# bezirganyan/m2-mixer

Measured on AMD Instinct MI355X. Metric: training samples/sec AV-MNIST M2-Mixer-B bf16, higher is better.
Workload: dtype bf16

## Files before the change

include/m2mixer.h:

```cpp
#ifndef M2MIXER_H
#define M2MIXER_H

#include <stdint.h>

#ifdef __cplusplus
extern "C" {
#endif

#define M2M_ABI_VERSION 18
#define M2M_MAX_BLOCKS 8
#define M2M_ROWS_PER_WG 16

#define M2M_SPLIT_GPART 1472

#define M2M_PREC_BF16 0
#define M2M_PREC_F32 1

typedef struct m2m_block {
    const float* ln1_w;
    const float* ln1_b;
    const float* tok_w1;
    const float* tok_b1;
    const float* tok_w2;
    const float* tok_b2;
// ... 92 lines not shown
    const float* x0; int64_t x0_sample_stride;
    float* out; int64_t out_sample_stride;
    float* pooled;
    int32_t x0_parts;
    int64_t x0_part_stride;
} m2m_tower_io;
int m2m_towers_forward(const m2m_tower* const* towers, const m2m_tower_io* io, int ntowers, int B, int training,
                       uint32_t seed, uint32_t step, const uint32_t* step_dev, void* stream);
int m2m_towers_forward_embeds_ok(const m2m_tower* const* towers, int ntowers, const m2m_embed* const* embeds, int B);
int m2m_towers_forward_embeds(const m2m_tower* const* towers, const m2m_tower_io* io, int ntowers,
                              const m2m_embed* const* embeds, const float* const* inputs, const m2m_step_head* head,
                              int B, int training, uint32_t seed, uint32_t step, const uint32_t* step_dev, void* stream);

int m2m_tower_backward(const m2m_tower* t, int B, const float* d_out, int64_t d_out_sample_stride,
                       const float* d_pooled, float* d_x0, int64_t d_x0_sample_stride,
                       uint32_t seed, uint32_t step, const uint32_t* step_dev, void* stream);
typedef struct m2m_tower_gio {
    const float* d_out; int64_t d_out_sample_stride;
    const float* d_pooled;
    float* d_x0; int64_t d_x0_sample_stride;
} m2m_tower_gio;
int m2m_towers_backward(const m2m_tower* const* towers, const m2m_tower_gio* io, int ntowers, int B,
                        uint32_t seed, uint32_t step, const uint32_t* step_dev, void* stream);
int m2m_tower_wgrad(const m2m_tower* t, int B, uint32_t seed, uint32_t step, const uint32_t* step_dev, void* stream);
int m2m_wgrad_form(const m2m_tower* t, int B);
int m2m_split_form(const m2m_tower* a, const m2m_tower* b, int B, int training);
int m2m_towers_wgrad(const m2m_tower* const* towers, const m2m_tower* const* dev_towers, int ntowers,
                     const m2m_embed* const* embeds, const float* const* inputs, const float* const* d_x0s,
                     const m2m_tower* const* embed_towers, int nembeds,
                     int B, uint32_t seed, uint32_t step, const uint32_t* step_dev, void* stream);
int m2m_wgrad_groups(const m2m_tower* t, int B);
int m2m_embeds_wgrad_form(const m2m_embed* const* embeds, const m2m_tower* const* embed_towers, int nembeds, int B);
int m2m_wgrad_slot_groups(const m2m_tower* const* towers, int ntowers, int B);
int m2m_wgrad_fold(const m2m_tower* t, void* stream);
int m2m_embed_wgrad(const m2m_embed* e, const float* input, const float* d_x0, int B, void* stream);
int m2m_embeds_wgrad(const m2m_embed* const* embeds, const float* const* inputs, const float* const* d_x0s, int nembeds, int B,
                     void* stream);

typedef struct m2m_head {
    const float* pooled;
    const float* w;
    const float* b;
    float* g_w;
    float* g_b;
    float* d_pooled;
    float weight;
    float* g_part;
    const float* tokens;
    int64_t tok_sample_stride;
    int32_t ntok;
} m2m_head;
int m2m_heads_part_tiles(int B);
int m2m_heads_ce(const m2m_head* heads, int nheads, const int64_t* labels, int B, int D, int K,
                 float* logits, float* losses, int32_t* preds, int zero_losses, void* stream);

int m2m_heads_bce(const m2m_head* heads, int nheads, const float* targets, const float* pos_weight, int B, int D, int K,
                  float* logits, float* losses, int32_t* preds, int zero_losses, void* stream);

int m2m_heads_ce_w(const m2m_head* heads, int nheads, const int64_t* labels, int B, int D, int K,
                   float* logits, float* losses, int32_t* preds, int zero_losses, const float* weights, void* stream);
int m2m_heads_bce_w(const m2m_head* heads, int nheads, const float* targets, const float* pos_weight, int B, int D, int K,
                    float* logits, float* losses, int32_t* preds, int zero_losses, const float* weights, void* stream);

int m2m_heads_edl(const m2m_head* heads, int nheads, const int64_t* labels, int B, int D, int K,
                  float* logits, float* losses, int32_t* preds, float* uncertainty, int32_t* combined,
                  int zero_losses, const float* weights, void* stream);

int m2m_towers_wgrad_heads(const m2m_tower* const* towers, const m2m_tower* const* dev_towers, int ntowers,
                           const m2m_embed* const* embeds, const float* const* inputs, const float* const* d_x0s,
                           const m2m_tower* const* embed_towers, int nembeds,
                           int B, uint32_t seed, uint32_t step, const uint32_t* step_dev,
                           const m2m_head* heads, int nheads, int K, void* stream);

int m2m_towers_wgrad_tail(const m2m_tower* const* towers, const m2m_tower* const* dev_towers, int ntowers,
                          const m2m_embed* const* embeds, const float* const* inputs, const float* const* d_x0s,
                          const m2m_tower* const* embed_towers, int nembeds,
                          int B, uint32_t seed, uint32_t step, const uint32_t* step_dev,
                          const m2m_head* heads, int nheads, int K, uint32_t* bump_counter, void* stream);

int m2m_tower_backward_heads_ok(const m2m_tower* t, int B, int nheads, int K);
int m2m_tower_backward_heads(const m2m_tower* t, int B, const m2m_head* heads, int nheads, int own, const int64_t* labels,
                             int K, float* logits, float* losses, int32_t* preds, float* d_x0, int64_t d_x0_sample_stride,
                             uint32_t seed, uint32_t step, const uint32_t* step_dev, void* stream);

#define M2M_MLP_MAX_LAYERS 4
typedef struct m2m_mlp {
    int32_t nlayers;
    int32_t has_out;
    int32_t dims[M2M_MLP_MAX_LAYERS + 1];
    float p_drop;
    uint32_t site_base;
    const float* w[M2M_MLP_MAX_LAYERS];
    const float* b[M2M_MLP_MAX_LAYERS];
    float* g_w[M2M_MLP_MAX_LAYERS];
    float* g_b[M2M_MLP_MAX_LAYERS];
    float* act[M2M_MLP_MAX_LAYERS];
} m2m_mlp;
int m2m_mlp_forward(const m2m_mlp* m, const float* x, int B, float* out, int64_t out_sample_stride, float* out_dense,
                    int training, uint32_t seed, uint32_t step, const uint32_t* step_dev, void* stream);
int m2m_mlp_backward(const m2m_mlp* m, const float* x, int B, const float* d_out, int64_t d_out_sample_stride,
                     const float* d_out_dense, void* stream);
int m2m_mlp_forward_ride(const m2m_mlp* m, const float* x, int B, float* out, int64_t out_sample_stride, float* out_dense,
                         int training, uint32_t seed, uint32_t step, const uint32_t* step_dev);
int m2m_mlp_backward_ride(const m2m_mlp* m, const float* x, int B, const float* d_out, int64_t d_out_sample_stride,
                          const float* d_out_dense);
int m2m_mlp_ride_flush(void* stream);

int m2m_adam_step(float* param, float* grad, float* exp_avg, float* exp_avg_sq, int64_t n,
                  float* state, float beta1, float beta2, float eps, float weight_decay,
                  float grad_scale, int bump_step, void* stream);
int m2m_adam_step_bf16(float* param, float* grad, const void* grad_bf16, float* exp_avg, float* exp_avg_sq, int64_t n,
                       float* state, float beta1, float beta2, float eps, float weight_decay,
                       float grad_scale, int bump_step, void* stream);

#define M2M_MAX_GRAD_RANGES 16
typedef struct m2m_grad_range { int64_t lo, n; const float* add; int32_t keep; int32_t reserved; } m2m_grad_range;
int m2m_adam_step_ranges(float* param, float* grad, const void* grad_bf16, float* exp_avg, float* exp_avg_sq, int64_t n,
                         float* state, float beta1, float beta2, float eps, float weight_decay, float grad_scale, int bump_step,
                         const m2m_grad_range* ranges, int nranges, void* stream);

int64_t m2m_adam_pack_plan_bytes(void);
int m2m_adam_pack_plan(const m2m_tower* const* towers, int ntowers, const m2m_embed* const* embeds, int nembeds,
                       float* param, float* grad, const void* grad_bf16, float* exp_avg, float* exp_avg_sq, int64_t n,
                       const float* state, float beta1, float beta2, float eps, float weight_decay, float grad_scale,
                       void* plan_host);
int m2m_adam_pack_plan_ranges(const m2m_tower* const* towers, int ntowers, const m2m_embed* const* embeds, int nembeds,
                              float* param, float* grad, const void* grad_bf16, float* exp_avg, float* exp_avg_sq, int64_t n,
                              const float* state, float beta1, float beta2, float eps, float weight_decay, float grad_scale,
                              const m2m_grad_range* ranges, int nranges, void* plan_host);
int m2m_adam_pack_all(const m2m_tower* const* towers, int ntowers, const m2m_embed* const* embeds, int nembeds,
                      const void* plan_dev, const void* plan_host, void* stream);

int m2m_step_prologue(float* adam_state, uint32_t* drop_counter, float* losses, int nlosses, void* stream);

int m2m_counter_add(uint32_t* counter, uint32_t delta, void* stream);

#define M2M_FUSION_SUM 1
#define M2M_FUSION_MEAN 2
#define M2M_FUSION_MAX 3
int m2m_fusion_forward(int mode, const float* a, const float* b, float* y, int64_t n, void* stream);
int m2m_fusion_backward(int mode, const float* a, const float* b, const float* dy, float* da, float* db, int64_t n, void* stream);

typedef struct m2m_gate {
    int32_t D;
    int32_t reserved;
    const float *w1, *b1, *w2, *b2, *wz, *bz;
    float *g_w1, *g_b1, *g_w2, *g_b2, *g_wz, *g_bz;
    float *t1, *t2, *z, *dh, *part;
} m2m_gate;
int64_t m2m_gate_part_floats(int64_t rows, int D);
int m2m_gate_forward(const m2m_gate* g, const float* a, const float* b, float* y, int64_t rows, int save, void* stream);
int m2m_gate_backward(const m2m_gate* g, const float* dy, float* da, float* db, int64_t rows, void* stream);
int m2m_gate_wgrad(const m2m_gate* g, const float* a, const float* b, int64_t rows, void* stream);

#define M2M_SCORES_MAX_CLASSES 64
#define M2M_SCORES_MAX_LABELS 128
int m2m_scores_multiclass(const int32_t* preds, const int64_t* labels, int nheads, int B, int K, uint64_t* table, void* stream);
int m2m_scores_multilabel(const int32_t* preds, const float* targets, int nheads, int B, int K, uint64_t* table, void* stream);

#define M2M_RANK_STATE_WORDS 4
int m2m_rank_append(const float* logits, const int64_t* labels, int nheads, int B, int K, float* probs, int32_t* row_labels,
                    int64_t capacity, uint32_t* state, void* stream);
int m2m_rank_counts(const float* probs, const int32_t* row_labels, int nheads, int64_t n, int K, int64_t capacity, uint32_t* counts,
                    void* stream);

int m2m_dropout_mask(const m2m_tower* t, int blk, int site, int B, uint32_t seed, uint32_t step,
// ... 13 lines not shown
```

m2_mixer_amd/_lib.py:

```python
from __future__ import annotations

import ctypes as C
import os
import subprocess

_HERE = os.path.dirname(os.path.abspath(__file__))
LIB_PATH = os.environ.get("M2M_LIB_PATH", os.path.join(_HERE, "libm2mixer.so"))
CSRC = os.path.join(_HERE, "csrc")

ABI_VERSION = 18
MAX_BLOCKS = 8
ROWS_PER_WG = 16
HCHN_PAD = 4096
SPLIT_ROWS = 128
SPLIT_MAX = 8
SPLIT_GPART = 1472
PREC_BF16, PREC_F32 = 0, 1
PREC_BY_NAME = {"bf16": PREC_BF16, "fp32": PREC_F32, "f32": PREC_F32}

_fp = C.c_void_p


class Block(C.Structure):
    PARAMS = ["ln1_w", "ln1_b", "tok_w1", "tok_b1", "tok_w2", "tok_b2", "ln2_w", "ln2_b",
# ... 8 lines not shown
    _fields_ = [("prec", C.c_int32), ("D", C.c_int32), ("N", C.c_int32), ("T", C.c_int32), ("C", C.c_int32),
                ("Cp", C.c_int32), ("nblocks", C.c_int32), ("has_final_ln", C.c_int32),
                ("p_drop", C.c_float), ("site_base", C.c_uint32),
                ("lnf_w", _fp), ("lnf_b", _fp), ("g_lnf_w", _fp), ("g_lnf_b", _fp), ("x_final", _fp),
                ("ws_a", _fp), ("ws_b", _fp), ("blk", Block * MAX_BLOCKS),
                ("slabs", _fp), ("nsplit", C.c_int32), ("wgrad_flags", C.c_int32), ("xres", _fp), ("gpart", _fp),
                ("a_nat", _fp * MAX_BLOCKS), ("dy_nat", _fp * MAX_BLOCKS),
                ("wslot", _fp * MAX_BLOCKS),
                ("dx0_chn", _fp)]


WGRAD_OVERWRITE = 1
WGRAD_REDUCES_SMALL = 2
WGRAD_GROUP_SLOTS = 4
MAX_GRAD_RANGES = 16


class GradRange(C.Structure):
    _fields_ = [("lo", C.c_int64), ("n", C.c_int64), ("add", _fp), ("keep", C.c_int32), ("reserved", C.c_int32)]


class TowerIO(C.Structure):
    _fields_ = [("x0", _fp), ("x0_ss", C.c_int64), ("out", _fp), ("out_ss", C.c_int64), ("pooled", _fp),
                ("x0_parts", C.c_int32), ("x0_part_stride", C.c_int64)]


class StepHead(C.Structure):
    _fields_ = [("adam_state", _fp), ("drop_counter", _fp), ("losses", _fp), ("nlosses", C.c_int32)]


class TowerGIO(C.Structure):
    _fields_ = [("d_out", _fp), ("d_out_ss", C.c_int64), ("d_pooled", _fp), ("d_x0", _fp), ("d_x0_ss", C.c_int64)]


class Embed(C.Structure):
    _fields_ = [("prec", C.c_int32), ("Cin", C.c_int32), ("H", C.c_int32), ("W", C.c_int32), ("ph", C.c_int32),
                ("pw", C.c_int32), ("D", C.c_int32), ("K", C.c_int32), ("Kp", C.c_int32),
                ("w", _fp), ("b", _fp), ("wn", _fp), ("g_w", _fp), ("g_b", _fp), ("wgrad_flags", C.c_int32), ("reserved", C.c_int32)]


class Head(C.Structure):
    _fields_ = [("pooled", _fp), ("w", _fp), ("b", _fp), ("g_w", _fp), ("g_b", _fp), ("d_pooled", _fp),
                ("weight", C.c_float), ("g_part", _fp), ("tokens", _fp), ("tok_sample_stride", C.c_int64), ("ntok", C.c_int32)]


SCORES_MAX_CLASSES, SCORES_MAX_LABELS = 64, 128
RANK_STATE_WORDS = 4
FUSION_SUM, FUSION_MEAN, FUSION_MAX = 1, 2, 3


class Gate(C.Structure):
    _fields_ = [("D", C.c_int32), ("reserved", C.c_int32)] + [(n, _fp) for n in (
        "w1", "b1", "w2", "b2", "wz", "bz", "g_w1", "g_b1", "g_w2", "g_b2", "g_wz", "g_bz", "t1", "t2", "z", "dh", "part")]


MLP_MAX_LAYERS = 4


class Mlp(C.Structure):
    _fields_ = [("nlayers", C.c_int32), ("has_out", C.c_int32), ("dims", C.c_int32 * (MLP_MAX_LAYERS + 1)),
                ("p_drop", C.c_float), ("site_base", C.c_uint32),
                ("w", _fp * MLP_MAX_LAYERS), ("b", _fp * MLP_MAX_LAYERS), ("g_w", _fp * MLP_MAX_LAYERS),
                ("g_b", _fp * MLP_MAX_LAYERS), ("act", _fp * MLP_MAX_LAYERS)]


SIGNATURES = {
    "m2m_abi_version": (C.c_int, []),
    "m2m_last_error": (C.c_char_p, []),
    "m2m_packed_bytes": (C.c_int64, [C.c_int, C.c_int64, C.c_int64]),
    "m2m_pack": (C.c_int, [C.c_int, C.c_int, C.c_int, _fp, C.c_int64, C.c_int64, C.c_int64, C.c_int64, _fp, _fp]),
    "m2m_pack_tower": (C.c_int, [C.POINTER(Tower), _fp]),
    "m2m_pack_embed": (C.c_int, [C.POINTER(Embed), _fp]),
    "m2m_pack_skips_w1tc": (C.c_int, [C.POINTER(Tower)]),
    "m2m_pack_all": (C.c_int, [C.POINTER(C.POINTER(Tower)), C.c_int, C.POINTER(C.POINTER(Embed)), C.c_int, _fp]),
    "m2m_embed_forward": (C.c_int, [C.POINTER(Embed), _fp, C.c_int, _fp, _fp]),
    "m2m_embed_forward_head": (C.c_int, [C.POINTER(Embed), _fp, C.c_int, _fp, C.POINTER(StepHead), _fp]),
    "m2m_tower_forward": (C.c_int, [C.POINTER(Tower), _fp, C.c_int64, C.c_int, _fp, C.c_int64, _fp, C.c_int,
                                    C.c_uint32, C.c_uint32, _fp, _fp]),
    "m2m_tower_backward": (C.c_int, [C.POINTER(Tower), C.c_int, _fp, C.c_int64, _fp, _fp, C.c_int64,
                                     C.c_uint32, C.c_uint32, _fp, _fp]),
    "m2m_tower_backward_heads_ok": (C.c_int, [C.POINTER(Tower), C.c_int, C.c_int, C.c_int]),
    "m2m_tower_backward_heads": (C.c_int, [C.POINTER(Tower), C.c_int, C.POINTER(Head), C.c_int, C.c_int, _fp, C.c_int, _fp, _fp, _fp, _fp,
                                           C.c_int64, C.c_uint32, C.c_uint32, _fp, _fp]),
    "m2m_tower_wgrad": (C.c_int, [C.POINTER(Tower), C.c_int, C.c_uint32, C.c_uint32, _fp, _fp]),
    "m2m_towers_can_group": (C.c_int, [C.POINTER(Tower), C.POINTER(Tower), C.c_int]),
    "m2m_towers_forward": (C.c_int, [C.POINTER(C.POINTER(Tower)), C.POINTER(TowerIO), C.c_int, C.c_int, C.c_int, C.c_uint32,
                                     C.c_uint32, _fp, _fp]),
    "m2m_towers_forward_embeds_ok": (C.c_int, [C.POINTER(C.POINTER(Tower)), C.c_int, C.POINTER(C.POINTER(Embed)), C.c_int]),
    "m2m_towers_forward_embeds": (C.c_int, [C.POINTER(C.POINTER(Tower)), C.POINTER(TowerIO), C.c_int, C.POINTER(C.POINTER(Embed)),
                                            C.POINTER(_fp), C.POINTER(StepHead), C.c_int, C.c_int, C.c_uint32, C.c_uint32, _fp, _fp]),
    "m2m_towers_backward": (C.c_int, [C.POINTER(C.POINTER(Tower)), C.POINTER(TowerGIO), C.c_int, C.c_int, C.c_uint32, C.c_uint32,
                                      _fp, _fp]),
    "m2m_towers_wgrad": (C.c_int, [C.POINTER(C.POINTER(Tower)), C.POINTER(_fp), C.c_int, C.POINTER(C.POINTER(Embed)), C.POINTER(_fp),
                                   C.POINTER(_fp), C.POINTER(C.POINTER(Tower)), C.c_int, C.c_int, C.c_uint32, C.c_uint32, _fp, _fp]),
    "m2m_towers_wgrad_heads": (C.c_int, [C.POINTER(C.POINTER(Tower)), C.POINTER(_fp), C.c_int, C.POINTER(C.POINTER(Embed)), C.POINTER(_fp),
                                         C.POINTER(_fp), C.POINTER(C.POINTER(Tower)), C.c_int, C.c_int, C.c_uint32, C.c_uint32, _fp,
                                         C.POINTER(Head), C.c_int, C.c_int, _fp]),
    "m2m_towers_wgrad_tail": (C.c_int, [C.POINTER(C.POINTER(Tower)), C.POINTER(_fp), C.c_int, C.POINTER(C.POINTER(Embed)), C.POINTER(_fp),
                                        C.POINTER(_fp), C.POINTER(C.POINTER(Tower)), C.c_int, C.c_int, C.c_uint32, C.c_uint32, _fp,
                                        C.POINTER(Head), C.c_int, C.c_int, _fp, _fp]),
    "m2m_heads_part_tiles": (C.c_int, [C.c_int]),
    "m2m_wgrad_form": (C.c_int, [C.POINTER(Tower), C.c_int]),
    "m2m_split_form": (C.c_int, [C.POINTER(Tower), C.POINTER(Tower), C.c_int, C.c_int]),
    "m2m_embeds_wgrad_form": (C.c_int, [C.POINTER(C.POINTER(Embed)), C.POINTER(C.POINTER(Tower)), C.c_int, C.c_int]),
    "m2m_wgrad_groups": (C.c_int, [C.POINTER(Tower), C.c_int]),
    "m2m_wgrad_slot_groups": (C.c_int, [C.POINTER(C.POINTER(Tower)), C.c_int, C.c_int]),
    "m2m_wgrad_fold": (C.c_int, [C.POINTER(Tower), _fp]),
    "m2m_adam_step_ranges": (C.c_int, [_fp, _fp, _fp, _fp, _fp, C.c_int64, _fp, C.c_float, C.c_float, C.c_float, C.c_float,
                                       C.c_float, C.c_int, C.POINTER(GradRange), C.c_int, _fp]),
    "m2m_counter_add": (C.c_int, [_fp, C.c_uint32, _fp]),
    "m2m_embed_wgrad": (C.c_int, [C.POINTER(Embed), _fp, _fp, C.c_int, _fp]),
    "m2m_embeds_wgrad": (C.c_int, [C.POINTER(C.POINTER(Embed)), C.POINTER(_fp), C.POINTER(_fp), C.c_int, C.c_int, _fp]),
    "m2m_embeds_forward": (C.c_int, [C.POINTER(C.POINTER(Embed)), C.POINTER(_fp), C.POINTER(_fp), C.POINTER(C.c_int), C.POINTER(C.c_int64),
                                     C.c_int, C.c_int, C.POINTER(StepHead), _fp]),
    "m2m_embed_fwd_splits": (C.c_int, [C.POINTER(Embed)]),
    "m2m_heads_ce": (C.c_int, [C.POINTER(Head), C.c_int, _fp, C.c_int, C.c_int, C.c_int, _fp, _fp, _fp, C.c_int, _fp]),
    "m2m_step_prologue": (C.c_int, [_fp, _fp, _fp, C.c_int, _fp]),
    "m2m_heads_bce": (C.c_int, [C.POINTER(Head), C.c_int, _fp, _fp, C.c_int, C.c_int, C.c_int, _fp, _fp, _fp, C.c_int, _fp]),
    "m2m_heads_ce_w": (C.c_int, [C.POINTER(Head), C.c_int, _fp, C.c_int, C.c_int, C.c_int, _fp, _fp, _fp, C.c_int, _fp, _fp]),
    "m2m_heads_bce_w": (C.c_int, [C.POINTER(Head), C.c_int, _fp, _fp, C.c_int, C.c_int, C.c_int, _fp, _fp, _fp, C.c_int, _fp, _fp]),
    "m2m_heads_edl": (C.c_int, [C.POINTER(Head), C.c_int, _fp, C.c_int, C.c_int, C.c_int, _fp, _fp, _fp, _fp, _fp, C.c_int, _fp, _fp]),
    "m2m_fusion_forward": (C.c_int, [C.c_int, _fp, _fp, _fp, C.c_int64, _fp]),
    "m2m_fusion_backward": (C.c_int, [C.c_int, _fp, _fp, _fp, _fp, _fp, C.c_int64, _fp]),
    "m2m_gate_part_floats": (C.c_int64, [C.c_int64, C.c_int]),
    "m2m_gate_forward": (C.c_int, [C.POINTER(Gate), _fp, _fp, _fp, C.c_int64, C.c_int, _fp]),
    "m2m_gate_backward": (C.c_int, [C.POINTER(Gate), _fp, _fp, _fp, C.c_int64, _fp]),
    "m2m_gate_wgrad": (C.c_int, [C.POINTER(Gate), _fp, _fp, C.c_int64, _fp]),
    "m2m_scores_multiclass": (C.c_int, [_fp, _fp, C.c_int, C.c_int, C.c_int, _fp, _fp]),
    "m2m_scores_multilabel": (C.c_int, [_fp, _fp, C.c_int, C.c_int, C.c_int, _fp, _fp]),
    "m2m_rank_append": (C.c_int, [_fp, _fp, C.c_int, C.c_int, C.c_int, _fp, _fp, C.c_int64, _fp, _fp]),
    "m2m_rank_counts": (C.c_int, [_fp, _fp, C.c_int, C.c_int64, C.c_int, C.c_int64, _fp, _fp]),
    "m2m_mlp_forward": (C.c_int, [C.POINTER(Mlp), _fp, C.c_int, _fp, C.c_int64, _fp, C.c_int, C.c_uint32, C.c_uint32,
                                  _fp, _fp]),
    "m2m_mlp_backward": (C.c_int, [C.POINTER(Mlp), _fp, C.c_int, _fp, C.c_int64, _fp, _fp]),
    "m2m_mlp_forward_ride": (C.c_int, [C.POINTER(Mlp), _fp, C.c_int, _fp, C.c_int64, _fp, C.c_int, C.c_uint32, C.c_uint32, _fp]),
    "m2m_mlp_backward_ride": (C.c_int, [C.POINTER(Mlp), _fp, C.c_int, _fp, C.c_int64, _fp]),
    "m2m_mlp_ride_flush": (C.c_int, [_fp]),
    "m2m_adam_step": (C.c_int, [_fp, _fp, _fp, _fp, C.c_int64, _fp, C.c_float, C.c_float, C.c_float, C.c_float,
                                C.c_float, C.c_int, _fp]),
    "m2m_adam_step_bf16": (C.c_int, [_fp, _fp, _fp, _fp, _fp, C.c_int64, _fp, C.c_float, C.c_float, C.c_float, C.c_float,
                                     C.c_float, C.c_int, _fp]),
    "m2m_adam_pack_plan_bytes": (C.c_int64, []),
    "m2m_adam_pack_plan": (C.c_int, [C.POINTER(C.POINTER(Tower)), C.c_int, C.POINTER(C.POINTER(Embed)), C.c_int, _fp, _fp, _fp, _fp, _fp,
                                    C.c_int64, _fp, C.c_float, C.c_float, C.c_float, C.c_float, C.c_float, _fp]),
    "m2m_adam_pack_plan_ranges": (C.c_int, [C.POINTER(C.POINTER(Tower)), C.c_int, C.POINTER(C.POINTER(Embed)), C.c_int, _fp, _fp, _fp, _fp, _fp,
                                           C.c_int64, _fp, C.c_float, C.c_float, C.c_float, C.c_float, C.c_float,
                                           C.POINTER(GradRange), C.c_int, _fp]),
    "m2m_adam_pack_all": (C.c_int, [C.POINTER(C.POINTER(Tower)), C.c_int, C.POINTER(C.POINTER(Embed)), C.c_int, _fp, _fp, _fp]),
    "m2m_dropout_mask": (C.c_int, [C.POINTER(Tower), C.c_int, C.c_int, C.c_int, C.c_uint32, C.c_uint32, _fp, _fp]),
    "m2m_gelu_probe": (C.c_int, [_fp, _fp, _fp, C.c_int64, _fp]),
    "m2m_gelu_table_probe": (C.c_int, [C.c_int, _fp, _fp, _fp, C.c_int64, C.c_float, _fp]),
    "m2m_gemm_probe": (C.c_int, [C.c_int, _fp, _fp, C.c_int, C.c_int, C.c_int, _fp, C.c_int, _fp, _fp, _fp, _fp]),
    "m2m_clock_probe": (C.c_int, [_fp, C.c_int, C.c_int, _fp]),
}

_lib = None


def csrc_hash() -> str:
    import glob
    import hashlib
    h = hashlib.sha256()
    for f in sorted(glob.glob(os.path.join(CSRC, "*.hip")) + glob.glob(os.path.join(CSRC, "*.h")) +
                    [os.path.join(os.path.dirname(_HERE), "include", "m2mixer.h")]):
        h.update(os.path.basename(f).encode())
        h.update(open(f, "rb").read())
    return h.hexdigest()


def build(force: bool = False, verbose: bool = False) -> str:
    if force:
        subprocess.run(["make", "-C", CSRC, "clean"], check=True, capture_output=not verbose)
    r = subprocess.run(["make", "-C", CSRC, "-j", str(min(6, os.cpu_count() or 2))], capture_output=True, text=True)
    if r.returncode != 0:
        raise RuntimeError("building libm2mixer.so failed:\n" + r.stdout[-4000:] + r.stderr[-4000:])
    if verbose:
        print(r.stdout)
    return LIB_PATH


def lib() -> C.CDLL:
    global _lib
    if _lib is None:
# ... 36 lines not shown
```

m2_mixer_amd/csrc/heads.hip:

```cpp
#include "dispatch.h"

#define HEAD_S 16
#define HEAD_MAXK 32
#define HEAD_MAXH 4

struct HeadArgs {
    m2m_head h[HEAD_MAXH];
    const float* weights;
};

template <bool BCE, int S, int DD>
__global__ __launch_bounds__(NTHREADS) void heads_kernel(const HeadArgs ha, const void* __restrict__ labels_v,
                                                         const float* __restrict__ pos_weight, int B, int D_rt,
                                                         int K, float* __restrict__ logits_out, float* __restrict__ losses,
                                                         int32_t* __restrict__ preds, int nheads) {
    const int64_t* labels = reinterpret_cast<const int64_t*>(labels_v);
    const float* targets = reinterpret_cast<const float*>(labels_v);
    extern __shared__ __attribute__((aligned(16))) char smem[];
    constexpr int D = DD, DL = DD + 4, D4 = DD / 4;
    float* pl = reinterpret_cast<float*>(smem);
    float* wl = pl + S * DL;
    float* lg = wl + HEAD_MAXK * DL;
    float* red = lg + S * HEAD_MAXK;
    float* tm = red + S;

    const int tid = threadIdx.x;
    const int hI = blockIdx.y;
    const m2m_head& hd = ha.h[hI];
    const float hw = ha.weights ? ha.weights[hI] : hd.weight;
    const int s0 = blockIdx.x * S;
    const int ns = min(S, B - s0);

    {
        constexpr int NP = (S * D4 + NTHREADS - 1) / NTHREADS, NW = (HEAD_MAXK * D4 + NTHREADS - 1) / NTHREADS;
        f32x4_t pv[NP], wv[NW];
#pragma unroll
        for (int i = 0; i < NP; ++i) {
            const int idx = tid + i * NTHREADS, sI = idx / D4, c = (idx % D4) * 4;
            pv[i] = f32x4_t{0.f, 0.f, 0.f, 0.f};
            if (idx < S * D4 && sI < ns) {
                if (hd.tokens) {
                    const float* col = hd.tokens + (long)(s0 + sI) * hd.tok_sample_stride + c;
                    const int N = hd.ntok;
                    f32x4_t a = f32x4_t{0.f, 0.f, 0.f, 0.f};
                    for (int n0 = 0; n0 < N; n0 += 8) {
                        f32x4_t t8[8];
#pragma unroll
                        for (int j = 0; j < 8; ++j) t8[j] = *reinterpret_cast<const f32x4_t*>(col + (long)min(n0 + j, N - 1) * D);
#pragma unroll
                        for (int j = 0; j < 8; ++j)
                            if (n0 + j < N) a += t8[j];
                    }
                    pv[i] = a * (1.0f / (float)N);
                } else pv[i] = *reinterpret_cast<const f32x4_t*>(hd.pooled + (long)(s0 + sI) * D + c);
            }
        }
#pragma unroll
        for (int i = 0; i < NW; ++i) {
            const int idx = tid + i * NTHREADS;
            wv[i] = f32x4_t{0.f, 0.f, 0.f, 0.f};
            if (idx < K * D4) wv[i] = *reinterpret_cast<const f32x4_t*>(hd.w + (long)idx * 4);
        }
#pragma unroll
        for (int i = 0; i < NP; ++i) {
            const int idx = tid + i * NTHREADS;
            if (idx < S * D4) *reinterpret_cast<f32x4_t*>(pl + (idx / D4) * DL + (idx % D4) * 4) = pv[i];
        }
#pragma unroll
        for (int i = 0; i < NW; ++i) {
            const int idx = tid + i * NTHREADS;
            if (idx < HEAD_MAXK * D4) *reinterpret_cast<f32x4_t*>(wl + (idx / D4) * DL + (idx % D4) * 4) = wv[i];
        }
    }
    __syncthreads();
    for (int idx = tid >> 2; idx < S * K; idx += NTHREADS / 4) {
        const int sI = idx / K, k = idx % K, part = tid & 3;
        constexpr int NC = D4 / 4;
        f32x4_t a4[NC], b4[NC];
#pragma unroll
        for (int c = 0; c < NC; ++c) {
            a4[c] = *reinterpret_cast<const f32x4_t*>(pl + sI * DL + 4 * (part + 4 * c));
            b4[c] = *reinterpret_cast<const f32x4_t*>(wl + k * DL + 4 * (part + 4 * c));
        }
        float a = 0.f;
#pragma unroll
        for (int c = 0; c < NC; ++c)
#pragma unroll
            for (int e = 0; e < 4; ++e) a = __builtin_fmaf(a4[c][e], b4[c][e], a);
        a = wave_sum_xor(a, 4) + hd.b[k];
        if (part == 0) {
            lg[sI * HEAD_MAXK + k] = a;
            if (sI < ns) logits_out[((long)hI * B + s0 + sI) * K + k] = a;
        }
    }
    __syncthreads();
    if (BCE) {
        const float scale = hw / ((float)B * (float)K);
        for (int idx = tid; idx < S * K; idx += NTHREADS) {
            const int sI = idx / K, k = idx % K;
            float term = 0.f, dl = 0.f;
            if (sI < ns) {
                const float x = lg[sI * HEAD_MAXK + k], y = targets[(long)(s0 + sI) * K + k], pw = pos_weight[k];
                const float ls = __builtin_fminf(x, 0.f) - log1pf(__expf(-__builtin_fabsf(x)));
                term = -(pw * y * ls + (1.f - y) * (ls - x));
                const float sg = 1.0f / (1.0f + __expf(-x));
                dl = scale * ((1.f - y) * sg - pw * y * (1.f - sg));
                preds[((long)hI * B + s0 + sI) * K + k] = x > 0.f ? 1 : 0;
            }
            lg[sI * HEAD_MAXK + k] = dl;
            tm[sI * HEAD_MAXK + k] = term;
        }
        __syncthreads();
        if (tid < S) {
            float term = 0.f;
            for (int k = 0; k < K; ++k) term += tm[tid * HEAD_MAXK + k];
            red[tid] = term / (float)K;
        }
    } else if (tid < S * 32) {
        const int sI = tid >> 5, k = tid & 31;
        const bool live = k < K;
        const float v = live ? lg[sI * HEAD_MAXK + k] : -3.0e38f;
        float mx = v;
        int am = live ? k : 0x7fffffff;
#pragma unroll
        for (int o = 16; o >= 1; o >>= 1) {
            const float ov = __shfl_xor(mx, o, 64);
            const int oa = __shfl_xor(am, o, 64);
            if (ov > mx || (ov == mx && oa < am)) { mx = ov; am = oa; }
        }
        const float ex = live ? __expf(v - mx) : 0.f;
        float se = ex;
#pragma unroll
        for (int o = 16; o >= 1; o >>= 1) se += __shfl_xor(se, o, 64);
        const int y = sI < ns ? (int)labels[s0 + sI] : 0;
        const float scale = hw / (float)B;
        const float dl = sI < ns ? scale * (ex * (1.0f / se) - (k == y ? 1.f : 0.f)) : 0.f;
        const float vy = __shfl(v, (tid & 32) + y, 64);
        if (live) lg[sI * HEAD_MAXK + k] = dl;
        if (k == 0) {
            red[sI] = sI < ns ? (__logf(se) + mx) - vy : 0.f;
            if (sI < ns) preds[(long)hI * B + s0 + sI] = am;
        }
    }
    __syncthreads();
    if (tid == 0) {
        float t = 0.f;
#pragma unroll
        for (int sI = 0; sI < S; ++sI) t += red[sI];
        t /= (float)B;
        atomicAdd(losses + hI, t);
        atomicAdd(losses + nheads, t * hw);
    }
    if (hd.d_pooled) {
        for (int idx = tid; idx < ns * D4; idx += NTHREADS) {
            const int sI = idx / D4, c = (idx % D4) * 4;
            f32x4_t a = f32x4_t{0.f, 0.f, 0.f, 0.f};
            int k = 0;
            for (; k + 4 <= K; k += 4) {
                f32x4_t w4[4];
                float d4[4];
#pragma unroll
                for (int j = 0; j < 4; ++j) { w4[j] = *reinterpret_cast<const f32x4_t*>(wl + (k + j) * DL + c); d4[j] = lg[sI * HEAD_MAXK + k + j]; }
#pragma unroll
                for (int j = 0; j < 4; ++j)
#pragma unroll
                    for (int e = 0; e < 4; ++e) a[e] = __builtin_fmaf(d4[j], w4[j][e], a[e]);
            }
            for (; k < K; ++k) {
                const f32x4_t w4 = *reinterpret_cast<const f32x4_t*>(wl + k * DL + c);
                const float dk = lg[sI * HEAD_MAXK + k];
#pragma unroll
                for (int e = 0; e < 4; ++e) a[e] = __builtin_fmaf(dk, w4[e], a[e]);
            }
            *reinterpret_cast<f32x4_t*>(hd.d_pooled + (long)(s0 + sI) * D + c) = a;
        }
        float* slot = hd.g_part ? hd.g_part + (long)blockIdx.x * M2M_SPLIT_GPART : nullptr;
        for (int idx = tid; idx < K * D4; idx += NTHREADS) {
            const int k = idx / D4, c = (idx % D4) * 4;
            f32x4_t p4[S];
            float d1[S];
#pragma unroll
            for (int sI = 0; sI < S; ++sI) { p4[sI] = *reinterpret_cast<const f32x4_t*>(pl + sI * DL + c); d1[sI] = lg[sI * HEAD_MAXK + k]; }
            f32x4_t a = f32x4_t{0.f, 0.f, 0.f, 0.f};
#pragma unroll
            for (int sI = 0; sI < S; ++sI)
#pragma unroll
                for (int e = 0; e < 4; ++e) a[e] = __builtin_fmaf(d1[sI], p4[sI][e], a[e]);
            if (slot) *reinterpret_cast<f32x4_t*>(slot + (long)k * D + c) = a;
            else {
#pragma unroll
                for (int e = 0; e < 4; ++e) atomicAdd(hd.g_w + (long)k * D + c + e, a[e]);
            }
        }
        if (tid < K) {
            float a = 0.f;
#pragma unroll
            for (int sI = 0; sI < S; ++sI) a += lg[sI * HEAD_MAXK + tid];
            if (slot) slot[K * D + tid] = a;
            else atomicAdd(hd.g_b + tid, a);
        }
        if (slot && tid < 2) slot[K * D + K + tid] = 0.f;
    }
}

__global__ void zero_floats_kernel(float* p, int n) {
    if ((int)threadIdx.x < n) p[threadIdx.x] = 0.f;
}

template <bool BCE, int S, int DD>
static int launch_heads_sd(const HeadArgs& ha, int nheads, const void* labels, const float* pos_weight, int B, int K,
                           float* logits, float* losses, int32_t* preds, hipStream_t st) {
    const size_t lds = sizeof(float) * ((size_t)S * (DD + 4) + (size_t)HEAD_MAXK * (DD + 4) + 2 * S * HEAD_MAXK + S);
    return m2m_launch<heads_kernel<BCE, S, DD>>(dim3((B + S - 1) / S, nheads), dim3(NTHREADS), lds, 160 * 1024, st, ha, labels, pos_weight, B, DD, K, logits,
                                                losses, preds, nheads);
}
template <bool BCE, int S>
static int launch_heads_s(const HeadArgs& ha, int nheads, const void* labels, const float* pos_weight, int B, int D, int K,
                          float* logits, float* losses, int32_t* preds, hipStream_t st) {
    const int rc = m2m_dispatch(m2m_wide_dims{}, D, M2M_NO_BUILD, [&](auto DD) {
        return launch_heads_sd<BCE, S, DD()>(ha, nheads, labels, pos_weight, B, K, logits, losses, preds, st);
    });
    if (rc != M2M_NO_BUILD) return rc;
    m2m_set_error("heads: hidden_dim must be 32, 64, 128 or 256", __FILE__, __LINE__);
// ... 62 lines not shown
```

m2_mixer_amd/csrc/host.h:

```cpp
#pragma once
#include "split.h"

void m2m_set_error(const char* msg, const char* file, int line);
int m2m_check_tower(const m2m_tower* t, int B);

static inline int64_t ceil_div(int64_t a, int64_t b) { return (a + b - 1) / b; }



int m2m_check_embed(const m2m_embed* e, int B);

bool m2m_can_group(const m2m_tower* a, const m2m_tower* b);
int m2m_chain_forward_rows(const m2m_tower* t, const float* x0, long x0_ss, int B, float* out, long out_ss, int training,
                           unsigned int seed, unsigned int step, const unsigned int* step_dev, hipStream_t st);
int m2m_chain_forward_rows_group(const m2m_tower* const* v, const float* const* x0, const long* x0_ss, int B, float* const* out,
                                 const long* out_ss, int training, unsigned int seed, unsigned int step, const unsigned int* step_dev,
                                 hipStream_t st);

bool m2m_small_part_deferred(SplitReduceTower& x, const m2m_tower* t, int B);
int m2m_chain_backward_rows(const m2m_tower* t, int B, const float* d_out, long d_out_ss, const float* d_pooled, float* d_x0,
                            long d_x0_ss, unsigned int seed, unsigned int step, const unsigned int* step_dev, hipStream_t st);
int m2m_chain_backward_rows_group(const m2m_tower* const* v, int B, const float* const* d_out, const long* d_out_ss,
                                  const float* const* d_pooled, float* const* d_x0, const long* d_x0_ss, unsigned int seed,
                                  unsigned int step, const unsigned int* step_dev, hipStream_t st);

bool m2m_wgrad_recompute(const m2m_tower* t, int B);

bool m2m_can_group_wide(const m2m_tower* a, const m2m_tower* b, int B);
int m2m_forward_wide(const m2m_tower* t, const float* x0, long x0_ss, int B, float* out, long out_ss, float* pooled,
                     int training, unsigned int seed, unsigned int step, const unsigned int* step_dev, hipStream_t st);
int m2m_backward_wide(const m2m_tower* t, int B, const float* d_out, long d_out_ss, const float* d_pooled, float* d_x0,
                      long d_x0_ss, unsigned int seed, unsigned int step, const unsigned int* step_dev, hipStream_t st);
int m2m_forward_wide_group(const m2m_tower* const* tw, const m2m_tower_io* io, int B, int training, unsigned int seed,
                           unsigned int step, const unsigned int* step_dev, hipStream_t st);
int m2m_backward_wide_group(const m2m_tower* const* tw, const m2m_tower_gio* io, int B, unsigned int seed, unsigned int step,
                            const unsigned int* step_dev, hipStream_t st);

bool m2m_split_eligible(const m2m_tower* t, int B, int training);
bool m2m_split_can_group(const m2m_tower* a, const m2m_tower* b);
int m2m_split_forward(const m2m_tower* const* towers, const m2m_tower_io* io, int ntow, int B, int training, unsigned int seed,
                      unsigned int step, const unsigned int* step_dev, hipStream_t st);
int m2m_split_backward(const m2m_tower* const* towers, const m2m_tower_gio* io, int ntow, int B, unsigned int seed, unsigned int step,
                       const unsigned int* step_dev, hipStream_t st);

int m2m_split_mix_forward(const SplitMixArgs& a, int D, int training, float p_drop, unsigned int seed, unsigned int step,
                          const unsigned int* step_dev, hipStream_t st);
int m2m_split_mix_backward(const SplitMixBwdArgs& a, int D, float p_drop, unsigned int seed, unsigned int step,
                           const unsigned int* step_dev, hipStream_t st);
int m2m_split_small_grads(const SplitReduceArgs& a, hipStream_t st);

int m2m_split_chain_forward(const SplitChainArgs& a, int D, int training, float p_drop, unsigned int seed, unsigned int step,
                            const unsigned int* step_dev, hipStream_t st);
int m2m_split_chain_backward(const SplitChainArgs& a, int D, float p_drop, unsigned int seed, unsigned int step,
                             const unsigned int* step_dev, hipStream_t st);
```

m2_mixer_amd/csrc/tower_bwd.hip:

```cpp
#include "tile.h"
#include "token_mfma.h"
#include "dispatch.h"
#include <algorithm>

#define BH_MAXH 3
struct BwdHeads {
    m2m_head h[BH_MAXH];
    const int64_t* labels;
    float* logits;
    int32_t* preds;
    int nheads, K, own;
};

template <int P, int D, int NMAX, int TG> struct BwdLds {
    static constexpr bool TOK = NMAX > 0;
    static constexpr int NM = TOK ? NMAX : 1, TW_LD = 2 * NM + 4, XLD = D + 4;
    static constexpr int RED_LD0 = ((32 / TG) * (1 + 2 * NM) + NM) * TG;
    static constexpr int RED_LD = RED_LD0 > TokRed<NM>::LD ? RED_LD0 : TokRed<NM>::LD;
    static constexpr int PB = 4 * D + (TOK ? 32 * TW_LD : 0);
    static constexpr size_t FIXED = (size_t)BM * XLD * sizeof(float) * (1 + RowSlabs<D>::N + 2) + 2 * (size_t)BM * D * Prec<P>::ESZ +
                                    GELU_TAB_N * sizeof(gtabh_t) + (TOK ? (size_t)NWAVES * RED_LD * sizeof(float) : 0);
    static size_t bytes(int nblocks, int N, int Cp) {
        return FIXED + (TOK ? (size_t)(BM / N) * D * sizeof(unsigned int) : 0) + (size_t)nblocks * PB * sizeof(float) +
               (size_t)Cp * sizeof(float) + 16 + 8 * (M2M_MAX_BLOCKS + 1 + BH_MAXH);
    }
};
#ifdef M2M_TIMERS
#define M2M_LDS_MAX (163840 - 1024)
#else
#define M2M_LDS_MAX 163840
#endif

TIMER_DECL(g_tm_bwd);
__device__ int g_bwd_static_split = 1;
static int bwd_split_mode_init(hipStream_t st) {
    static bool done = false;
    if (done) return 0;
    if (m2m_env_int("M2M_BWD_TICKETS", 0) != 0) {
        const int v = 0;
        hipStreamCaptureStatus cs = hipStreamCaptureStatusNone;
        (void)hipStreamIsCapturing(st, &cs);
        if (cs != hipStreamCaptureStatusNone) { m2m_set_error("tower_backward: first launch with M2M_BWD_TICKETS=1 inside a stream capture (run one eager step first)", __FILE__, __LINE__); return -1; }
        M2M_CHECK_HIP(hipMemcpyToSymbol(HIP_SYMBOL(g_bwd_static_split), &v, sizeof(v)));
    }
    done = true;
    return 0;
}
TIMER_READER(m2m_debug_timers_bwd, g_tm_bwd)

template <class TW, int P, int D, int NMAX, int TG, int DM, bool PART = false, bool HREC = false, bool HEADS = false>
static __device__ __forceinline__ void tower_bwd_body(const TW& tw, int B, const float* __restrict__ d_out, long d_out_ss,
                                                      const float* __restrict__ d_pooled, float* __restrict__ d_x0, long d_x0_ss,
                                                      unsigned int seed, unsigned int step_host,
                                                      const unsigned int* __restrict__ step_dev, int wg, int nwg, char* smem,
                                                      float* __restrict__ part = nullptr, char* dx0_chn = nullptr,
                                                      const BwdHeads* hd = nullptr) {
    typedef Prec<P> Pr;
    typedef TileGeom<D> G;
    typedef BwdLds<P, D, NMAX, TG> L;
    constexpr int XLD = G::XLD, DT = G::DT, KD = D / Pr::KB, NF = Chain<P>::NF;
    constexpr bool TOK = NMAX > 0;
    constexpr int NM = TOK ? NMAX : 1;
    constexpr int TILE_F = BM * XLD;
    constexpr int IMG_B = BM * D * Pr::ESZ;
    constexpr int EPT = D / TPR, NSL = RowSlabs<D>::N;
    constexpr int TW_LD = 2 * NM + 4, RED_LD = L::RED_LD, PB = L::PB;
    constexpr int O_LN1W = 0, O_LN1B = D, O_LN2W = 2 * D, O_LN2B = 3 * D, O_TOKW = 4 * D;

    float* dxs = reinterpret_cast<float*>(smem);
    float* slabs = dxs + TILE_F;
    float* t_prod = slabs;
    float* t_up = slabs + TILE_F;
    float* ub = slabs + 2 * TILE_F;
    float* dov = slabs + 3 * TILE_F;
    float* tdy = slabs + NSL * TILE_F;
    float* ta = tdy + TILE_F;
    char* at = reinterpret_cast<char*>(ta + TILE_F);
    char* dyp = at + IMG_B;
    gtabh_t* gtab = reinterpret_cast<gtabh_t*>(dyp + IMG_B);
    float* red = reinterpret_cast<float*>(gtab + GELU_TAB_N);
    unsigned int* wth = reinterpret_cast<unsigned int*>(red + (TOK ? NWAVES * RED_LD : 0));
    float* par = reinterpret_cast<float*>(wth + (TOK ? (BM / tw.N) * D : 0));
    float* bias_s = par + tw.nblocks * PB;
    unsigned int* qctr = reinterpret_cast<unsigned int*>(bias_s + tw.Cp);
    unsigned long long* slotp = reinterpret_cast<unsigned long long*>(qctr + 4);

    const int tid = threadIdx.x, lane = tid & 63, g = lane >> 4, il = lane & 15;
    const int wave = tid >> 6;
    const int N = tw.N, T = tw.T, Cp = tw.Cp;
    const int SPW = TOK ? BM / N : 0;
    const int s0 = wg * SPW;
    const int ns = TOK ? min(SPW, B - s0) : 0;
    const long row0 = TOK ? (long)s0 * N : (long)wg * BM;
    const int R = TOK ? ns * N : (int)min((long)BM, (long)B * N - row0);
    constexpr int TPP = WPAIR / BM;
    const long pair_off = (long)(wg / TPP) * (WPAIR * D * Pr::ESZ);
    const int tile_in_pair = wg % TPP;
    const unsigned int step = step_host + (step_dev ? *step_dev : 0u);

    TIMER_LSTART();
    if (PART && threadIdx.x <= (unsigned)tw.nblocks + (HEADS ? BH_MAXH : 0))
        slotp[threadIdx.x] = (unsigned long long)(part + ((long)threadIdx.x * nwg + wg) * SPP_STRIDE);
    float* hdp = slabs + 3 * 4 * D + BH_MAXH * 32 * (D + 1) + BH_MAXH * 4 * 32;
    if constexpr (HEADS && PART && TOK) {
        const int nh = hd->nheads, K = hd->K, DL = D + 1;
        float* hpool = slabs;
        float* hwt = hpool + 3 * 4 * D;
        float* hlog = hwt + BH_MAXH * 32 * DL;
        for (int i = tid; i < nh * SPW * D; i += NTHREADS) {
            const int h = i / (SPW * D), sl = (i / D) % SPW, d = i % D;
            hpool[(h * 4 + sl) * D + d] = sl < ns ? hd->h[h].pooled[(long)(s0 + sl) * D + d] : 0.f;
        }
        for (int i = tid; i < nh * K * D; i += NTHREADS) {
            const int h = i / (K * D), k = (i / D) % K, d = i % D;
            hwt[(h * 32 + k) * DL + d] = hd->h[h].w[k * D + d];
        }
        __syncthreads();
        for (int i = tid >> 3; i < nh * SPW * K; i += NTHREADS / 8) {
            const int h = i / (SPW * K), sl = (i / K) % SPW, k = i % K, part8 = tid & 7;
            float a = 0.f;
            for (int d = part8; d < D; d += 8) a = __builtin_fmaf(hpool[(h * 4 + sl) * D + d], hwt[(h * 32 + k) * DL + d], a);
            a = wave_sum_xor(a, 8) + hd->h[h].b[k];
            if (part8 == 0) {
                hlog[(h * 4 + sl) * 32 + k] = a;
                if (sl < ns) hd->logits[((long)h * B + s0 + sl) * K + k] = a;
            }
        }
        __syncthreads();
        float term = 0.f;
        if (tid < nh * SPW) {
            const int h = tid / SPW, sl = tid % SPW;
            float* lg = hlog + (h * 4 + sl) * 32;
            if (sl < ns) {
                const int y = (int)hd->labels[s0 + sl];
                float mx = lg[0];
                int am = 0;
                for (int k = 1; k < K; ++k) { const float v = lg[k]; if (v > mx) { mx = v; am = k; } }
                float se = 0.f;
                for (int k = 0; k < K; ++k) se += __expf(lg[k] - mx);
                term = (__logf(se) + mx - lg[y]) / (float)B;
                const float scale = hd->h[h].weight / (float)B, inv = 1.0f / se;
                for (int k = 0; k < K; ++k) lg[k] = scale * (__expf(lg[k] - mx) * inv - (k == y ? 1.f : 0.f));
                hd->preds[(long)h * B + s0 + sl] = am;
            } else {
                for (int k = 0; k < K; ++k) lg[k] = 0.f;
            }
            hlog[BH_MAXH * 4 * 32 - 16 + tid] = term;
        }
        __syncthreads();
        for (int i = tid; i < nh * ns * D; i += NTHREADS) {
            const int h = i / (ns * D), sl = (i / D) % ns, d = i % D;
            float a = 0.f;
            for (int k = 0; k < K; ++k) a = __builtin_fmaf(hlog[(h * 4 + sl) * 32 + k], hwt[(h * 32 + k) * DL + d], a);
            if (h == hd->own) hdp[sl * D + d] = a;
            else hd->h[h].d_pooled[(long)(s0 + sl) * D + d] = a;
        }
        for (int i = tid; i < nh * (K * D + K + 2); i += NTHREADS) {
            const int h = i / (K * D + K + 2), e = i % (K * D + K + 2);
            float* sl_h = reinterpret_cast<float*>(slotp[tw.nblocks + 1 + h]);
            float a = 0.f;
            if (e < K * D) {
                const int k = e / D, d = e % D;
                for (int sl = 0; sl < SPW; ++sl) a = __builtin_fmaf(hlog[(h * 4 + sl) * 32 + k], hpool[(h * 4 + sl) * D + d], a);
            } else if (e < K * D + K) {
                for (int sl = 0; sl < SPW; ++sl) a += hlog[(h * 4 + sl) * 32 + (e - K * D)];
            } else {
                for (int sl = 0; sl < SPW; ++sl) a += hlog[BH_MAXH * 4 * 32 - 16 + h * SPW + sl];
                if (e == K * D + K + 1) a *= hd->h[h].weight;
            }
            sl_h[e] = a;
        }
        __syncthreads();
    }
    constexpr int MAXB = (int)(sizeof(tw.blk) / sizeof(tw.blk[0]));
    constexpr int XI = (BM * (D / 4) + NTHREADS - 1) / NTHREADS, BPT = 8, TI = TOK ? (32 * TW_LD + NTHREADS - 1) / NTHREADS : 1;
    float4 uv[XI];
    {
        const float invN = 1.0f / (float)N;
#pragma unroll
        for (int k = 0; k < XI; ++k) {
            const int idx = tid + k * NTHREADS, r = idx / (D / 4), c = (idx % (D / 4)) * 4;
            uv[k] = make_float4(0.f, 0.f, 0.f, 0.f);
            if (idx < BM * (D / 4) && r < R) {
                const long gr = row0 + r, gs = gr / N;
                if (d_out) uv[k] = *reinterpret_cast<const float4*>(d_out + gs * d_out_ss + (gr % N) * D + c);
                if constexpr (HEADS && PART && TOK) {
                    const float4 p = *reinterpret_cast<const float4*>(hdp + (gs - s0) * D + c);
                    uv[k].x += p.x * invN; uv[k].y += p.y * invN; uv[k].z += p.z * invN; uv[k].w += p.w * invN;
                } else if (d_pooled) {
                    const float4 p = *reinterpret_cast<const float4*>(d_pooled + gs * D + c);
                    uv[k].x += p.x * invN; uv[k].y += p.y * invN; uv[k].z += p.z * invN; uv[k].w += p.w * invN;
                }
            }
        }
    }
    float xm[EPT];
    float nb[BPT];
    {
        const int r = tid / TPR, j = tid % TPR;
#pragma unroll
        for (int e = 0; e < EPT; ++e) xm[e] = 0.f;
        if (r < R) ld_row<D>(tw.blk[tw.nblocks - 1].x_mid + (row0 + r) * D, j, xm);
        const M2M_AS1 float* b1p = reinterpret_cast<const M2M_AS1 float*>(to_gptr(tw.blk[tw.nblocks - 1].ch_b1p));
#pragma unroll
        for (int k = 0; k < BPT; ++k) {
            nb[k] = 0.f;
            if (tid + k * NTHREADS < Cp) nb[k] = b1p[tid + k * NTHREADS];
        }
    }
    float pv[MAXB][4], tv[TI][MAXB];
#pragma unroll
    for (int b = 0; b < MAXB; ++b) {
#pragma unroll
        for (int q = 0; q < 4; ++q) pv[b][q] = 0.f;
        if (b < tw.nblocks && tid < D) {
            const m2m_block& bk = tw.blk[b];
            if (TOK) { pv[b][0] = bk.ln1_w[tid]; pv[b][1] = bk.ln1_b[tid]; }
            pv[b][2] = bk.ln2_w[tid]; pv[b][3] = bk.ln2_b[tid];
        }
#pragma unroll
        for (int k = 0; k < TI; ++k) {
            tv[k][b] = 0.f;
            const int idx = tid + k * NTHREADS, t = idx / TW_LD, j = idx % TW_LD;
            if (TOK && b < tw.nblocks && idx < 32 * TW_LD && t < T) {
                const m2m_block& bk = tw.blk[b];
                const M2M_AS1 float* w1 = reinterpret_cast<const M2M_AS1 float*>(to_gptr(bk.tok_w1));
                const M2M_AS1 float* w2 = reinterpret_cast<const M2M_AS1 float*>(to_gptr(bk.tok_w2));
                const M2M_AS1 float* b1 = reinterpret_cast<const M2M_AS1 float*>(to_gptr(bk.tok_b1));
                const bool v1 = j < NMAX, v2 = !v1 && j < 2 * NMAX;
                const M2M_AS1 float* src = v1 ? w1 + (t * N + j) : (v2 ? w2 + ((j - NMAX) * T + t) : b1 + t);
                const bool ok = v1 ? j < N : (v2 ? j - NMAX < N : j == 2 * NMAX);
                if (ok) tv[k][b] = *src;
            }
        }
    }
    if (Act<P>::USES_TABLE) gelu_tabh_fill(gtab, make_drop(true, tw.p_drop, 0u, 0u, 0u).scale, tid, NTHREADS);
#pragma unroll
    for (int b = 0; b < MAXB; ++b)
        if (b < tw.nblocks) {
            float* pb = par + b * PB;
            if (tid < D) {
                if (TOK) { pb[O_LN1W + tid] = pv[b][0]; pb[O_LN1B + tid] = pv[b][1]; }
                pb[O_LN2W + tid] = pv[b][2]; pb[O_LN2B + tid] = pv[b][3];
            }
            if constexpr (TOK) {
#pragma unroll
                for (int k = 0; k < TI; ++k)
                    if (tid + k * NTHREADS < 32 * TW_LD) pb[O_TOKW + tid + k * NTHREADS] = tv[k][b];
            }
        }
    {
#pragma unroll
        for (int k = 0; k < XI; ++k) {
            const int idx = tid + k * NTHREADS, r = idx / (D / 4), c = (idx % (D / 4)) * 4;
            if (idx < BM * (D / 4)) *reinterpret_cast<float4*>((tw.has_final_ln ? tdy : dxs) + r * XLD + c) = uv[k];
        }
        __syncthreads();
        if (tw.has_final_ln)
        {
            if constexpr (PART) {
                float* sl = reinterpret_cast<float*>(slotp[0]);
                ln_backward_tile<D, false>(tw.x_final + row0 * D, R, tdy, tw.lnf_w, dxs, false, ta, sl + SPP_LNF(D), sl + SPP_LNF(D) + D, tid);
            } else
            ln_backward_tile<D>(tw.x_final + row0 * D, R, tdy, tw.lnf_w, dxs, false, ta, tw.g_lnf_w, tw.g_lnf_b, tid);
        }
    }

    TIMER_LMARK(0);
    int pend = -1;
    auto colsums = [&](const float* pw, const float* pb_, float* gw, float* gb, int t0, bool store = false) {
        _Pragma("unroll 1") for (int d = t0; d < 2 * D; d += NTHREADS) {
            const float* src = d < D ? pw : pb_;
            const int c = d < D ? d : d - D;
            float s_ = 0.f;
#pragma unroll 4
            for (int r = 0; r < BM; ++r) s_ += src[r * XLD + c];
            if (store) (d < D ? gw : gb)[c] = s_;
            else atomicAdd((d < D ? gw : gb) + c, s_);
        }
    };
    auto slot_of = [&](int b) -> float* { return PART ? reinterpret_cast<float*>(slotp[tw.nblocks - b]) : nullptr; };
    for (int b = tw.nblocks - 1; b >= 0; --b) {
        const m2m_block& bk = tw.blk[b];
        const float* pb = par + b * PB;
        const unsigned int site = tw.site_base + 4u * b;
        const Drop dr_th = make_drop(true, tw.p_drop, seed, step, site + 0);
        const Drop dr_to = make_drop(true, tw.p_drop, seed, step, site + 1);
        const Drop dr_ch = make_drop(true, tw.p_drop, seed, step, site + 2);
        const Drop dr_co = make_drop(true, tw.p_drop, seed, step, site + 3);

        int tb1 = tid;
        asm volatile("" : "+v"(tb1));
        {
            const int r = tb1 / TPR, j = tb1 % TPR;
            float dy[EPT], a[EPT], mean, rstd;
            ld_row<D>(dxs + r * XLD, j, dy);
#pragma unroll
            for (int e = 0; e < EPT; ++e) {
                const int c = ln_col<D>(e, j);
                const float v = drop_keep_elem<DM>(dr_co, (unsigned int)(row0 + r) * D + c) ? dy[e] * dr_co.scale : 0.f;
                dy[e] = r < R ? v : 0.f;
            }
            st_row<D>(tdy + r * XLD, j, dy);
            pack_row_nat<P, D>(dyp, r, j, dy);
            reg_stats<D>(xm, mean, rstd);
#pragma unroll
            for (int e = 0; e < EPT; ++e) {
                const int c = ln_col<D>(e, j);
                a[e] = (xm[e] - mean) * rstd * pb[O_LN2W + c] + pb[O_LN2B + c];
            }
            st_row<D>(ta + r * XLD, j, a);
            pack_row_nat<P, D>(at, r, j, a);
            if (TOK && pend >= 0) {
                float* sl = slot_of(pend);
                if constexpr (PART) colsums(t_prod, ub, sl + SPP_LN1(D), sl + SPP_LN1(D) + D, tb1, true);
                else colsums(t_prod, ub, tw.blk[pend].g_ln1_w, tw.blk[pend].g_ln1_b, tb1);
            }
            if (tb1 == 0) *qctr = NWAVES;
#pragma unroll
            for (int k = 0; k < BPT; ++k)
                if (tb1 + k * NTHREADS < Cp) bias_s[tb1 + k * NTHREADS] = nb[k];
        }
        __syncthreads();
        TIMER_LMARK(1);
        gptr_w_t p_gb2 = to_gptr_w(bk.g_ch_b2), p_dyt = to_gptr_w(bk.dyt_chn), p_atc = to_gptr_w(bk.at_chn);
        gptr_t p_w1n = to_gptr(bk.w1n), p_w2tn = to_gptr(bk.w2tn), p_w1tc = to_gptr(bk.w1tc);
        gptr_w_t p_dh = to_gptr_w(bk.dh_chn), p_h = to_gptr_w(bk.h_chn);
        asm volatile("" : "+s"(p_gb2), "+s"(p_dyt), "+s"(p_atc), "+s"(p_w1n), "+s"(p_w2tn), "+s"(p_w1tc), "+s"(p_dh), "+s"(p_h));
        constexpr bool HOLD0 = D <= 128;
        const unsigned int lane16_0 = (unsigned int)lane * 16u;
        Frag w1f[2][HOLD0 ? D / Pr::KB : 1], w2f[2][HOLD0 ? D / Pr::KB : 1];
        if (HOLD0 && wave < (Cp >> 5)) {
#pragma unroll
// ... 584 lines not shown
            gxsum = wave_sum_xor(gxsum, TPR) * (1.0f / D);
            ld_row<D>(dxs + r * XLD, j, dx);
            float pr[EPT];
#pragma unroll
            for (int e = 0; e < EPT; ++e) {
                const bool valid = r < R;
                if (valid) dx[e] += rstd1 * (gg[e] - gsum - xh1[e] * gxsum);
                pr[e] = valid ? du[e] * xh1[e] : 0.f;
                if (!valid) du[e] = 0.f;
            }
            st_row<D>(dxs + r * XLD, j, dx);
            st_row<D>(t_prod + r * XLD, j, pr);
            st_row<D>(ub + r * XLD, j, du);
            pend = b;
        }
        }
        if (b > 0) {
            const int r = tb3 / TPR, j = tb3 % TPR;
#pragma unroll
            for (int e = 0; e < EPT; ++e) xm[e] = 0.f;
            if (r < R) ld_row<D>(tw.blk[b - 1].x_mid + (row0 + r) * D, j, xm);
            const M2M_AS1 float* b1p = reinterpret_cast<const M2M_AS1 float*>(to_gptr(tw.blk[b - 1].ch_b1p));
#pragma unroll
            for (int k = 0; k < BPT; ++k) {
                nb[k] = 0.f;
                if (tb3 + k * NTHREADS < Cp) nb[k] = b1p[tb3 + k * NTHREADS];
            }
        }
        __syncthreads();
        TIMER_LMARK(6);
    }
    if (TOK && pend >= 0) {
        float* sl = slot_of(pend);
        if constexpr (PART) colsums(t_prod, ub, sl + SPP_LN1(D), sl + SPP_LN1(D) + D, tid, true);
        else colsums(t_prod, ub, tw.blk[pend].g_ln1_w, tw.blk[pend].g_ln1_b, tid);
    }

    _Pragma("unroll 1") for (int idx = tid; idx < R * (D / 4); idx += NTHREADS) {
        const int r = idx / (D / 4), c = (idx % (D / 4)) * 4;
        const long gr = row0 + r;
        *reinterpret_cast<float4*>(d_x0 + (gr / N) * d_x0_ss + (gr % N) * D + c) =
            *reinterpret_cast<const float4*>(dxs + r * XLD + c);
    }
    if (dx0_chn) pack_tile_chn_t<P, D>(dxs, dx0_chn + pair_off, tile_in_pair, tid);
    TIMER_LFLUSH(g_tm_bwd);
}

template <int P, int D, int NMAX, int TG, int DM, bool PART = false, bool HREC = false>
__global__ __launch_bounds__(NTHREADS) void tower_bwd_kernel(const m2m_tower tw, int B, const float* __restrict__ d_out,
                                                             long d_out_ss, const float* __restrict__ d_pooled,
                                                             float* __restrict__ d_x0, long d_x0_ss, unsigned int seed,
                                                             unsigned int step_host, const unsigned int* __restrict__ step_dev) {
    extern __shared__ __attribute__((aligned(16))) char smem[];
    tower_bwd_body<m2m_tower, P, D, NMAX, TG, DM, PART, HREC>(tw, B, d_out, d_out_ss, d_pooled, d_x0, d_x0_ss, seed, step_host, step_dev,
                                                               blockIdx.x, gridDim.x, smem, PART ? tw.gpart : nullptr, (char*)tw.dx0_chn);
}
template <int P, int D, int NMAX, int TG, int DM, bool HREC>
__global__ __launch_bounds__(NTHREADS) void tower_bwd_heads_kernel(const m2m_tower tw, const BwdHeads hd, int B, float* __restrict__ d_x0,
                                                                   long d_x0_ss, unsigned int seed, unsigned int step_host,
                                                                   const unsigned int* __restrict__ step_dev) {
    extern __shared__ __attribute__((aligned(16))) char smem[];
    tower_bwd_body<m2m_tower, P, D, NMAX, TG, DM, true, HREC, true>(tw, B, nullptr, 0, nullptr, d_x0, d_x0_ss, seed, step_host, step_dev,
                                                                     blockIdx.x, gridDim.x, smem, tw.gpart, (char*)tw.dx0_chn, &hd);
}

struct BwdGroupArgs {
    m2m_tower4 tw[2];
    const float* d_out[2];
    long d_out_ss[2];
    const float* d_pooled[2];
    float* d_x0[2];
    long d_x0_ss[2];
    int ntiles[2];
    float* part[2];
    char* dx0_chn[2];
};
static_assert(sizeof(BwdGroupArgs) <= 3584, "kernel arguments are limited to 4 KiB");

static bool m2m_small_part(const m2m_tower* t) {
    static const bool off = m2m_env_int("M2M_SMALL_PART", 1) == 0;
    return !off && t->gpart != nullptr && !m2m_is_wide(t) && t->prec == PREC_BF16 && t->D == 128 && t->nblocks >= 1 &&
           2 * t->T * t->N + t->T + t->N <= SPP_TOK_MAX;
}
static void m2m_small_part_reduce_args(SplitReduceTower& x, const m2m_tower* t, int nwg, const BwdHeads* hd = nullptr, float* losses = nullptr) {
    memset(&x, 0, sizeof(x));
    x.part = t->gpart; x.ntiles = nwg; x.nlaunch = t->nblocks + 1; x.D = t->D; x.N = t->N; x.T = t->T;
    if (hd) {
        x.head_set0 = t->nblocks + 1; x.nheads = hd->nheads; x.K = hd->K; x.losses = losses;
        for (int h = 0; h < hd->nheads; ++h) { x.g_hw[h] = hd->h[h].g_w; x.g_hb[h] = hd->h[h].g_b; }
        x.nlaunch += hd->nheads;
    }
    if (t->has_final_ln) { x.g_lnf_w = t->g_lnf_w; x.g_lnf_b = t->g_lnf_b; }
    for (int b = 0; b < t->nblocks; ++b) {
        const int L = t->nblocks - b;
        const m2m_block& k = t->blk[b];
        x.g_ln2_w[L] = k.g_ln2_w; x.g_ln2_b[L] = k.g_ln2_b;
        x.g_tok_w1[L] = k.g_tok_w1; x.g_tok_w2[L] = k.g_tok_w2; x.g_tok_b1[L] = k.g_tok_b1; x.g_tok_b2[L] = k.g_tok_b2;
        x.g_ln1_w[L] = k.g_ln1_w; x.g_ln1_b[L] = k.g_ln1_b;
        x.g_b2[L] = k.g_ch_b2;
    }
}
bool m2m_small_part_deferred(SplitReduceTower& x, const m2m_tower* t, int B) {
    if (!t || m2m_is_wide(t) || t->N < 1 || t->N > 8 || !m2m_small_part(t) || m2m_split_eligible(t, B, 1)) return false;
    const int SPW = BM / t->N;
    m2m_small_part_reduce_args(x, t, (B + SPW - 1) / SPW);
    return true;
}
template <int P, int D, int NMAX, int TG, int DM, bool PART = false, bool HREC = false>
__global__ __launch_bounds__(NTHREADS) void tower_bwd_group_kernel(const BwdGroupArgs a, int B, unsigned int seed,
                                                                   unsigned int step_host, const unsigned int* __restrict__ step_dev) {
    extern __shared__ __attribute__((aligned(16))) char smem[];
    const int id = blockIdx.x, xcd = id & 7, t = xcd >> 2;
    const int wg = (id >> 3) * 4 + (xcd & 3);
    if (wg >= a.ntiles[t]) return;
    tower_bwd_body<m2m_tower4, P, D, NMAX, TG, DM, PART, HREC>(a.tw[t], B, a.d_out[t], a.d_out_ss[t], a.d_pooled[t], a.d_x0[t], a.d_x0_ss[t],
                                                                seed, step_host, step_dev, wg, a.ntiles[t], smem, PART ? a.part[t] : nullptr, a.dx0_chn[t]);
}

#ifdef M2M_ISA_PROBE
template __global__ void tower_bwd_group_kernel<PREC_BF16, 128, 4, 8, DM_HALF, true, false>(const BwdGroupArgs, int, unsigned int, unsigned int, const unsigned int*);
template __global__ void tower_bwd_kernel<PREC_BF16, 128, 8, 16, DM_HALF, true, false>(const m2m_tower, int, const float*, long, const float*, float*, long, unsigned int, unsigned int, const unsigned int*);
#else
template <int P, int D, int NMAX, int TG>
static size_t bwd_lds_bytes(int nblocks, int N, int Cp) { return BwdLds<P, D, NMAX, TG>::bytes(nblocks, N, Cp); }

template <bool CAN_PART, bool CAN_HREC, class F>
static int bwd_forms(bool part, bool hrec, F&& f) {
    if constexpr (CAN_PART && CAN_HREC) { if (part && hrec) return f(std::true_type{}, std::true_type{}); }
    if constexpr (CAN_PART) { if (part) return f(std::true_type{}, std::false_type{}); }
    if constexpr (CAN_HREC) { if (hrec) return f(std::false_type{}, std::true_type{}); }
    return f(std::false_type{}, std::false_type{});
}

template <int P, int D, int NMAX, int TG, int DM>
static int launch_bwd_group_dm(const BwdGroupArgs& a, int B, unsigned int seed, unsigned int step, const unsigned int* step_dev,
                               hipStream_t st, bool hrec_req) {
    const size_t lds = std::max(bwd_lds_bytes<P, D, NMAX, TG>(a.tw[0].nblocks, a.tw[0].N, a.tw[0].Cp),
                                bwd_lds_bytes<P, D, NMAX, TG>(a.tw[1].nblocks, a.tw[1].N, a.tw[1].Cp));
    if (lds > M2M_LDS_MAX || a.tw[0].Cp > 8 * NTHREADS || a.tw[1].Cp > 8 * NTHREADS) {
        m2m_set_error("towers_backward: blocks x channel_dim exceed the workgroup's LDS", __FILE__, __LINE__);
        return -1;
    }
    constexpr bool CAN_PART = P == PREC_BF16 && D == 128 && NMAX > 0;
    const bool part = CAN_PART && a.part[0] && a.part[1];
    constexpr bool CAN_HREC = P == PREC_BF16 && D == 128 && DM != DM_GEN;
    const bool hrec = CAN_HREC && hrec_req;
    if (hrec_req && !CAN_HREC) { m2m_set_error("towers_backward: recompute form requested for an instantiation without it", __FILE__, __LINE__); return -1; }
    const int mx = a.ntiles[0] > a.ntiles[1] ? a.ntiles[0] : a.ntiles[1];
    const int grid = 8 * ((mx + 3) / 4);
    return bwd_forms<CAN_PART, CAN_HREC>(part, hrec, [&](auto PART, auto HREC) {
        return m2m_launch<tower_bwd_group_kernel<P, D, NMAX, TG, DM, PART(), HREC()>>(dim3(grid), dim3(NTHREADS), lds, M2M_LDS_MAX, st, a, B, seed,
                                                                                     step, step_dev);
    });
}
template <int P, int D, int NMAX, int TG>
static int launch_bwd_group(const BwdGroupArgs& a, int B, unsigned int seed, unsigned int step, const unsigned int* step_dev,
                            hipStream_t st, bool hrec) {
    return m2m_dispatch_dm(1, a.tw[0].p_drop, [&](auto DM) { return launch_bwd_group_dm<P, D, NMAX, TG, DM()>(a, B, seed, step, step_dev, st, hrec); });
}

template <int P, int D, int NMAX, int TG, int DM>
static int launch_bwd_dm(const m2m_tower* t, int B, const float* d_out, long d_out_ss, const float* d_pooled, float* d_x0,
                      long d_x0_ss, unsigned int seed, unsigned int step, const unsigned int* step_dev, hipStream_t st) {
    const int SPW = NMAX > 0 ? BM / t->N : 1;
    const int grid = NMAX > 0 ? (B + SPW - 1) / SPW : (int)(((long)B * t->N + BM - 1) / BM);
    const size_t lds = bwd_lds_bytes<P, D, NMAX, TG>(t->nblocks, t->N, t->Cp);
    if (lds > M2M_LDS_MAX || t->Cp > 8 * NTHREADS) { m2m_set_error("tower_backward: blocks x channel_dim exceed the workgroup's LDS", __FILE__, __LINE__); return -1; }
    constexpr bool CAN_PART = P == PREC_BF16 && D == 128 && NMAX > 0;
    const bool part = CAN_PART && m2m_small_part(t);
    constexpr bool CAN_HREC = P == PREC_BF16 && D == 128 && DM != DM_GEN;
    const bool hrec = CAN_HREC && m2m_wgrad_recompute(t, B);
    const int rc = bwd_forms<CAN_PART, CAN_HREC>(part, hrec, [&](auto PART, auto HREC) {
        return m2m_launch<tower_bwd_kernel<P, D, NMAX, TG, DM, PART(), HREC()>>(dim3(grid), dim3(NTHREADS), lds, M2M_LDS_MAX, st, *t, B, d_out, d_out_ss,
                                                                               d_pooled, d_x0, d_x0_ss, seed, step, step_dev);
    });
    if (rc) return rc;
    if (part && !(t->wgrad_flags & M2M_WGRAD_REDUCES_SMALL)) {
        SplitReduceArgs r;
        memset(&r, 0, sizeof(r));
        r.ntow = 1;
        m2m_small_part_reduce_args(r.t[0], t, grid);
        return m2m_split_small_grads(r, st);
    }
    return 0;
}

template <int P, int D, int NMAX, int TG, int DM>
static int launch_bwd_heads_dm(const m2m_tower* t, int B, const BwdHeads& hd, float* losses, float* d_x0, long d_x0_ss, unsigned int seed,
                               unsigned int step, const unsigned int* step_dev, hipStream_t st) {
    const int SPW = BM / t->N;
    const int grid = (B + SPW - 1) / SPW;
    const size_t lds = bwd_lds_bytes<P, D, NMAX, TG>(t->nblocks, t->N, t->Cp);
    if (lds > M2M_LDS_MAX || t->Cp > 8 * NTHREADS) { m2m_set_error("tower_backward_heads: blocks x channel_dim exceed the workgroup's LDS", __FILE__, __LINE__); return -1; }
    constexpr bool CAN_HREC = DM != DM_GEN;
    const bool hrec = CAN_HREC && m2m_wgrad_recompute(t, B);
    const int rc = bwd_forms<false, CAN_HREC>(false, hrec, [&](auto, auto HREC) {
        return m2m_launch<tower_bwd_heads_kernel<P, D, NMAX, TG, DM, HREC()>>(dim3(grid), dim3(NTHREADS), lds, M2M_LDS_MAX, st, *t, hd, B, d_x0, d_x0_ss,
                                                                             seed, step, step_dev);
    });
    if (rc) return rc;
    SplitReduceArgs r;
    memset(&r, 0, sizeof(r));
    r.ntow = 1;
    m2m_small_part_reduce_args(r.t[0], t, grid, &hd, losses);
    return m2m_split_small_grads(r, st);
}

template <int P, int D, int NMAX, int TG>
static int launch_bwd(const m2m_tower* t, int B, const float* d_out, long d_out_ss, const float* d_pooled, float* d_x0,
                      long d_x0_ss, unsigned int seed, unsigned int step, const unsigned int* step_dev, hipStream_t st) {
    return m2m_dispatch_dm(1, t->p_drop, [&](auto DM) {
        return launch_bwd_dm<P, D, NMAX, TG, DM()>(t, B, d_out, d_out_ss, d_pooled, d_x0, d_x0_ss, seed, step, step_dev, st);
    });
}

int m2m_chain_backward_rows(const m2m_tower* t, int B, const float* d_out, long d_out_ss, const float* d_pooled, float* d_x0,
                            long d_x0_ss, unsigned int seed, unsigned int step, const unsigned int* step_dev, hipStream_t st) {
    if (int rc = bwd_split_mode_init(st)) return rc;
    const int rc = m2m_dispatch_pd(m2m_wide_dims{}, t->prec, t->D, [&](auto P, auto D) {
        return launch_bwd<P(), D(), 0, 8>(t, B, d_out, d_out_ss, d_pooled, d_x0, d_x0_ss, seed, step, step_dev, st);
    });
    if (rc != M2M_NO_BUILD) return rc;
    m2m_set_error("tower_backward (wide): unsupported (prec, D)", __FILE__, __LINE__);
    return -1;
}

int m2m_chain_backward_rows_group(const m2m_tower* const* v, int B, const float* const* d_out, const long* d_out_ss,
                                  const float* const* d_pooled, float* const* d_x0, const long* d_x0_ss, unsigned int seed,
                                  unsigned int step, const unsigned int* step_dev, hipStream_t st) {
    if (int rc = bwd_split_mode_init(st)) return rc;
    BwdGroupArgs a;
    memset(&a, 0, sizeof(a));
    for (int i = 0; i < 2; ++i) {
        a.tw[i] = m2m_shrink(v[i]);
        a.d_out[i] = d_out[i]; a.d_out_ss[i] = d_out_ss[i]; a.d_pooled[i] = d_pooled[i];
        a.d_x0[i] = d_x0[i]; a.d_x0_ss[i] = d_x0_ss[i];
        a.ntiles[i] = (int)(((long)B * v[i]->N + BM - 1) / BM);
    }
    const m2m_tower* t = v[0];
    const int rc = m2m_dispatch_pd(m2m_pair_dims{}, t->prec, t->D, [&](auto P, auto D) {
        return launch_bwd_group<P(), D(), 0, 8>(a, B, seed, step, step_dev, st, false);
    });
    if (rc != M2M_NO_BUILD) return rc;
    m2m_set_error("towers_backward (wide): hidden_dim 256 only", __FILE__, __LINE__);
    return -1;
}

extern "C" int m2m_towers_backward(const m2m_tower* const* towers, const m2m_tower_gio* io, int ntowers, int B, uint32_t seed,
                                   uint32_t step, const uint32_t* step_dev, void* stream) {
    if (!towers || !io || ntowers != 2) { m2m_set_error("towers_backward: exactly two towers per launch", __FILE__, __LINE__); return -1; }
    if (int rc = bwd_split_mode_init(reinterpret_cast<hipStream_t>(stream))) return rc;
    for (int i = 0; i < 2; ++i)
        if (int rc = m2m_check_tower(towers[i], B)) return rc;
    if (m2m_split_eligible(towers[0], B, 1) && m2m_split_eligible(towers[1], B, 1) && m2m_split_can_group(towers[0], towers[1]))
        return m2m_split_backward(towers, io, 2, B, seed, step, step_dev, reinterpret_cast<hipStream_t>(stream));
    for (int i = 0; i < 2; ++i)
        if ((towers[i]->wgrad_flags & M2M_WGRAD_REDUCES_SMALL) && m2m_split_eligible(towers[i], B, 1)) {
            m2m_set_error("towers_backward: a tower with M2M_WGRAD_REDUCES_SMALL is eligible for the column-split path but its partner is not: launch them separately", __FILE__, __LINE__);
            return -1;
        }
    if (m2m_can_group_wide(towers[0], towers[1], B))
        return m2m_backward_wide_group(towers, io, B, seed, step, step_dev, reinterpret_cast<hipStream_t>(stream));
    if (!m2m_can_group(towers[0], towers[1])) {
        m2m_set_error("towers_backward: the two towers do not share a kernel instantiation: launch them separately", __FILE__, __LINE__);
        return -1;
    }
    BwdGroupArgs a;
    for (int i = 0; i < 2; ++i) {
        a.tw[i] = m2m_shrink(towers[i]);
        a.d_out[i] = io[i].d_out; a.d_out_ss[i] = (long)io[i].d_out_sample_stride;
        a.d_pooled[i] = io[i].d_pooled;
        a.d_x0[i] = io[i].d_x0; a.d_x0_ss[i] = (long)io[i].d_x0_sample_stride;
        a.dx0_chn[i] = (char*)towers[i]->dx0_chn;
        const int SPW = BM / towers[i]->N;
        a.ntiles[i] = (B + SPW - 1) / SPW;
    }
    static const bool group_part = m2m_env_int("M2M_SMALL_PART", 1) == 2;
    const bool flagged = (towers[0]->wgrad_flags & M2M_WGRAD_GROUP_SLOTS) && (towers[1]->wgrad_flags & M2M_WGRAD_GROUP_SLOTS);
    const bool part = (group_part || flagged) && m2m_small_part(towers[0]) && m2m_small_part(towers[1]);
    const bool defer = flagged && (towers[0]->wgrad_flags & M2M_WGRAD_REDUCES_SMALL) && (towers[1]->wgrad_flags & M2M_WGRAD_REDUCES_SMALL);
    for (int i = 0; i < 2; ++i) {
        const int f = towers[i]->wgrad_flags;
        if (((f & M2M_WGRAD_GROUP_SLOTS) && !part) || ((f & M2M_WGRAD_REDUCES_SMALL) && !defer)) {
            m2m_set_error("towers_backward: M2M_WGRAD_GROUP_SLOTS / M2M_WGRAD_REDUCES_SMALL must be set on both towers, with slot buffers (gpart)", __FILE__, __LINE__);
            return -1;
        }
    }
    for (int i = 0; i < 2; ++i) a.part[i] = part ? towers[i]->gpart : nullptr;
    hipStream_t st = reinterpret_cast<hipStream_t>(stream);
    const m2m_tower* t = towers[0];
    const bool hrec = m2m_wgrad_recompute(towers[0], B) && m2m_wgrad_recompute(towers[1], B);
    if (hrec != (m2m_wgrad_recompute(towers[0], B) || m2m_wgrad_recompute(towers[1], B))) {
        m2m_set_error("towers_backward: the two towers disagree on the weight-gradient form: launch them separately", __FILE__, __LINE__);
        return -1;
    }
    auto finish = [&](int rc) -> int {
        if (rc || !part || defer) return rc;
        SplitReduceArgs r;
        memset(&r, 0, sizeof(r));
        r.ntow = 2;
        for (int i = 0; i < 2; ++i) m2m_small_part_reduce_args(r.t[i], towers[i], a.ntiles[i]);
        return m2m_split_small_grads(r, st);
    };
    const int rc = m2m_dispatch_pd(m2m_fused_dims{}, t->prec, t->D, [&](auto P, auto D) {
        return m2m_fused_class(t->N, t->T, [&](auto NMAX, auto TG) {
            return finish(launch_bwd_group<P(), D(), NMAX(), TG()>(a, B, seed, step, step_dev, st, hrec));
        });
    });
    if (rc != M2M_NO_BUILD) return rc;
    m2m_set_error("towers_backward: unsupported (prec, D)", __FILE__, __LINE__);
    return -1;
}

extern "C" int m2m_tower_backward_heads_ok(const m2m_tower* t, int B, int nheads, int K) {
    if (!t || m2m_check_tower(t, B) != 0) return 0;
    static const bool on = m2m_env_int("M2M_FUSED_HEADS", 0) == 1;
    if (!on || !m2m_small_part(t) || m2m_split_eligible(t, B, 1)) return 0;
    if (nheads < 1 || nheads > BH_MAXH || K < 2 || K * t->D + K + 2 > SPP_STRIDE || K > 16) return 0;
    return 1;
}
extern "C" int m2m_tower_backward_heads(const m2m_tower* t, int B, const m2m_head* heads, int nheads, int own, const int64_t* labels,
                                        int K, float* logits, float* losses, int32_t* preds, float* d_x0, int64_t d_x0_ss,
                                        uint32_t seed, uint32_t step, const uint32_t* step_dev, void* stream) {
    if (!m2m_tower_backward_heads_ok(t, B, nheads, K)) { m2m_set_error("tower_backward_heads: unsupported tower / heads (see m2m_tower_backward_heads_ok)", __FILE__, __LINE__); return -1; }
    if (!heads || !labels || !logits || !losses || !preds || !d_x0 || own < 0 || own >= nheads) { m2m_set_error("tower_backward_heads: null argument", __FILE__, __LINE__); return -1; }
    if (int rc = bwd_split_mode_init(reinterpret_cast<hipStream_t>(stream))) return rc;
    BwdHeads hd;
    memset(&hd, 0, sizeof(hd));
    for (int h = 0; h < nheads; ++h) {
        hd.h[h] = heads[h];
        if (!heads[h].pooled || !heads[h].w || !heads[h].b || !heads[h].g_w || !heads[h].g_b || (h != own && !heads[h].d_pooled)) {
            m2m_set_error("tower_backward_heads: incomplete head", __FILE__, __LINE__);
            return -1;
        }
    }
    hd.labels = labels; hd.logits = logits; hd.preds = preds; hd.nheads = nheads; hd.K = K; hd.own = own;
    hipStream_t st = reinterpret_cast<hipStream_t>(stream);
    return m2m_fused_class(t->N, t->T, [&](auto NMAX, auto TG) {
        return m2m_dispatch_dm(1, t->p_drop, [&](auto DM) {
            return launch_bwd_heads_dm<PREC_BF16, 128, NMAX(), TG(), DM()>(t, B, hd, losses, d_x0, d_x0_ss, seed, step, step_dev, st);
        });
    });
}

extern "C" int m2m_tower_backward(const m2m_tower* t, int B, const float* d_out, int64_t d_out_ss, const float* d_pooled,
                                  float* d_x0, int64_t d_x0_ss, uint32_t seed, uint32_t step, const uint32_t* step_dev, void* stream) {
    if (int rc = m2m_check_tower(t, B)) return rc;
    hipStream_t st = reinterpret_cast<hipStream_t>(stream);
    if (int rc = bwd_split_mode_init(st)) return rc;
    if (m2m_is_wide(t)) return m2m_backward_wide(t, B, d_out, d_out_ss, d_pooled, d_x0, d_x0_ss, seed, step, step_dev, st);
    if (m2m_split_eligible(t, B, 1)) {
        m2m_tower_gio io1;
        io1.d_out = d_out; io1.d_out_sample_stride = d_out_ss; io1.d_pooled = d_pooled; io1.d_x0 = d_x0; io1.d_x0_sample_stride = d_x0_ss;
        return m2m_split_backward(&t, &io1, 1, B, seed, step, step_dev, st);
    }
    const int rc = m2m_dispatch_pd(m2m_fused_dims{}, t->prec, t->D, [&](auto P, auto D) {
        return m2m_fused_class(t->N, t->T, [&](auto NMAX, auto TG) {
            return launch_bwd<P(), D(), NMAX(), TG()>(t, B, d_out, d_out_ss, d_pooled, d_x0, d_x0_ss, seed, step, step_dev, st);
        });
    });
    if (rc != M2M_NO_BUILD) return rc;
    m2m_set_error("tower_backward: unsupported (prec, D)", __FILE__, __LINE__);
    return -1;
}
#endif
```

m2_mixer_amd/csrc/tower_wgrad.hip:

```cpp
#include "tile.h"
#include "embed_wgrad.h"
#include "dispatch.h"
#include <string.h>

#if defined(__HIP_DEVICE_COMPILE__)
#define M2M_GLOBAL_AS __attribute__((address_space(1)))
#else
#define M2M_GLOBAL_AS
#endif

#define WBM 32
#define WG_RING_MAX 24
#define WG_WAVES 4
#define WG_WAVES_WIDE 5
#define WG_LA 4
#define WG_MINWAVES 2
#define WG_OUT_ATOMIC 0
#define WG_OUT_ADD 1
#define WG_OUT_STORE 2

TIMER_DECL(g_tm_wg);
TIMER_READER(m2m_debug_timers_wgrad, g_tm_wg)

#include "tower_wgrad_rc.h"
// ... 360 lines not shown

bool m2m_wgrad_recompute(const m2m_tower* t, int B) {
    static const int on = m2m_env_int("M2M_WGRAD_RECOMP", 0);
    if (!on || t->prec != PREC_BF16 || t->D != 128 || t->nblocks < 1 || t->Cp < 64) return false;
    if (m2m_drop_mode(1, t->p_drop) == DM_GEN) return false;
    if (m2m_split_eligible(t, B, 1)) return false;
    return true;
}
extern "C" int m2m_wgrad_form(const m2m_tower* t, int B) { return t && m2m_wgrad_recompute(t, B) ? 1 : 0; }

static bool wgrad_slot_usable(const m2m_tower* t) {
    static const int on = m2m_env_int("M2M_WGRAD_SLOT", 1);
    if (!on || t->nblocks < 1) return false;
    for (int b = 0; b < t->nblocks; ++b) {
        const m2m_block& k = t->blk[b];
        if (!t->wslot[b]) return false;
        if (k.g_ch_b1 != k.g_ch_w1 + (long)t->C * t->D || k.g_ch_w2 != k.g_ch_b1 + t->C) return false;
    }
    return true;
}

struct WgradPlan { int ntiles, nsl, groups, tpg, rpt, slot; };
static WgradPlan wgrad_plan(const m2m_tower* t, int B, int cols, bool honour_overwrite = true) {
    const bool wide = m2m_is_wide(t);
    const int SPW = wide ? 1 : BM / t->N;
    const int nchain = wide ? (int)(((long)B * t->N + BM - 1) / BM) : (B + SPW - 1) / SPW;
    const int ntiles = (nchain * BM + WBM - 1) / WBM;
    const int nsl = (t->Cp + cols - 1) / cols;
    int groups = 1;
    const int wgs = nsl * t->nblocks;
    while (wgs * groups < 128 && (ntiles + groups - 1) / groups > 64) ++groups;
    if (groups < (32 + wgs - 1) / wgs) groups = (32 + wgs - 1) / wgs;
    groups = m2m_env_int("M2M_WGRAD_GROUPS", groups);
    if (ntiles > 64) groups = m2m_env_int("M2M_WGRAD_LONG_GROUPS", groups);
    if (honour_overwrite && (t->wgrad_flags & M2M_WGRAD_OVERWRITE)) groups = 1;
    if (groups < 1) groups = 1;
    int tpg = (ntiles + groups - 1) / groups;
    if (tpg < 4) tpg = 4;
    if (tpg > ntiles) tpg = ntiles;
    groups = (ntiles + tpg - 1) / tpg;
    WgradPlan pl;
    pl.ntiles = ntiles; pl.nsl = nsl; pl.groups = groups; pl.tpg = tpg; pl.slot = 0;
    pl.rpt = wide ? BM : SPW * t->N;
    return pl;
}
static int wgrad_cols(const m2m_tower* t, int B) {
    if (m2m_wgrad_recompute(t, B)) return RcGeom<128>::COLS;
    if (t->prec == PREC_BF16 && t->D == 128) return WgradGeom<PREC_BF16, 128>::COLS;
    return t->prec == PREC_BF16 && t->D < 128 ? WG_WAVES * 32 : WG_WAVES * 16;
}
extern "C" int m2m_wgrad_groups(const m2m_tower* t, int B) {
    if (!t || t->nblocks < 1) return 1;
    return wgrad_plan(t, B, wgrad_cols(t, B), false).groups;
}

template <int P, int D, int RCDM>
static int launch_wgrad(const m2m_tower* t, int B, unsigned int seed, unsigned int step, const unsigned int* step_dev, hipStream_t st) {
    typedef WgradKernelGeom<P, D, RCDM> KG;
    const WgradPlan pl = wgrad_plan(t, B, KG::COLS);
    const size_t lds = (size_t)KG::LDS_B;
    return m2m_launch<tower_wgrad_kernel<P, D, RCDM>>(dim3(pl.nsl, t->nblocks, pl.groups), dim3(KG::THREADS), lds, lds, st, *t, pl.ntiles, pl.tpg, 0,
                                                      pl.rpt, seed, step, step_dev, 0);
}

static void wgrad_group_plans(const m2m_tower* const* host, int n, int B, int cols, WgradPlan* pl) {
    int min_tpg = 1 << 30;
    WgradPlan nat[WG_MAX_TOWERS];
    for (int i = 0; i < n; ++i) {
        pl[i] = wgrad_plan(host[i], B, cols);
        nat[i] = wgrad_plan(host[i], B, cols, false);
        if (nat[i].tpg < min_tpg) min_tpg = nat[i].tpg;
    }
    for (int i = 0; i < n; ++i) {
        if (n < 2 || !wgrad_slot_usable(host[i])) continue;
        if (nat[i].groups == 2) { pl[i] = nat[i]; pl[i].slot = 1; }
        else if (nat[i].groups == 1 && nat[i].tpg >= 2 * min_tpg && nat[i].tpg >= 32) { pl[i] = nat[i]; pl[i].groups = 2; pl[i].tpg = (pl[i].ntiles + 1) / 2; pl[i].slot = 1; }
    }
}

template <int P, int D, int RCDM>
static int launch_wgrad_group(const m2m_tower* const* host, const m2m_tower* const* dev, int n, const m2m_embed* const* embeds,
                              const float* const* inputs, const float* const* d_x0s, const m2m_tower* const* embed_towers,
                              int nembeds, int B, unsigned int seed, unsigned int step, const unsigned int* step_dev, hipStream_t st,
                              const SplitReduceTower* heads_reduce = nullptr, unsigned int* bump_counter = nullptr) {
    typedef WgradKernelGeom<P, D, RCDM> KG;
    WgradGroupArgs a;
    memset(&a, 0, sizeof(a));
    int njobs = 0, total = 0;
    int order[WG_MAX_TOWERS];
    WgradPlan pl[WG_MAX_TOWERS];
    wgrad_group_plans(host, n, B, KG::COLS, pl);
    for (int i = 0; i < n; ++i) order[i] = i;
    for (int i = 0; i < n; ++i)
        for (int j = i + 1; j < n; ++j)
            if (pl[order[j]].tpg > pl[order[i]].tpg) { const int t = order[i]; order[i] = order[j]; order[j] = t; }
    for (int k = 0; k < n; ++k) {
        const int i = order[k];
        a.tw[i] = dev[i];
        a.ntiles[i] = pl[i].ntiles; a.tpg[i] = pl[i].tpg; a.groups[i] = pl[i].groups; a.nsl[i] = pl[i].nsl; a.slot[i] = pl[i].slot;
        a.rpt[i] = pl[i].rpt;
        for (int b = 0; b < host[i]->nblocks; ++b) {
            if (njobs >= WG_MAX_JOBS) { m2m_set_error("towers_wgrad: more than 32 (tower, block) jobs", __FILE__, __LINE__); return -1; }
            a.job_tower[njobs] = (unsigned char)i;
            a.job_block[njobs] = (unsigned char)b;
            a.job_start[njobs] = (short)total;
            total += pl[i].nsl * pl[i].groups;
            ++njobs;
        }
    }
    if (njobs == 0 && nembeds == 0) return 0;
    if (total > 32000) { m2m_set_error("towers_wgrad: too many workgroups for one launch", __FILE__, __LINE__); return -1; }
    a.job_start[njobs] = (short)total;
    int max_len = 0;
    for (int x = 0, at = 0; x < 8; ++x) {
        const int len = total / 8 + (x < total % 8 ? 1 : 0);
        a.xcd_start[x] = (short)at; a.xcd_len[x] = (short)len;
        at += len;
        if (len > max_len) max_len = len;
    }
    a.njobs = njobs; a.n_tower_wgs = 8 * max_len;
    a.seed = seed; a.step_host = step; a.step_dev = step_dev;
    a.bump_counter = bump_counter;
    a.dma = 0;
    EmbedWgradGroupArgs ea;
    memset(&ea, 0, sizeof(ea));
    int n_embed_wgs = 0;
    size_t lds_e = 0;
    bool embeds_separately = false;
    if (nembeds) {
        n_embed_wgs = (P == PREC_BF16 && nembeds == EMB_GROUP) ? embed_wgrad_group_args_fast(ea, embeds, inputs, embed_towers, B) : 0;
        if (n_embed_wgs) lds_e = embed_wgrad_fast_lds<D, KG::THREADS>();
        else if (KG::THREADS == 256) { static const int ewgs = m2m_env_int("M2M_EMBED_WGS", D >= 256 ? 128 : 512);    n_embed_wgs = embed_wgrad_group_args(ea, embeds, inputs, d_x0s, B, ewgs, nembeds); lds_e = embed_wgrad_lds<D, P>(); }
        else embeds_separately = true;
    }
    if (embeds_separately) {
        if (nembeds == 1) { if (int rc = m2m_embed_wgrad(embeds[0], inputs[0], d_x0s[0], B, (void*)st)) return rc; }
        else if (int rc = m2m_embeds_wgrad(embeds, inputs, d_x0s, nembeds, B, (void*)st)) return rc;
    }
    if constexpr (P == PREC_BF16) {
        static const int merged = m2m_env_int("M2M_EMBED_MERGED", 1);
        if (n_embed_wgs && ea.fast && !merged && KG::THREADS != 256) {
            const size_t le = embed_wgrad_fast_lds<D, 256>();
            if (int rc = m2m_launch<embed_wgrad_fast_group_kernel<D>>(dim3((unsigned)n_embed_wgs), dim3(256), le, le, st, ea)) return rc;
            n_embed_wgs = 0; lds_e = 0;
        }
    }
    const size_t lds_t = (size_t)KG::LDS_B;
    const size_t lds = lds_t > lds_e ? lds_t : lds_e;
    static const int embed_first = m2m_env_int("M2M_EMBED_FIRST", 1);
    if (ea.fast && n_embed_wgs && embed_first) { a.n_embed_first = n_embed_wgs; a.n_embed_pad = (n_embed_wgs + 7) & ~7; n_embed_wgs = 0; }
    SplitReduceArgs ra;
    memset(&ra, 0, sizeof(ra));
    for (int i = 0; i < n; ++i) {
        if (!(host[i]->wgrad_flags & M2M_WGRAD_REDUCES_SMALL)) continue;
        SplitReduceTower x;
        if (!m2m_small_part_deferred(x, host[i], B)) continue;
        if (ra.ntow < SPR_MAX_TOWERS && KG::THREADS % SPR_COLS == 0) { ra.t[ra.ntow++] = x; continue; }
        SplitReduceArgs one;
        memset(&one, 0, sizeof(one));
        one.t[0] = x; one.ntow = 1;
        if (int rc = m2m_split_small_grads(one, st)) return rc;
    }
    if (heads_reduce) {
        if (ra.ntow < SPR_MAX_TOWERS && KG::THREADS % SPR_COLS == 0) ra.t[ra.ntow++] = *heads_reduce;
        else {
            SplitReduceArgs one;
            memset(&one, 0, sizeof(one));
            one.t[0] = *heads_reduce; one.ntow = 1;
            if (int rc = m2m_split_small_grads(one, st)) return rc;
        }
    }
    for (int i = 0; i < ra.ntow; ++i) a.reduce_sets = ra.t[i].nlaunch > a.reduce_sets ? ra.t[i].nlaunch : a.reduce_sets;
    a.n_reduce = SPR_NBX * a.reduce_sets * ra.ntow;
    return m2m_launch<tower_wgrad_group_kernel<P, D, RCDM>>(dim3((unsigned)(a.n_embed_pad + a.n_tower_wgs + n_embed_wgs + a.n_reduce)), dim3(KG::THREADS),
                                                            lds, lds, st, a, ea, ra);
}

extern "C" int m2m_wgrad_slot_groups(const m2m_tower* const* towers, int ntowers, int B) {
    if (!towers || ntowers < 1 || ntowers > WG_MAX_TOWERS) return 0;
    WgradPlan pl[WG_MAX_TOWERS];
    wgrad_group_plans(towers, ntowers, B, wgrad_cols(towers[0], B), pl);
    int bits = 0;
    for (int i = 0; i < ntowers; ++i) bits |= pl[i].slot << i;
    return bits;
}

extern "C" int m2m_tower_wgrad(const m2m_tower* t, int B, uint32_t seed, uint32_t step, const uint32_t* step_dev, void* stream) {
    if (int rc = m2m_check_tower(t, B)) return rc;
    if (t->nblocks == 0) return 0;
    hipStream_t st = reinterpret_cast<hipStream_t>(stream);
    if (t->wgrad_flags & M2M_WGRAD_REDUCES_SMALL) {
        SplitReduceArgs one;
        memset(&one, 0, sizeof(one));
        if (m2m_small_part_deferred(one.t[0], t, B)) {
            one.ntow = 1;
            if (int rc = m2m_split_small_grads(one, st)) return rc;
        }
    }
    if (m2m_wgrad_recompute(t, B))
        return m2m_dispatch<DM_NONE, DM_HALF>(m2m_drop_mode(1, t->p_drop), -1, [&](auto DM) { return launch_wgrad<PREC_BF16, 128, DM()>(t, B, seed, step, step_dev, st); });
    const int rc = m2m_dispatch_pd(m2m_wide_dims{}, t->prec, t->D, [&](auto P, auto D) { return launch_wgrad<P(), D(), -1>(t, B, seed, step, step_dev, st); });
    if (rc != M2M_NO_BUILD) return rc;
    m2m_set_error("tower_wgrad: unsupported (prec, D)", __FILE__, __LINE__);
    return -1;
}

static int towers_wgrad_impl(const m2m_tower* const* towers, const m2m_tower* const* dev_towers, int ntowers,
                             const m2m_embed* const* embeds, const float* const* inputs, const float* const* d_x0s,
                             const m2m_tower* const* embed_towers, int nembeds,
                             int B, uint32_t seed, uint32_t step, const uint32_t* step_dev,
                             const m2m_head* heads, int nheads, int K, void* stream, uint32_t* bump_counter = nullptr) {
    SplitReduceTower hr;
    const SplitReduceTower* heads_reduce = nullptr;
    if (heads && nheads > 0) {
        if (nheads > 3 || K < 2 || !towers || ntowers < 1 || !towers[0]) { m2m_set_error("towers_wgrad_heads: 1..3 heads, K >= 2", __FILE__, __LINE__); return -1; }
        const int D = towers[0]->D, tiles = m2m_heads_part_tiles(B);
        if ((long)K * D + K + 2 > SPP_STRIDE) { m2m_set_error("towers_wgrad_heads: K*D + K + 2 exceeds the slot", __FILE__, __LINE__); return -1; }
        memset(&hr, 0, sizeof(hr));
        for (int h = 0; h < nheads; ++h) {
            if (!heads[h].g_part || !heads[h].g_w || !heads[h].g_b || heads[h].g_part != heads[0].g_part + (long)h * tiles * SPP_STRIDE) {
                m2m_set_error("towers_wgrad_heads: every head needs g_w, g_b and consecutive g_part buffers", __FILE__, __LINE__);
                return -1;
            }
            hr.g_hw[h] = heads[h].g_w; hr.g_hb[h] = heads[h].g_b;
        }
        hr.part = heads[0].g_part; hr.ntiles = tiles; hr.nlaunch = nheads; hr.D = D; hr.head_set0 = 0; hr.nheads = nheads; hr.K = K;
        hr.losses = nullptr;
        heads_reduce = &hr;
    }
    if (!towers || !dev_towers || ntowers < 1 || ntowers > WG_MAX_TOWERS) { m2m_set_error("towers_wgrad: 1..4 towers", __FILE__, __LINE__); return -1; }
    if (nembeds != 0 && (nembeds < 1 || nembeds > EMB_GROUP || !embeds || !inputs || !d_x0s)) {
        m2m_set_error("towers_wgrad: at most two patch embeddings", __FILE__, __LINE__);
        return -1;
    }
    for (int i = 0; i < ntowers; ++i) {
        if (int rc = m2m_check_tower(towers[i], B)) return rc;
        if (!dev_towers[i]) { m2m_set_error("towers_wgrad: missing device-resident descriptor", __FILE__, __LINE__); return -1; }
        if (towers[i]->prec != towers[0]->prec || towers[i]->D != towers[0]->D) {
            m2m_set_error("towers_wgrad: the towers of one launch must share precision and hidden_dim", __FILE__, __LINE__);
            return -1;
        }
        if (m2m_wgrad_recompute(towers[i], B) != m2m_wgrad_recompute(towers[0], B) ||
            (m2m_wgrad_recompute(towers[0], B) && m2m_drop_mode(1, towers[i]->p_drop) != m2m_drop_mode(1, towers[0]->p_drop))) {
            m2m_set_error("towers_wgrad: the towers of one launch must share the weight-gradient form and the dropout mode", __FILE__, __LINE__);
            return -1;
        }
    }
    for (int i = 0; i < nembeds; ++i) {
        if (int rc = m2m_check_embed(embeds[i], B)) return rc;
        if (!inputs[i] || !d_x0s[i]) { m2m_set_error("towers_wgrad: null embedding input", __FILE__, __LINE__); return -1; }
        if (embeds[i]->prec != towers[0]->prec || embeds[i]->D != towers[0]->D) {
            m2m_set_error("towers_wgrad: embeddings must share the towers' precision and hidden_dim", __FILE__, __LINE__);
            return -1;
        }
    }
    hipStream_t st = reinterpret_cast<hipStream_t>(stream);
    const m2m_tower* t = towers[0];
    if (bump_counter && m2m_wgrad_recompute(t, B)) {
        m2m_set_error("towers_wgrad_tail: the recompute form READS the dropout counter in this launch; advance it with m2m_counter_add", __FILE__, __LINE__);
        return -1;
    }
    if (m2m_wgrad_recompute(t, B))
        return m2m_dispatch<DM_NONE, DM_HALF>(m2m_drop_mode(1, t->p_drop), -1, [&](auto DM) {
            return launch_wgrad_group<PREC_BF16, 128, DM()>(towers, dev_towers, ntowers, embeds, inputs, d_x0s, embed_towers, nembeds, B, seed, step, step_dev, st, heads_reduce);
        });
    const int rc = m2m_dispatch_pd(m2m_wide_dims{}, t->prec, t->D, [&](auto P, auto D) {
        return launch_wgrad_group<P(), D(), -1>(towers, dev_towers, ntowers, embeds, inputs, d_x0s, embed_towers, nembeds, B, seed, step, step_dev, st, heads_reduce, bump_counter);
    });
    if (rc != M2M_NO_BUILD) return rc;
    m2m_set_error("towers_wgrad: unsupported (prec, D)", __FILE__, __LINE__);
    return -1;
}

extern "C" int m2m_towers_wgrad(const m2m_tower* const* towers, const m2m_tower* const* dev_towers, int ntowers,
                                const m2m_embed* const* embeds, const float* const* inputs, const float* const* d_x0s,
                                const m2m_tower* const* embed_towers, int nembeds,
                                int B, uint32_t seed, uint32_t step, const uint32_t* step_dev, void* stream) {
    return towers_wgrad_impl(towers, dev_towers, ntowers, embeds, inputs, d_x0s, embed_towers, nembeds, B, seed, step, step_dev, nullptr, 0, 0, stream);
}
extern "C" int m2m_towers_wgrad_heads(const m2m_tower* const* towers, const m2m_tower* const* dev_towers, int ntowers,
                                      const m2m_embed* const* embeds, const float* const* inputs, const float* const* d_x0s,
                                      const m2m_tower* const* embed_towers, int nembeds,
                                      int B, uint32_t seed, uint32_t step, const uint32_t* step_dev,
                                      const m2m_head* heads, int nheads, int K, void* stream) {
    return towers_wgrad_impl(towers, dev_towers, ntowers, embeds, inputs, d_x0s, embed_towers, nembeds, B, seed, step, step_dev, heads, nheads, K, stream);
}

extern "C" int m2m_towers_wgrad_tail(const m2m_tower* const* towers, const m2m_tower* const* dev_towers, int ntowers,
                                     const m2m_embed* const* embeds, const float* const* inputs, const float* const* d_x0s,
                                     const m2m_tower* const* embed_towers, int nembeds,
                                     int B, uint32_t seed, uint32_t step, const uint32_t* step_dev,
                                     const m2m_head* heads, int nheads, int K, uint32_t* bump_counter, void* stream) {
    return towers_wgrad_impl(towers, dev_towers, ntowers, embeds, inputs, d_x0s, embed_towers, nembeds, B, seed, step, step_dev, heads, nheads, K, stream, bump_counter);
}

extern "C" int m2m_embeds_wgrad_form(const m2m_embed* const* embeds, const m2m_tower* const* embed_towers, int nembeds, int B) {
    if (!embeds || !embed_towers || nembeds != EMB_GROUP) return 0;
    EmbedWgradGroupArgs ea;
    const float* ins[EMB_GROUP] = {nullptr, nullptr};
    return embed_wgrad_group_args_fast(ea, embeds, ins, embed_towers, B) > 0 ? 1 : 0;
}

__global__ void wgrad_fold_kernel(float* __restrict__ g, const float* __restrict__ s, long n) {
    const long stride = (long)gridDim.x * blockDim.x;
    for (long i = (long)blockIdx.x * blockDim.x + threadIdx.x; i < n; i += stride) g[i] += s[i];
}
extern "C" int m2m_wgrad_fold(const m2m_tower* t, void* stream) {
    if (!t) { m2m_set_error("wgrad_fold: null tower", __FILE__, __LINE__); return -1; }
    if (!wgrad_slot_usable(t)) { m2m_set_error("wgrad_fold: channel gradients are not contiguous", __FILE__, __LINE__); return -1; }
    hipStream_t st = reinterpret_cast<hipStream_t>(stream);
    const long n = 2L * t->C * t->D + t->C;
    for (int b = 0; b < t->nblocks; ++b) {
        if (int rc = m2m_launch<wgrad_fold_kernel>(dim3(512), dim3(256), 0, 0, st, t->blk[b].g_ch_w1, t->wslot[b], n)) return rc;
    }
    return 0;
}
#endif
```

m2_mixer_amd/engine.py:

```python
from __future__ import annotations

from collections import OrderedDict
from typing import Dict, List, Optional, Sequence, Tuple

import ctypes as C

import torch

from . import _lib as L
from . import config
from .runtime import (AdamPackPlan, BLOCK_FIELDS, BLOCK_KEYS, EmbedRuntime, MlpRuntime, TowerRuntime, block_param_shapes, heads_bce,
                      heads_ce, heads_edl, can_group, can_group_embeds, can_pack_all, embeds_forward, pack_all,
                      towers_backward, towers_forward, towers_forward_embeds_ok, towers_wgrad, wgrad_slot_groups,
                      _embed_ptrs, _grad_ranges, _tower_ptrs)


def config_fused_update(n_params: int = 0) -> bool:
    env = config.switch("M2M_FUSED_UPDATE")
    if env is not None:
        return env == "1"
    return n_params > 0


def _num_patch(c: dict) -> int:
# ... 160 lines not shown
            raise RuntimeError(f"RankBuffer.add: needs contiguous device tensors logits float32 ({nh}, B, {self.K}) and labels "
                               f"int64 (B), got {tuple(logits.shape)} {logits.dtype} and {tuple(labels.shape)} {labels.dtype}")
        L.check(L.lib().m2m_rank_append(logits.data_ptr(), labels.data_ptr(), nh, B, self.K, self.probs.data_ptr(),
                                        self.labels.data_ptr(), self.capacity, self.state.data_ptr(), L.stream_ptr()), "rank_append")

    def reset(self):
        self.state.zero_()

    def rows(self) -> int:
        return int(self.state[0].item()) & 0xFFFFFFFF

    def counts(self) -> Tuple[torch.Tensor, torch.Tensor]:
        st = self.state.cpu().numpy().view("uint32")
        n = int(st[0])
        if n > self.capacity:
            raise RuntimeError(f"RankBuffer: overflow: capacity {self.capacity} rows, {n} rows seen since the last reset "
                               "(rank_capacity= sets the capacity)")
        self.skipped = int(st[2])
        nh = len(self.head_names)
        out = torch.zeros(nh, n, 4, dtype=torch.int32, device=self.state.device)
        if n:
            L.check(L.lib().m2m_rank_counts(self.probs.data_ptr(), self.labels.data_ptr(), nh, n, self.K, self.capacity,
                                            out.data_ptr(), L.stream_ptr()), "rank_counts")
        return out.cpu().to(torch.int64), self.labels[:n].cpu().to(torch.int64)

    def compute(self, names: Optional[Sequence[str]] = None) -> Dict[str, float]:
        from . import scores as S
        counts, labels = self.counts()
        return S.task_rank_scores(self.task, counts.numpy(), labels.numpy(), self.K, self.head_names, names)


class _FlatEngine:

    SEGMENTS: Tuple[str, ...] = ()

    SCORES_TASK: str = ""

    def __init__(self, cfg: dict, batch_size: int, device, precision, lr, betas, eps, weight_decay, seed, init, share=None,
                 scores: bool = False, rank_scores: bool = False, rank_capacity: int = 65536):
        self.cfg, self.B = cfg, int(batch_size)
        self.device = torch.device(device)
        if self.device.type != "cuda":
            raise RuntimeError(f"{type(self).__name__} runs on the GPU only (MI355X); there is no CPU path")
        L.lib()
        self.prec = config.prec_id(precision)
        self.betas, self.eps, self.weight_decay = betas, eps, weight_decay
        self.p_drop = float(cfg.get("dropout", 0.0))
        self.K = cfg["num_classes"]
        self.shapes = self._param_shapes(cfg)
        n = sum(int(torch.Size(s).numel()) for s in self.shapes.values())
        self.n_params = n
        self._fused_update = config_fused_update(n)
        dev = self.device
        if share is not None:
            if share.n_params != n or list(share.shapes.items()) != list(self.shapes.items()) or share.device != dev:
                raise RuntimeError("share=: the other engine must hold the same model on the same device")
            self.flat_p, self.flat_g, self.flat_m, self.flat_v = share.flat_p, share.flat_g, share.flat_m, share.flat_v
        else:
            self.flat_p = torch.zeros(n, device=dev)
            self.flat_g = torch.zeros(n, device=dev)
            self.flat_m = torch.zeros(n, device=dev)
            self.flat_v = torch.zeros(n, device=dev)
        self.params: Dict[str, torch.Tensor] = OrderedDict()
        self.grads: Dict[str, torch.Tensor] = OrderedDict()
        self.exp_avg: Dict[str, torch.Tensor] = OrderedDict()
        self.exp_avg_sq: Dict[str, torch.Tensor] = OrderedDict()
        bounds: Dict[str, Tuple[int, int]] = {}
        off = 0
        for k, shp in self.shapes.items():
            cnt = int(torch.Size(shp).numel())
            self.params[k] = self.flat_p[off:off + cnt].view(shp)
            self.grads[k] = self.flat_g[off:off + cnt].view(shp)
            self.exp_avg[k] = self.flat_m[off:off + cnt].view(shp)
            self.exp_avg_sq[k] = self.flat_v[off:off + cnt].view(shp)
            seg = self._segment_of(k)
            lo, hi = bounds.get(seg, (off, off))
            if hi != off:
                raise AssertionError(f"segment {seg} is not contiguous in the flat buffer")
            bounds[seg] = (lo, off + cnt)
            off += cnt
        self.segments = bounds
        if share is not None:
            self.adam_state, self.drop_step = share.adam_state, share.drop_step
            self.loss_weights, self._loss_weight_group = share.loss_weights, share._loss_weight_group
        else:
            self.adam_state = torch.tensor([0.0, lr, 0.0, 0.0], device=dev)
            self.drop_step = torch.zeros(1, dtype=torch.int32, device=dev)
            self.loss_weights = torch.tensor(self._head_weight_list(), dtype=torch.float32, device=dev)
            self._loss_weight_group = {"fused_heads": False}
        self.seed = (share.seed if share is not None else seed) & 0xFFFFFFFF
        self.scores: Optional[ScoreTable] = None
        if share is not None:
            self.scores = share.scores
        elif scores:
            self.scores = self.new_score_table()
        self.rank: Optional[RankBuffer] = None
        self.rank_capacity = share.rank_capacity if share is not None else int(rank_capacity)
        if share is not None:
            self.rank = share.rank
        elif rank_scores:
            self.rank = self.new_rank_buffer()
        if init and share is None:
            self.reset_parameters(seed)
        self.logits = torch.zeros(3, self.B, self.K, device=dev)
        self.losses = torch.zeros(4, device=dev)
        self._graph = None
        self._static = None
        self._adam_plans: Dict[tuple, AdamPackPlan] = {}
        self._slot_towers: List[TowerRuntime] = []
        self._ranges_add: list = []
        self._slots_folded = False
        self._towers: List[TowerRuntime] = []
        self._embeds: List[EmbedRuntime] = []
        self._fused_heads = False
        self._eval_only = False
        self._tail_engines: Dict[int, "_FlatEngine"] = {}
        self.s_b = torch.cuda.Stream(device=dev)
        self.s_fus = torch.cuda.Stream(device=dev)
        self.s_emb = torch.cuda.Stream(device=dev)
        self.concurrent = config.switch_on("M2M_CONCURRENT")
        self._build()
        if self._fused_heads:
            self._loss_weight_group["fused_heads"] = True
        self.pack()

    def _make_tower(self, prefix: str, c: dict, N: int, site: int) -> TowerRuntime:
        rt = TowerRuntime(c["hidden_dim"], N, c["token_dim"], c["channel_dim"], c["num_mixers"], True, self.p_drop,
                          self.prec, site)
        nb = c["num_mixers"]
        blocks = [{f: self.params[f"{prefix}mixer_blocks.{i}.{BLOCK_KEYS[f]}"] for f in BLOCK_FIELDS} for i in range(nb)]
        rt.bind_params(blocks, (self.params[prefix + "layer_norm.weight"], self.params[prefix + "layer_norm.bias"]))
        rt.bind_grad_tensors([{f: self.grads[f"{prefix}mixer_blocks.{i}.{BLOCK_KEYS[f]}"] for f in BLOCK_FIELDS}
                              for i in range(nb)],
                             (self.grads[prefix + "layer_norm.weight"], self.grads[prefix + "layer_norm.bias"]))
        rt.ensure_buffers(self.B)
        rt.ensure_workspace(self.B)
        return rt

    def _setup_wgrad(self, launches: Sequence[Sequence[TowerRuntime]]):
        self._slot_towers, self._ranges_add = [], []
        if not config.switch_on("M2M_WGRAD_OVERWRITE"):
            return
        cand = []
        for towers in launches:
            bits = 0
            if len(towers) > 1 and config.switch_on("M2M_WGRAD_SLOT"):
                have = [t.alloc_wslot(self.flat_g) for t in towers]
                bits = wgrad_slot_groups(towers, self.B) if all(have) else 0
            cand += [(t, bool(bits >> i & 1)) for i, t in enumerate(towers)]
        table = []
        cand.sort(key=lambda c: not c[1])
        for t, slot in cand:
            if not slot:
                t.clear_wslot()
            rng = t.channel_grad_ranges(self.flat_g)
            fits = rng is not None and len(table) + len(rng) <= L.MAX_GRAD_RANGES
            if slot and not fits:
                raise RuntimeError("more slot ranges than m2m_adam_step_ranges takes")
            if not fits or (t.wgrad_groups(self.B) != 1 and not slot):
                continue
            t.set_wgrad_overwrite(True)
            views = t.wslot_views() if slot else [None] * len(rng)
            if slot:
                self._slot_towers.append(t)
            table += [(lo, n, v, 1) for (lo, n), v in zip(rng, views)]
        self._ranges_add = sorted(table, key=lambda r: r[0])

    @property
    def _ranges_keep(self) -> list:
        return [(lo, n, None, k) for lo, n, _, k in self._ranges_add]

    def _head(self, name: str, pooled, d_pooled, weight: float, with_grad: bool) -> dict:
        key = "classifier_fusion.classifer." if name == "fusion" else f"classifier_{name}."
        P, Gr = self.params, self.grads
        return dict(pooled=pooled, w=P[key + "weight"], b=P[key + "bias"], g_w=Gr[key + "weight"], g_b=Gr[key + "bias"],
                    d_pooled=d_pooled if with_grad else None, weight=weight)

    def _streams(self, concurrent: Optional[bool] = None):
        main = torch.cuda.current_stream()
        conc = self.concurrent if concurrent is None else (concurrent and self.concurrent)
        return main, (self.s_b if conc else main), (self.s_fus if conc else main)

    def reset_parameters(self, seed: int = 42):
        gen = torch.Generator().manual_seed(seed)
        for k, shp in self.shapes.items():
            if _is_layer_norm(k):
                v = torch.ones(shp) if k.endswith("weight") else torch.zeros(shp)
            else:
                wshape = self.shapes[k[:-4] + "weight"] if k.endswith("bias") else shp
                fan_in = int(torch.Size(wshape[1:]).numel())
                bound = 1.0 / fan_in ** 0.5
                v = (torch.rand(shp, generator=gen) * 2 - 1) * bound
            self.params[k].copy_(v)

    EXTRA_STATE_KEYS: Tuple[str, ...] = ()

    def _consume_extra_state(self, key: str, value: torch.Tensor):
        raise KeyError(key)

    def load_state_dict(self, sd: Dict[str, torch.Tensor]):
        missing = [k for k in self.shapes if k not in sd]
        extra = [k for k in sd if k not in self.shapes and k not in self.EXTRA_STATE_KEYS]
        if missing or extra:
            raise KeyError(f"state dict mismatch: missing {missing[:4]}, unexpected {extra[:4]}")
        for k in self.shapes:
            self.params[k].copy_(sd[k].to(self.device, torch.float32).reshape(self.shapes[k]))
        for k in self.EXTRA_STATE_KEYS:
            if k in sd:
                self._consume_extra_state(k, sd[k])
        self.pack()

    def _extra_state(self) -> "OrderedDict[str, torch.Tensor]":
        return OrderedDict()

    def state_dict(self) -> "OrderedDict[str, torch.Tensor]":
        out = OrderedDict((k, v.detach().clone()) for k, v in self.params.items())
        out.update(self._extra_state())
        return out

    def optimizer_state_dict(self) -> dict:
        step = float(self.adam_state[0])
        state = {i: {"step": torch.tensor(step), "exp_avg": self.exp_avg[k].detach().cpu().clone(),
                     "exp_avg_sq": self.exp_avg_sq[k].detach().cpu().clone()} for i, k in enumerate(self.shapes)}
        group = {"lr": float(self.adam_state[1]), "betas": tuple(self.betas), "eps": self.eps, "weight_decay": self.weight_decay,
                 "amsgrad": False, "maximize": False, "params": list(range(len(self.shapes)))}
        return {"state": state, "param_groups": [group]}

    def load_optimizer_state_dict(self, osd: dict):
        keys = list(self.shapes)
        state = osd.get("state", {})
        bad = [i for i in state if not isinstance(i, int) or i < 0 or i >= len(keys)]
        if bad:
            raise KeyError(f"optimizer state: entries {bad[:4]} do not index this model's {len(keys)} parameters")
        steps = {float(st["step"]) for st in state.values() if "step" in st}
        if len(steps) > 1:
            raise RuntimeError("optimizer state: the fused Adam keeps ONE step count for all parameters")
        for i, k in enumerate(keys):
            st = state.get(i)
            if st is None or "exp_avg" not in st:
                self.exp_avg[k].zero_()
                self.exp_avg_sq[k].zero_()
                continue
            self.exp_avg[k].copy_(st["exp_avg"].to(self.device, torch.float32).reshape(self.shapes[k]))
            self.exp_avg_sq[k].copy_(st["exp_avg_sq"].to(self.device, torch.float32).reshape(self.shapes[k]))
        self.adam_state[0] = steps.pop() if steps else 0.0
        if osd.get("param_groups"):
            self.set_lr(float(osd["param_groups"][0]["lr"]))

    def set_lr(self, lr: float):
        self.adam_state[1] = lr

    HEAD_NAMES: Tuple[str, str, str] = ("a", "b", "fusion")

    def _head_weight_list(self) -> List[float]:
        return [float(self.head_weights[n]) for n in self.HEAD_NAMES]

    def set_loss_weights(self, *weights: float):
        if len(weights) != len(self.HEAD_NAMES):
            raise ValueError(f"set_loss_weights: {len(self.HEAD_NAMES)} coefficients ({', '.join(self.HEAD_NAMES)})")
        if self._loss_weight_group["fused_heads"]:
            raise RuntimeError("set_loss_weights: the fused heads + fusion backward launch (M2M_FUSED_HEADS=1) takes the loss "
                               "weights by value; a changing loss weight needs that switch off")
        vals = [float(w) for w in weights]
        self.loss_weights.copy_(torch.tensor(vals, dtype=torch.float32))
        self.head_weights = dict(zip(self.HEAD_NAMES, vals))

    def set_fusion_loss_weight(self, w: float):
        raise NotImplementedError(f"{type(self).__name__}: its loss has no fusion_loss_weight")

    def _sibling_kwargs(self) -> dict:
        return {"fusion_loss_weight": self.fusion_loss_weight} if hasattr(self, "fusion_loss_weight") else {}

    def sibling(self, batch_size: int, trains: bool = True):
        prec = {v: k for k, v in L.PREC_BY_NAME.items() if k in ("bf16", "fp32")}[self.prec]
        sib = type(self)(self.cfg, batch_size, device=self.device, precision=prec, lr=float(self.adam_state[1]),
                         betas=self.betas, eps=self.eps, weight_decay=self.weight_decay, seed=self.seed, init=False,
                         share=self, **self._sibling_kwargs())
        if hasattr(self, "pos_weight"):
            sib.pos_weight.copy_(self.pos_weight)
        if not trains:
            sib._eval_only = True
            return sib
        mine, theirs = {r[0] for r in self._ranges_add}, {r[0] for r in sib._ranges_add}
        narrowed = [lo for lo, n, v, k in self._ranges_add if k and lo not in theirs]
        if narrowed and self._graph is not None:
            raise RuntimeError(f"sibling({batch_size}): this engine's captured graph keeps {len(narrowed)} gradient range(s) uncleared "
                               "that the sibling's backward would not overwrite; build training siblings before capture() "
                               "(or capture again afterwards)")
        for eng, other in ((self, theirs), (sib, mine)):
            eng._ranges_add = [(lo, n, v, int(k and lo in other)) for lo, n, v, k in eng._ranges_add]
        return sib

    def _check_grad_bf16(self, grad_bf16: Optional[torch.Tensor]):
        if grad_bf16 is not None and (grad_bf16.dtype != torch.bfloat16 or grad_bf16.numel() != self.n_params or not grad_bf16.is_cuda):
            raise RuntimeError("grad_bf16 must be a bf16 device copy of the whole flat gradient")

    def _adam(self, lo: int, hi: int, scale: float, grad_bf16: Optional[torch.Tensor] = None, ranges=None):
        self._check_grad_bf16(grad_bf16)
        n = hi - lo
        p, g, m, v = (t.data_ptr() + lo * 4 for t in (self.flat_p, self.flat_g, self.flat_m, self.flat_v))
        g16 = 0 if grad_bf16 is None else grad_bf16.data_ptr() + lo * 2
        tail = (self.adam_state.data_ptr(), self.betas[0], self.betas[1], self.eps, self.weight_decay, -abs(scale), 0)
        if ranges:
            L.check(L.lib().m2m_adam_step_ranges(p, g, g16, m, v, n, *tail, _grad_ranges(ranges), len(ranges), L.stream_ptr()),
                    "adam_step_ranges")
        elif grad_bf16 is None:
            L.check(L.lib().m2m_adam_step(p, g, m, v, n, *tail, L.stream_ptr()), "adam_step")
        else:
            L.check(L.lib().m2m_adam_step_bf16(p, g, g16, m, v, n, *tail, L.stream_ptr()), "adam_step_bf16")

    def _prologue(self):
        L.check(L.lib().m2m_step_prologue(self.adam_state.data_ptr(), self.drop_step.data_ptr(), self.losses.data_ptr(), 4,
                                          L.stream_ptr()), "step_prologue")

    def forward_backward(self, *batch):
        self._step(batch, fused_update=False)
        for t in self._slot_towers:
            t.wgrad_fold()
        self._slots_folded = True

    def fused_step(self, *batch):
        self._step(batch, fused_update=True)
        return self.losses

    def _step(self, batch, fused_update: bool):
        self._check_trains()
        self._slots_folded = False
        self._forward(*batch, training=True, with_grad=True, prologue=True)
        self._score_forward(batch[-1])
        self._backward(*batch[:-1], fused_update=fused_update)
        self._score_backward(batch[-1])

    def new_score_table(self) -> ScoreTable:
        return ScoreTable(self.SCORES_TASK, self.HEAD_NAMES, self.K, self.device)

    def score_table(self, split: str) -> ScoreTable:
        if split == "train":
            if self.scores is None:
                raise RuntimeError("score_table('train'): this engine was built with scores=False")
            return self.scores
        tables = self.__dict__.setdefault("_split_scores", {})
        if split not in tables:
            tables[split] = self.new_score_table()
        return tables[split]

# ... 160 lines not shown
                for i in range(steps):
                    self.losses, self.logits, self.preds = self.losses_steps[i], self.logits_steps[i], self.preds_steps[i]
                    self.fused_step(*slots[i])

            first = all_steps
        nupd = {"none": 0, "single": 1, "pipelined": len(self._update_chunks())}[_exchange_mode(grad_sync)]
        graphs = (graph_of(first), *[graph_of(lambda k=k: update(k, scale)) for k in range(nupd)])
        if steps > 1:
            self.losses, self.logits, self.preds = home
        self._slots_folded = False
        self._graph = graphs

        def replay(*new_batch):
            if new_batch and new_batch[0] is not None:
                if len(new_batch) != nb * steps:
                    raise ValueError(f"replay expects {nb * steps} tensors ({steps} step(s) x {nb}), got {len(new_batch)}")
                for i in range(steps):
                    for dst, src in zip(slots[i], new_batch[i * nb:(i + 1) * nb]):
                        dst.copy_(src, non_blocking=True)
            self._run_step(grad_sync, graphs[0].replay, lambda k, scale: graphs[1 + k].replay())
            return out_losses

        replay.losses = out_losses
        return replay


class _TwoTowerEngine(_FlatEngine):

    MODS: Tuple[str, str] = ("image", "audio")

    def _param_shapes(self, cfg):
        return two_tower_param_shapes(cfg, self.MODS)

    def _segment_of(self, k: str) -> str:
        a, b = self.MODS
        return a if k.startswith(f"{a}_mixer.") else (b if k.startswith(f"{b}_mixer.") else "fusion")

    def _build(self):
        a, b = self.MODS
        cfg = self.cfg
        ca, cb, cm = cfg[a], cfg[b], cfg["multimodal"]
        self.D = ca["hidden_dim"]
        self.fusion_name = fusion_function_name(cm)
        self.concat = self.fusion_name == "ConcatFusion"
        if not (cb["hidden_dim"] == self.D == cm["hidden_dim"]):
            raise RuntimeError(f"both towers and the fusion mixer must share hidden_dim ({self.fusion_name} on dim 1)")
        if self.fusion_name == "BiModalGatedUnit" and not (cm["mod1_in"] == cm["mod2_in"] == cm["out_size"] == self.D):
            raise RuntimeError(f"multimodal.mod1_in / mod2_in / out_size = {cm['mod1_in']} / {cm['mod2_in']} / {cm['out_size']}: "
                               f"the engine's BiModalGatedUnit takes and gives the towers' hidden_dim {self.D} (one D for the heads)")
        self.Na, self.Nb = _num_patch(ca), _num_patch(cb)
        self.Nf = fusion_tokens(cm, self.Na, self.Nb)
        self.t_a = self._make_tower(f"{a}_mixer.", ca, self.Na, 0)
        self.t_b = self._make_tower(f"{b}_mixer.", cb, self.Nb, 1024)
        self.t_fus = self._make_tower("fusion_mixer.", cm, self.Nf, 2048)

        def make_embed(prefix, c):
            e = EmbedRuntime(c["in_channels"], c["image_size"][0], c["image_size"][1], c["patch_size"], c["patch_size"],
                             self.D, self.prec)
            e.bind_params(self.params[prefix + "to_patch_embedding.0.weight"], self.params[prefix + "to_patch_embedding.0.bias"])
            e.bind_grads(self.grads[prefix + "to_patch_embedding.0.weight"], self.grads[prefix + "to_patch_embedding.0.bias"])
            return e

        self.e_a = make_embed(f"{a}_mixer.", ca)
        self.e_b = make_embed(f"{b}_mixer.", cb)
        self._towers, self._embeds = [self.t_a, self.t_b, self.t_fus], [self.e_a, self.e_b]
        B, D, dev = self.B, self.D, self.device
        f = lambda *s: torch.zeros(*s, device=dev)
        grouped = can_group_embeds(self.e_a, self.e_b) and can_group(self.t_a, self.t_b, self.B)
        self.x0_splits = (self.e_a.fwd_splits(), self.e_b.fwd_splits()) if grouped and not self.t_a.wide else (1, 1)
        self._x0_a, self._x0_b = f(self.x0_splits[0], B * self.Na, D), f(self.x0_splits[1], B * self.Nb, D)
        self.x0_a, self.x0_b = self._x0_a[0], self._x0_b[0]
        self.fused, self.fus_out = f(B, self.Nf, D), f(B, self.Nf, D)
        self.pool_a, self.pool_b, self.pool_fus = f(B, D), f(B, D), f(B, D)
        self.dpool_a, self.dpool_b, self.dpool_fus = f(B, D), f(B, D), f(B, D)
        self.d_fused = f(B, self.Nf, D)
        self.dx0_a, self.dx0_b = f(B * self.Na, D), f(B * self.Nb, D)
        self._build_fusion()
        self.preds = torch.zeros(self._preds_shape(), dtype=torch.int32, device=dev)
        self._early_fus_wgrad = (self.concurrent and self.t_fus.wide and B * self.Nf <= 8192 and
                                 config.switch_on("M2M_EARLY_FUSION_WGRAD"))
        self._setup_wgrad([[self.t_fus], [self.t_a, self.t_b]] if self._early_fus_wgrad else [[self.t_fus, self.t_a, self.t_b]])
        self._fused_heads = self._heads_are_ce() and self.t_fus.backward_heads_ok(B, 3, self.K)
        self._heads_pool = (self.t_a.wide and self.t_b.wide and self.t_fus.wide and config.switch_on("M2M_HEADS_POOL"))
        self.t_fus.set_wgrad_reduces_small(not self._fused_heads and config.switch_on("M2M_DEFER_SMALL"))
        self._head_part, self._wgrad_heads = None, None
        if (self._heads_write_slots() and not self._fused_heads and config.switch_on("M2M_HEAD_SLOTS")
                and self.K * D + self.K + 2 <= L.SPLIT_GPART):
            self._head_part = torch.zeros(3, int(L.lib().m2m_heads_part_tiles(B)), L.SPLIT_GPART, device=dev)
        if (config.switch_on("M2M_GROUP_SLOTS") and self.t_a.has_small_slots() and self.t_b.has_small_slots()
                and can_group(self.t_a, self.t_b, self.B)):
            for t in (self.t_a, self.t_b):
                t.set_wgrad_group_slots(True)
                t.set_wgrad_reduces_small(True)
        self._embed_towers = []
        if config.switch_on("M2M_EMBED_FAST") and self.t_a.enable_dx0_image(B) and self.t_b.enable_dx0_image(B):
            self._embed_towers = [self.t_a, self.t_b]
            fast = bool(L.lib().m2m_embeds_wgrad_form(_embed_ptrs(self._embeds), _tower_ptrs(self._embed_towers), 2, B))
            if fast and config.switch_on("M2M_WGRAD_OVERWRITE") and len(self._ranges_add) + 2 <= L.MAX_GRAD_RANGES:
                for e, pre in ((self.e_a, f"{a}_mixer."), (self.e_b, f"{b}_mixer.")):
                    gw = self.grads[pre + "to_patch_embedding.0.weight"]
                    e.set_wgrad_overwrite(True)
                    self._ranges_add.append(((gw.data_ptr() - self.flat_g.data_ptr()) // 4, gw.numel(), None, 1))
                self._ranges_add.sort(key=lambda r: r[0])

        self._embed_fold = (config.switch_on("M2M_EMBED_FOLD") and grouped and self.concurrent and not self._early_fus_wgrad
                            and self.x0_splits is not None and self.e_a.prec == self.t_a.prec and self.e_a.D == self.t_a.D
                            and towers_forward_embeds_ok([self.t_a, self.t_b], [self.e_a, self.e_b], B)
                            and self.t_a.wgrad_form(B) == 0 and self.t_fus.wgrad_form(B) == 0)
        self._pending_bump = False

    def _build_fusion(self):
        B, D, dev = self.B, self.D, self.device
        self.out_a = self.out_b = self.d_out_a = self.d_out_b = None
        self.gate = None
        if self.concat:
            return
        f = lambda *s: torch.zeros(*s, device=dev)
        self.out_a, self.out_b = f(B, self.Na, D), f(B, self.Nb, D)
        if self.fusion_name == "SumFusion":
            self.d_out_a = self.d_out_b = self.d_fused
        else:
            self.d_out_a, self.d_out_b = f(B, self.Na, D), f(B, self.Nb, D)
        if self.fusion_name != "BiModalGatedUnit":
            return
        rows = B * self.Nf
        self._gate_bufs = dict(t1=f(rows, D), t2=f(rows, D), z=f(rows, D), dh=f(rows, 3 * D),
                               part=f(int(L.lib().m2m_gate_part_floats(rows, D))))
        g = L.Gate()
        g.D = D
        P, G = self.params, self.grads
        for fld, key in (("w1", "mod1_hidden.weight"), ("b1", "mod1_hidden.bias"), ("w2", "mod2_hidden.weight"),
                         ("b2", "mod2_hidden.bias"), ("wz", "z_hidden.weight"), ("bz", "z_hidden.bias")):
            setattr(g, fld, P["fusion_function." + key].data_ptr())
            setattr(g, "g_" + fld, G["fusion_function." + key].data_ptr())
        for fld, t in self._gate_bufs.items():
            setattr(g, fld, t.data_ptr())
        self.gate = g

    def _tower_outputs(self):
        D = self.D
        if self.concat:
            return self.fused, self.fused.view(-1)[self.Na * D:], self.Nf * D
        return self.out_a, self.out_b, None

    def _fusion_forward(self, training: bool):
        rows = self.B * self.Nf
        if self.concat:
            return
        if self.gate is not None:
            L.check(L.lib().m2m_gate_forward(C.byref(self.gate), self.out_a.data_ptr(), self.out_b.data_ptr(), self.fused.data_ptr(),
                                             rows, int(training), L.stream_ptr()), "gate_forward")
        else:
            L.check(L.lib().m2m_fusion_forward(_ELEM_FUSION_MODE[self.fusion_name], self.out_a.data_ptr(), self.out_b.data_ptr(),
                                               self.fused.data_ptr(), rows * self.D, L.stream_ptr()), "fusion_forward")

    def _fusion_backward(self):
        rows = self.B * self.Nf
        if self.concat or self.fusion_name == "SumFusion":
            return
        if self.gate is not None:
            L.check(L.lib().m2m_gate_backward(C.byref(self.gate), self.d_fused.data_ptr(), self.d_out_a.data_ptr(),
                                              self.d_out_b.data_ptr(), rows, L.stream_ptr()), "gate_backward")
            L.check(L.lib().m2m_gate_wgrad(C.byref(self.gate), self.out_a.data_ptr(), self.out_b.data_ptr(), rows, L.stream_ptr()),
                    "gate_wgrad")
        else:
            L.check(L.lib().m2m_fusion_backward(_ELEM_FUSION_MODE[self.fusion_name], self.out_a.data_ptr(), self.out_b.data_ptr(),
                                                self.d_fused.data_ptr(), self.d_out_a.data_ptr(), self.d_out_b.data_ptr(),
# ... 2 lines not shown
    def _preds_shape(self):
        return (3, self.B)

    def _loss_heads(self, heads, labels, zero_losses):
        raise NotImplementedError

    def _heads_are_ce(self) -> bool:
        return False

    def _heads_write_slots(self) -> bool:
        return self._heads_are_ce()

    def _forward(self, xa, xb, labels, training: bool, with_grad: bool, prologue: bool = False):
        B, D = self.B, self.D
        sd = self.drop_step if training else None
        fs = self.Nf * D
        out_a, b_part, ts = self._tower_outputs()
        sa_, sb_ = (ts, ts) if self.concat else (self.Na * D, self.Nb * D)
        main, side, _ = self._streams()
        so = 0
        pa, pb, pf = (None, None, None) if self._heads_pool else (self.pool_a, self.pool_b, self.pool_fus)
        self._pending_bump = False
        if self._embed_fold and training and prologue:
            so, self._pending_bump = 1, True
            towers_forward([self.t_a, self.t_b],
                           [(self.x0_a, self.Na * D, out_a, sa_, pa), (self.x0_b, self.Nb * D, b_part, sb_, pb)],
                           B, training, self.seed, so, sd, embeds=[self.e_a, self.e_b], inputs=[xa, xb],
                           head=(self.adam_state, self.losses))
        elif self.concurrent and can_group(self.t_a, self.t_b, self.B):
            sa, sb = self.x0_splits
            if can_group_embeds(self.e_a, self.e_b):
                head = (self.adam_state, self.drop_step, self.losses) if prologue else None
                embeds_forward([self.e_a, self.e_b], [xa, xb], [self._x0_a, self._x0_b], B, [sa, sb], head)
            else:
                if prologue:
                    self._prologue()
                sa = sb = 1
                self.e_a.forward(xa, B, self.x0_a)
                self.e_b.forward(xb, B, self.x0_b)
            towers_forward([self.t_a, self.t_b],
                           [(self.x0_a, self.Na * D, out_a, sa_, pa, sa, B * self.Na * D),
                            (self.x0_b, self.Nb * D, b_part, sb_, pb, sb, B * self.Nb * D)],
                           B, training, self.seed, 0, sd)
        else:
            if prologue:
                self._prologue()
            side.wait_stream(main)
            with torch.cuda.stream(side):
                self.e_b.forward(xb, B, self.x0_b)
                self.t_b.forward(self.x0_b, self.Nb * D, B, b_part, sb_, pb, training, self.seed, 0, sd)
            self.e_a.forward(xa, B, self.x0_a)
            self.t_a.forward(self.x0_a, self.Na * D, B, out_a, sa_, pa, training, self.seed, 0, sd)
            main.wait_stream(side)
        self._fusion_forward(training and with_grad)
        self.t_fus.forward(self.fused, fs, B, self.fus_out, fs, pf, training, self.seed, so, sd)
        a, b = self.MODS
        hw = self.head_weights
        heads = [self._head(a, self.pool_a, self.dpool_a, hw[a], with_grad),
                 self._head(b, self.pool_b, self.dpool_b, hw[b], with_grad),
                 self._head("fusion", self.pool_fus, self.dpool_fus, hw["fusion"], with_grad)]
        if self._heads_pool:
            heads[0]["tokens"] = (out_a, self.Na, sa_)
            heads[1]["tokens"] = (b_part.data_ptr(), self.Nb, sb_)
            heads[2]["tokens"] = (self.fus_out, self.Nf, fs)
        self._wgrad_heads = None
        if training and with_grad and self._head_part is not None:
            for i, h in enumerate(heads):
                h["g_part"] = self._head_part[i]
            self._wgrad_heads = heads
        self._heads = heads
        self._labels = labels
        if training and with_grad and self._fused_heads:
            return
        self._loss_heads(heads, labels, not training)

    def _backward(self, xa, xb, fused_update: bool = False):
        B, D = self.B, self.D
        fs = self.Nf * D
        sd = self.drop_step
        a, b = self.MODS
        so = 1 if self._pending_bump else 0
        if self._fused_heads:
            self.t_fus.backward_heads(B, self._heads, 2, self._labels, self.K, (self.logits, self.losses, self.preds),
                                      self.d_fused, fs, self.seed, so, sd)
        else:
            self.t_fus.backward(B, None, 0, self.dpool_fus, self.d_fused, fs, self.seed, so, sd)
        if self.concat:
            d_a_part, d_b_part, sa_, sb_ = self.d_fused, self.d_fused.view(-1)[self.Na * D:], fs, fs
        else:
            self._fusion_backward()
            d_a_part, d_b_part, sa_, sb_ = self.d_out_a, self.d_out_b, self.Na * D, self.Nb * D
        main, s_a, s_f = self._streams()
        wg_towers = [self.t_fus, self.t_a, self.t_b]
        if self._early_fus_wgrad:
            s_f.wait_stream(main)
            with torch.cuda.stream(s_f):
                self.t_fus.wgrad(B, self.seed, so, sd)
            wg_towers = [self.t_a, self.t_b]
        s_e = self.s_emb if self.concurrent else main
        if self.concurrent and can_group(self.t_a, self.t_b, self.B):
            towers_backward([self.t_a, self.t_b],
                            [(d_a_part, sa_, self.dpool_a, self.dx0_a, self.Na * D), (d_b_part, sb_, self.dpool_b, self.dx0_b, self.Nb * D)],
                            B, self.seed, so, sd)
        else:
            s_a.wait_stream(main)
            with torch.cuda.stream(s_a):
                self.t_a.backward(B, d_a_part, sa_, self.dpool_a, self.dx0_a, self.Na * D, self.seed, so, sd)
            self.t_b.backward(B, d_b_part, sb_, self.dpool_b, self.dx0_b, self.Nb * D, self.seed, so, sd)
            main.wait_stream(s_a)
        bump = self.drop_step if self._pending_bump else None
        if can_group_embeds(self.e_a, self.e_b) and self.e_a.prec == self.t_a.prec and self.e_a.D == self.t_a.D:
            towers_wgrad(wg_towers, B, [self.e_a, self.e_b], [xa, xb], [self.dx0_a, self.dx0_b],
                         seed=self.seed, step=so, step_dev=sd, embed_towers=self._embed_towers, heads=self._wgrad_heads, K=self.K,
                         bump=bump)
        else:
            if bump is not None:
                raise RuntimeError("the embedding fold needs the merged weight-gradient launch (it advances the dropout counter)")
            s_e.wait_stream(main)
            with torch.cuda.stream(s_e):
                self.e_b.wgrad(xb, self.dx0_b, B)
                self.e_a.wgrad(xa, self.dx0_a, B)
            towers_wgrad(wg_towers, B, seed=self.seed, step=so, step_dev=sd, heads=self._wgrad_heads, K=self.K)
            main.wait_stream(s_e)
        self._pending_bump = False
        if self._early_fus_wgrad:
            main.wait_stream(s_f)
        if fused_update:
            self._update(1.0)

    def _update_chunks(self):
        a, b = self.MODS
        mods = {a: [self.t_a, self.e_a], b: [self.t_b, self.e_b], "fusion": [self.t_fus]}
        segs = sorted(self.segments.items(), key=lambda kv: kv[1][0])
        return [(lo, hi, mods[name]) for name, (lo, hi) in segs]

    @torch.no_grad()
    def evaluate(self, xa, xb, labels, scores: Optional[ScoreTable] = None, rank: Optional[RankBuffer] = None):
        self._forward(xa, xb, labels, False, False)
        if scores is not None:
            scores.add(self.preds, labels)
        if rank is not None:
            rank.add(self.logits, labels)
        a, b = self.MODS
        return {"logits": self.logits[2], f"{a}_logits": self.logits[0], f"{b}_logits": self.logits[1],
                f"loss_{a}": self.losses[0], f"loss_{b}": self.losses[1], "loss_fusion": self.losses[2],
                "loss": self.losses[3], "preds": self.preds[2], f"preds_{a}": self.preds[0], f"preds_{b}": self.preds[1]}


class AVMnistEngine(_TwoTowerEngine):

    MODS = ("image", "audio")

    def __init__(self, cfg: dict, batch_size: int, device="cuda:0", precision: Optional[str] = None,
                 lr: float = 1e-2, betas=(0.9, 0.999), eps: float = 1e-8, weight_decay: float = 0.0,
                 fusion_loss_weight: float = 1.0 / 3, seed: int = 42, init: bool = True, share=None, scores: bool = False,
                 rank_scores: bool = False, rank_capacity: int = 65536):
        w = fusion_loss_weight
        ow = (1 - w) / 2
        self.head_weights = {"image": 3 * ow, "audio": 3 * ow, "fusion": 3 * w}
        self.fusion_loss_weight = w
        super().__init__(cfg, batch_size, device, precision, lr, betas, eps, weight_decay, seed, init, share, scores, rank_scores,
                         rank_capacity)

    HEAD_NAMES = ("image", "audio", "fusion")
    SCORES_TASK = "avmnist"

    def set_fusion_loss_weight(self, w: float):
        ow = (1 - w) / 2
        self.set_loss_weights(3 * ow, 3 * ow, 3 * w)
        self.fusion_loss_weight = w

    def _loss_heads(self, heads, labels, zero_losses):
        heads_ce(heads, labels, self.B, self.D, self.K, out=(self.logits, self.losses, self.preds), zero_losses=zero_losses,
                 weights=self.loss_weights)

    def _heads_are_ce(self) -> bool:
        return True

    t_img = property(lambda self: self.t_a)
    t_aud = property(lambda self: self.t_b)
    e_img = property(lambda self: self.e_a)
    e_aud = property(lambda self: self.e_b)
    s_aud = property(lambda self: self.s_b)
    Ni = property(lambda self: self.Na)
    x0_img = property(lambda self: self.x0_a)


class AVMnistUQEngine(AVMnistEngine):

    def __init__(self, cfg: dict, batch_size: int, device="cuda:0", precision: Optional[str] = None,
                 lr: float = 1e-2, betas=(0.9, 0.999), eps: float = 1e-8, weight_decay: float = 0.0,
                 seed: int = 42, init: bool = True, share=None, scores: bool = False,
                 rank_scores: bool = False, rank_capacity: int = 65536):
        if rank_scores:
            raise RuntimeError("AVMnistUQEngine: rank_scores=True: the ranking buffers store the softmax of the logits, which is "
                               "not the evidential model's class probability (alpha / S)")
        self.head_weights = {"image": 1.0, "audio": 1.0, "fusion": 1.0}
        _TwoTowerEngine.__init__(self, cfg, batch_size, device, precision, lr, betas, eps, weight_decay, seed, init, share, scores,
                                 rank_scores, rank_capacity)
        self.uncertainty = torch.zeros(3, self.B, device=self.device)

    def set_fusion_loss_weight(self, w: float):
        raise NotImplementedError("AVMnistUQEngine: its loss has no fusion_loss_weight (models/avmnist.py:511)")

    def _loss_heads(self, heads, labels, zero_losses):
# ... 209 lines not shown
```

m2_mixer_amd/runtime.py:

```python
from __future__ import annotations

import ctypes as C
from typing import Dict, List, Optional, Sequence

import torch

from . import _lib as L

BLOCK_KEYS = {
    "ln1_w": "token_mix.0.weight", "ln1_b": "token_mix.0.bias",
    "tok_w1": "token_mix.2.net.0.weight", "tok_b1": "token_mix.2.net.0.bias",
    "tok_w2": "token_mix.2.net.3.weight", "tok_b2": "token_mix.2.net.3.bias",
    "ln2_w": "channel_mix.0.weight", "ln2_b": "channel_mix.0.bias",
    "ch_w1": "channel_mix.1.net.0.weight", "ch_b1": "channel_mix.1.net.0.bias",
    "ch_w2": "channel_mix.1.net.3.weight", "ch_b2": "channel_mix.1.net.3.bias",
}
BLOCK_FIELDS = list(BLOCK_KEYS.keys())


def block_param_shapes(D: int, N: int, T: int, Cc: int) -> Dict[str, tuple]:
    return {"ln1_w": (D,), "ln1_b": (D,), "tok_w1": (T, N), "tok_b1": (T,), "tok_w2": (N, T), "tok_b2": (N,),
            "ln2_w": (D,), "ln2_b": (D,), "ch_w1": (Cc, D), "ch_b1": (Cc,), "ch_w2": (D, Cc), "ch_b2": (D,)}


def _check_tensor(t: torch.Tensor, shape, name: str):
    if not t.is_cuda:
        raise RuntimeError(f"{name}: m2_mixer_amd runs on the GPU only (got a {t.device} tensor); "
                           "there is no CPU path -- the CPU restatement under oracle/ is test infrastructure")
    if t.dtype != torch.float32 or not t.is_contiguous() or tuple(t.shape) != tuple(shape):
        raise RuntimeError(f"{name}: expected contiguous float32 {tuple(shape)}, got {t.dtype} {tuple(t.shape)}")


def _tower_ptrs(towers):
    return (C.POINTER(L.Tower) * max(len(towers), 1))(*[C.pointer(t.desc) for t in towers])


def _embed_ptrs(embeds):
    return (C.POINTER(L.Embed) * max(len(embeds), 1))(*[C.pointer(e.desc) for e in embeds])


def _data_ptrs(tensors):
    return (C.c_void_p * max(len(tensors), 1))(*[t.data_ptr() for t in tensors])


def _device_descs(towers):
    return (C.c_void_p * max(len(towers), 1))(*[t.device_desc() for t in towers])


def _grad_ranges(ranges):
    arr = (L.GradRange * max(len(ranges), 1))()
    for i, (lo, n, add, keep) in enumerate(ranges):
        arr[i].lo, arr[i].n, arr[i].add, arr[i].keep = lo, n, L.ptr(add), int(keep)
    return arr


def _step_head(adam_state, losses, drop_counter=None):
    return C.byref(L.StepHead(L.ptr(adam_state), L.ptr(drop_counter), L.ptr(losses), int(losses.numel())))


def _drop_tail(seed: int, step: int, step_dev: Optional[torch.Tensor] = None):
    return seed & 0xFFFFFFFF, step & 0xFFFFFFFF, L.ptr(step_dev), L.stream_ptr()


class TowerRuntime:

    def __init__(self, D: int, N: int, T: int, Cc: int, nblocks: int, has_final_ln: bool, p_drop: float,
                 prec: int, site_base: int = 0):
        if nblocks > L.MAX_BLOCKS:
            raise RuntimeError(f"one m2m_tower holds at most {L.MAX_BLOCKS} blocks; deeper towers are a chain of them "
                               "(modules/mixer.py does that; the fused engines take towers of up to 8 blocks)")
        self.D, self.N, self.T, self.C, self.nblocks = D, N, T, Cc, nblocks
        self.Cp = (Cc + 31) // 32 * 32
        self.prec = prec
        self.has_final_ln = bool(has_final_ln)
        self.desc = L.Tower()
        d = self.desc
        d.prec, d.D, d.N, d.T, d.C, d.Cp = prec, D, N, T, Cc, self.Cp
        d.nblocks, d.has_final_ln = nblocks, int(self.has_final_ln)
        d.p_drop = float(p_drop)
        d.site_base = site_base
        self._keep: Dict[str, object] = {}
        self._param_ptrs: List[int] = []
        self._param_versions: List[int] = []
        self._packed_for: Optional[List[int]] = None
        self._bufB = 0
        self._wsB = 0
# ... 179 lines not shown
        L.check(L.lib().m2m_tower_forward(C.byref(self.desc), x0.data_ptr(), x0_ss, B, out.data_ptr(), out_ss,
                                          L.ptr(pooled), int(training), *_drop_tail(seed, step, step_dev)), "tower_forward")

    def backward(self, B: int, d_out: Optional[torch.Tensor], d_out_ss: int, d_pooled: Optional[torch.Tensor],
                 d_x0: torch.Tensor, d_x0_ss: int, seed: int, step: int, step_dev: Optional[torch.Tensor] = None):
        L.check(L.lib().m2m_tower_backward(C.byref(self.desc), B, L.ptr(d_out), d_out_ss, L.ptr(d_pooled),
                                           d_x0.data_ptr(), d_x0_ss, *_drop_tail(seed, step, step_dev)), "tower_backward")

    def enable_dx0_image(self, B: int) -> bool:
        if self.wide or self.prec != L.PREC_BF16 or self.nblocks == 0:
            return False
        self._keep["want_dx0_image"] = True
        self._bufB = 0
        self.ensure_buffers(B)
        return True

    def wgrad_form(self, B: int) -> int:
        return int(L.lib().m2m_wgrad_form(C.byref(self.desc), B))

    def split_form(self, B: int, training: bool = True, other: Optional["TowerRuntime"] = None) -> int:
        return int(L.lib().m2m_split_form(C.byref(self.desc), C.byref(other.desc) if other is not None else None, B, int(training)))

    def wgrad_groups(self, B: int) -> int:
        return int(L.lib().m2m_wgrad_groups(C.byref(self.desc), B))

    def channel_grad_ranges(self, flat_g: torch.Tensor):
        out = []
        cd = self.C * self.D
        base, end = flat_g.data_ptr(), flat_g.data_ptr() + flat_g.numel() * 4
        for i in range(self.nblocks):
            b = self.desc.blk[i]
            w1, b1, w2 = b.g_ch_w1, b.g_ch_b1, b.g_ch_w2
            if not w1 or b1 != w1 + 4 * cd or w2 != b1 + 4 * self.C or w1 < base or w2 + 4 * cd > end:
                return None
            out.append(((w1 - base) // 4, 2 * cd + self.C))
        return out

    def alloc_wslot(self, flat_g: torch.Tensor) -> bool:
        rng = self.channel_grad_ranges(flat_g)
        if rng is None or self.nblocks == 0:
            return False
        n = rng[0][1]
        buf = torch.zeros(self.nblocks * (n + 8), device=self.device)
        views = []
        off = 0
        for i, (lo, _) in enumerate(rng):
            while (off - lo) % 4:
                off += 1
            v = buf[off:off + n]
            self.desc.wslot[i] = v.data_ptr()
            views.append(v)
            off += n
        self._keep["wslot"] = (buf, views)
        return True

    def clear_wslot(self):
        for i in range(L.MAX_BLOCKS):
            self.desc.wslot[i] = None
        self._keep.pop("wslot", None)

    def wslot_views(self):
        return self._keep["wslot"][1] if "wslot" in self._keep else None

    def set_wgrad_overwrite(self, on: bool):
        self.desc.wgrad_flags = (self.desc.wgrad_flags | L.WGRAD_OVERWRITE) if on else (self.desc.wgrad_flags & ~L.WGRAD_OVERWRITE)

    def set_wgrad_reduces_small(self, on: bool):
        self.desc.wgrad_flags = (self.desc.wgrad_flags | L.WGRAD_REDUCES_SMALL) if on else (self.desc.wgrad_flags & ~L.WGRAD_REDUCES_SMALL)

    def has_small_slots(self) -> bool:
        return (not self.wide and self.prec == L.PREC_BF16 and self.D == 128 and self.nblocks > 0
                and 2 * self.T * self.N + self.T + self.N <= 576)

    def set_wgrad_group_slots(self, on: bool):
        self.desc.wgrad_flags = (self.desc.wgrad_flags | L.WGRAD_GROUP_SLOTS) if on else (self.desc.wgrad_flags & ~L.WGRAD_GROUP_SLOTS)

    def wgrad_fold(self):
        L.check(L.lib().m2m_wgrad_fold(C.byref(self.desc), L.stream_ptr()), "wgrad_fold")

    def backward_heads_ok(self, B: int, nheads: int, K: int) -> bool:
        return bool(L.lib().m2m_tower_backward_heads_ok(C.byref(self.desc), B, nheads, K))

    def backward_heads(self, B: int, heads: Sequence[dict], own: int, labels: torch.Tensor, K: int, out, d_x0: torch.Tensor,
                       d_x0_ss: int, seed: int, step: int, step_dev: Optional[torch.Tensor] = None):
        arr = _head_array(heads)
        logits, losses, preds = out
        L.check(L.lib().m2m_tower_backward_heads(C.byref(self.desc), B, arr, len(heads), own, labels.data_ptr(), K, logits.data_ptr(),
                                                 losses.data_ptr(), preds.data_ptr(), d_x0.data_ptr(), d_x0_ss,
                                                 *_drop_tail(seed, step, step_dev)), "tower_backward_heads")

    def wgrad(self, B: int, seed: int, step: int, step_dev: Optional[torch.Tensor] = None):
        L.check(L.lib().m2m_tower_wgrad(C.byref(self.desc), B, *_drop_tail(seed, step, step_dev)), "tower_wgrad")

    def device_desc(self) -> int:
        raw = bytes(self.desc)
        if self._keep.get("desc_bytes") != raw:
            self._keep["desc_dev"] = torch.frombuffer(bytearray(raw), dtype=torch.uint8).to(self.device)
            self._keep["desc_bytes"] = raw
        return self._keep["desc_dev"].data_ptr()

    def dropout_mask(self, blk: int, site: int, B: int, seed: int, step: int) -> torch.Tensor:
        n = {0: B * self.D * self.T, 1: B * self.D * self.N, 2: B * self.N * self.Cp, 3: B * self.N * self.D}[site]
        m = torch.empty(n, dtype=torch.uint8, device=self.device)
        L.check(L.lib().m2m_dropout_mask(C.byref(self.desc), blk, site, B, *_drop_tail(seed, step)[:2], m.data_ptr(), L.stream_ptr()),
                "dropout_mask")
        return m


def can_group(a: TowerRuntime, b: TowerRuntime, B: Optional[int] = None) -> bool:
    if B is not None:
        return bool(L.lib().m2m_towers_can_group(C.byref(a.desc), C.byref(b.desc), B))
    return (not a.wide and not b.wide and a.prec == b.prec and a.D == b.D and a.desc.p_drop == b.desc.p_drop
            and (a.N <= 4) == (b.N <= 4) and (a.T % 16 == 0) == (b.T % 16 == 0) and a.nblocks <= 4 and b.nblocks <= 4)


def towers_forward_embeds_ok(towers: Sequence[TowerRuntime], embeds: Sequence["EmbedRuntime"], B: int) -> bool:
    return bool(L.lib().m2m_towers_forward_embeds_ok(_tower_ptrs(towers), len(towers), _embed_ptrs(embeds), B))


def towers_forward(towers: Sequence[TowerRuntime], ios: Sequence[tuple], B: int, training: bool, seed: int, step: int,
                   step_dev: Optional[torch.Tensor] = None, embeds: Sequence["EmbedRuntime"] = (), inputs: Sequence[torch.Tensor] = (),
                   head: Optional[tuple] = None):
    n = len(towers)
    for t in towers:
        if training:
            t.ensure_buffers(B)
        t.ensure_workspace(B)
    host = _tower_ptrs(towers)
    io = (L.TowerIO * n)()
    for i, (x0, x0_ss, out, out_ss, pooled, *parts) in enumerate(ios):
        io[i].x0, io[i].x0_ss, io[i].out, io[i].out_ss, io[i].pooled = x0.data_ptr(), x0_ss, out.data_ptr(), out_ss, L.ptr(pooled)
        io[i].x0_parts, io[i].x0_part_stride = parts if parts else (1, 0)
    if len(embeds):
        hd = _step_head(*head) if head is not None else None
        L.check(L.lib().m2m_towers_forward_embeds(host, io, n, _embed_ptrs(embeds), _data_ptrs(inputs), hd, B, int(training),
                                                  *_drop_tail(seed, step, step_dev)), "towers_forward_embeds")
        return
    L.check(L.lib().m2m_towers_forward(host, io, n, B, int(training), *_drop_tail(seed, step, step_dev)), "towers_forward")


def towers_backward(towers: Sequence[TowerRuntime], ios: Sequence[tuple], B: int, seed: int, step: int,
                    step_dev: Optional[torch.Tensor] = None):
    n = len(towers)
    io = (L.TowerGIO * n)()
    for i, (d_out, d_out_ss, d_pooled, d_x0, d_x0_ss) in enumerate(ios):
        io[i].d_out, io[i].d_out_ss, io[i].d_pooled = L.ptr(d_out), d_out_ss, L.ptr(d_pooled)
        io[i].d_x0, io[i].d_x0_ss = d_x0.data_ptr(), d_x0_ss
    L.check(L.lib().m2m_towers_backward(_tower_ptrs(towers), io, n, B, *_drop_tail(seed, step, step_dev)), "towers_backward")


def wgrad_slot_groups(towers: Sequence[TowerRuntime], B: int) -> int:
    return int(L.lib().m2m_wgrad_slot_groups(_tower_ptrs(towers), len(towers), B))


def towers_wgrad(towers: Sequence[TowerRuntime], B: int, embeds: Sequence["EmbedRuntime"] = (),
                 inputs: Sequence[torch.Tensor] = (), d_x0s: Sequence[torch.Tensor] = (), seed: int = 0, step: int = 0,
                 step_dev: Optional[torch.Tensor] = None, embed_towers: Sequence[TowerRuntime] = (),
                 heads: Optional[Sequence[dict]] = None, K: int = 0, bump: Optional[torch.Tensor] = None):
    n, ne = len(towers), len(embeds)
    et = _tower_ptrs(embed_towers) if len(embed_towers) == ne and ne else None
    args = (_tower_ptrs(towers), _device_descs(towers), n, _embed_ptrs(embeds), _data_ptrs(inputs), _data_ptrs(d_x0s), et, ne, B,
            *_drop_tail(seed, step, step_dev)[:3])
    if bump is not None:
        L.check(L.lib().m2m_towers_wgrad_tail(*args, _head_array(heads) if heads else None, len(heads) if heads else 0, K,
                                              bump.data_ptr(), L.stream_ptr()), "towers_wgrad_tail")
        return
    if heads:
        L.check(L.lib().m2m_towers_wgrad_heads(*args, _head_array(heads), len(heads), K, L.stream_ptr()), "towers_wgrad_heads")
        return
    L.check(L.lib().m2m_towers_wgrad(*args, L.stream_ptr()), "towers_wgrad")


def can_pack_all(towers: Sequence[TowerRuntime], embeds: Sequence["EmbedRuntime"]) -> bool:
    precs = {t.prec for t in towers} | {e.prec for e in embeds}
    return len(towers) <= 3 and len(embeds) <= 2 and len(precs) == 1 and all(t.nblocks <= 4 for t in towers)


def pack_all(towers: Sequence[TowerRuntime], embeds: Sequence["EmbedRuntime"]):
    L.check(L.lib().m2m_pack_all(_tower_ptrs(towers), len(towers), _embed_ptrs(embeds), len(embeds), L.stream_ptr()), "pack_all")
    for t in towers:
        t.mark_packed()
    for e in embeds:
        e.mark_packed()


class AdamPackPlan:

    def __init__(self, towers: Sequence[TowerRuntime], embeds: Sequence["EmbedRuntime"], flat_p, flat_g, grad_bf16, flat_m, flat_v,
                 state, betas, eps: float, weight_decay: float, grad_scale: float, ranges=None):
        self.towers, self.embeds = list(towers), list(embeds)
        nt, ne = len(towers), len(embeds)
        self._tp, self._ep = _tower_ptrs(towers), _embed_ptrs(embeds)
        nbytes = int(L.lib().m2m_adam_pack_plan_bytes())
        self.host = C.create_string_buffer(nbytes)
        ranges = list(ranges or [])
        L.check(L.lib().m2m_adam_pack_plan_ranges(self._tp, nt, self._ep, ne, flat_p.data_ptr(), flat_g.data_ptr(), L.ptr(grad_bf16),
                                                  flat_m.data_ptr(), flat_v.data_ptr(), flat_p.numel(), state.data_ptr(), betas[0], betas[1],
                                                  eps, weight_decay, abs(grad_scale), _grad_ranges(ranges), len(ranges), self.host),
                "adam_pack_plan_ranges")
        self.dev = torch.frombuffer(bytearray(self.host.raw), dtype=torch.uint8).to(flat_p.device)
        self._keep = (flat_p, flat_g, grad_bf16, flat_m, flat_v, state, [r[2] for r in ranges])

    def run(self):
        L.check(L.lib().m2m_adam_pack_all(self._tp, len(self.towers), self._ep, len(self.embeds), self.dev.data_ptr(), self.host,
                                          L.stream_ptr()), "adam_pack_all")
        for t in self.towers:
            t.mark_packed()
        for e in self.embeds:
            e.mark_packed()


class EmbedRuntime:

    def __init__(self, Cin: int, H: int, W: int, ph: int, pw: int, D: int, prec: int):
        self.desc = L.Embed()
        d = self.desc
        kb = 32 if prec == L.PREC_BF16 else 16
        K = Cin * ph * pw
        d.prec, d.Cin, d.H, d.W, d.ph, d.pw, d.D, d.K = prec, Cin, H, W, ph, pw, D, K
        d.Kp = (K + kb - 1) // kb * kb
        self.N = (H // ph) * (W // pw)
        self.D, self.K, self.prec = D, K, prec
        self._keep = {}
        self._packed_for = None

    def bind_params(self, w: torch.Tensor, b: torch.Tensor):
        if not w.is_cuda:
            raise RuntimeError("patch embedding: m2_mixer_amd runs on the GPU only; there is no CPU path")
        if w.dtype != torch.float32 or not w.is_contiguous() or w.numel() != self.D * self.K:
            raise RuntimeError(f"embedding weight: expected contiguous float32 with {self.D * self.K} elements")
        self.desc.w, self.desc.b = w.data_ptr(), b.data_ptr()
        self._keep["w"], self._keep["b"] = w, b
        self._packed_for = None
        if "wn" not in self._keep:
            wn = torch.zeros(L.packed_bytes(self.prec, self.D, self.desc.Kp), dtype=torch.uint8, device=w.device)
            self.desc.wn = wn.data_ptr()
            self._keep["wn"] = wn

    def params_changed(self, w, b) -> bool:
        return w.data_ptr() != self.desc.w or b.data_ptr() != self.desc.b

    def mark_packed(self):
        self._packed_for = self._keep["w"]._version

    def invalidate(self):
# ... 204 lines not shown
```

Measured before the change: 1.048 million.

## Rework fused heads backward: per-wave head pairs, device loss weights, deferred small reduce

Replaces the block-wide LDS staging of head pooled/weights in the fused heads+fusion backward kernel with a per-wave, register-resident path: each wave loads one (head, sample) pair's pooled row and weights into registers, computes logits by shuffles, and runs a shared cross-entropy helper. Loss weights are now read from a device tensor, so the fused heads path no longer forbids changing loss weights. The small-parameter head gradient reduction moves into the weight-gradient launch through a new wgrad_bwd_heads entry point, which allows deferred small reduces alongside fused heads. This is meant to cut LDS traffic and barriers in the backward kernel and overlap the head work with the token loads, at the cost of more registers and a more complex kernel.

New measurement: 1.046 million. Within noise of the previous version (-0.2%).

```diff
diff --git a/include/m2mixer.h b/include/m2mixer.h
--- a/include/m2mixer.h
+++ b/include/m2mixer.h
@@ -198,6 +198,16 @@
 int m2m_tower_backward_heads(const m2m_tower* t, int B, const m2m_head* heads, int nheads, int own, const int64_t* labels,
                              int K, float* logits, float* losses, int32_t* preds, float* d_x0, int64_t d_x0_sample_stride,
                              uint32_t seed, uint32_t step, const uint32_t* step_dev, void* stream);
+int m2m_tower_backward_heads_w(const m2m_tower* t, int B, const m2m_head* heads, int nheads, int own, const int64_t* labels,
+                               int K, float* logits, float* losses, int32_t* preds, float* d_x0, int64_t d_x0_sample_stride,
+                               uint32_t seed, uint32_t step, const uint32_t* step_dev, const float* weights, void* stream);
+
+int m2m_towers_wgrad_bwd_heads(const m2m_tower* const* towers, const m2m_tower* const* dev_towers, int ntowers,
+                               const m2m_embed* const* embeds, const float* const* inputs, const float* const* d_x0s,
+                               const m2m_tower* const* embed_towers, int nembeds,
+                               int B, uint32_t seed, uint32_t step, const uint32_t* step_dev,
+                               const m2m_head* heads, int nheads, int K, int heads_tower, float* losses,
+                               uint32_t* bump_counter, void* stream);
 
 #define M2M_MLP_MAX_LAYERS 4
 typedef struct m2m_mlp {
diff --git a/m2_mixer_amd/_lib.py b/m2_mixer_amd/_lib.py
--- a/m2_mixer_amd/_lib.py
+++ b/m2_mixer_amd/_lib.py
@@ -114,6 +114,8 @@
     "m2m_tower_backward_heads_ok": (C.c_int, [C.POINTER(Tower), C.c_int, C.c_int, C.c_int]),
     "m2m_tower_backward_heads": (C.c_int, [C.POINTER(Tower), C.c_int, C.POINTER(Head), C.c_int, C.c_int, _fp, C.c_int, _fp, _fp, _fp, _fp,
                                            C.c_int64, C.c_uint32, C.c_uint32, _fp, _fp]),
+    "m2m_tower_backward_heads_w": (C.c_int, [C.POINTER(Tower), C.c_int, C.POINTER(Head), C.c_int, C.c_int, _fp, C.c_int, _fp, _fp, _fp, _fp,
+                                             C.c_int64, C.c_uint32, C.c_uint32, _fp, _fp, _fp]),
     "m2m_tower_wgrad": (C.c_int, [C.POINTER(Tower), C.c_int, C.c_uint32, C.c_uint32, _fp, _fp]),
     "m2m_towers_can_group": (C.c_int, [C.POINTER(Tower), C.POINTER(Tower), C.c_int]),
     "m2m_towers_forward": (C.c_int, [C.POINTER(C.POINTER(Tower)), C.POINTER(TowerIO), C.c_int, C.c_int, C.c_int, C.c_uint32,
@@ -131,6 +133,9 @@
     "m2m_towers_wgrad_tail": (C.c_int, [C.POINTER(C.POINTER(Tower)), C.POINTER(_fp), C.c_int, C.POINTER(C.POINTER(Embed)), C.POINTER(_fp),
                                         C.POINTER(_fp), C.POINTER(C.POINTER(Tower)), C.c_int, C.c_int, C.c_uint32, C.c_uint32, _fp,
                                         C.POINTER(Head), C.c_int, C.c_int, _fp, _fp]),
+    "m2m_towers_wgrad_bwd_heads": (C.c_int, [C.POINTER(C.POINTER(Tower)), C.POINTER(_fp), C.c_int, C.POINTER(C.POINTER(Embed)), C.POINTER(_fp),
+                                             C.POINTER(_fp), C.POINTER(C.POINTER(Tower)), C.c_int, C.c_int, C.c_uint32, C.c_uint32, _fp,
+                                             C.POINTER(Head), C.c_int, C.c_int, C.c_int, _fp, _fp, _fp]),
     "m2m_heads_part_tiles": (C.c_int, [C.c_int]),
     "m2m_wgrad_form": (C.c_int, [C.POINTER(Tower), C.c_int]),
     "m2m_split_form": (C.c_int, [C.POINTER(Tower), C.POINTER(Tower), C.c_int, C.c_int]),
diff --git a/m2_mixer_amd/csrc/heads.hip b/m2_mixer_amd/csrc/heads.hip
--- a/m2_mixer_amd/csrc/heads.hip
+++ b/m2_mixer_amd/csrc/heads.hip
@@ -1,4 +1,5 @@
 #include "dispatch.h"
+#include "heads_dev.h"
 
 #define HEAD_S 16
 #define HEAD_MAXK 32
@@ -119,26 +120,13 @@
     } else if (tid < S * 32) {
         const int sI = tid >> 5, k = tid & 31;
         const bool live = k < K;
-        const float v = live ? lg[sI * HEAD_MAXK + k] : -3.0e38f;
-        float mx = v;
-        int am = live ? k : 0x7fffffff;
-#pragma unroll
-        for (int o = 16; o >= 1; o >>= 1) {
-            const float ov = __shfl_xor(mx, o, 64);
-            const int oa = __shfl_xor(am, o, 64);
-            if (ov > mx || (ov == mx && oa < am)) { mx = ov; am = oa; }
-        }
-        const float ex = live ? __expf(v - mx) : 0.f;
-        float se = ex;
-#pragma unroll
-        for (int o = 16; o >= 1; o >>= 1) se += __shfl_xor(se, o, 64);
         const int y = sI < ns ? (int)labels[s0 + sI] : 0;
-        const float scale = hw / (float)B;
-        const float dl = sI < ns ? scale * (ex * (1.0f / se) - (k == y ? 1.f : 0.f)) : 0.f;
-        const float vy = __shfl(v, (tid & 32) + y, 64);
+        float dl, term;
+        int am;
+        head_ce_lanes32(lg[sI * HEAD_MAXK + k], k, K, y, hw / (float)B, sI < ns, dl, term, am);
         if (live) lg[sI * HEAD_MAXK + k] = dl;
         if (k == 0) {
-            red[sI] = sI < ns ? (__logf(se) + mx) - vy : 0.f;
+            red[sI] = term;
             if (sI < ns) preds[(long)hI * B + s0 + sI] = am;
         }
     }
diff --git a/m2_mixer_amd/csrc/heads_dev.h b/m2_mixer_amd/csrc/heads_dev.h
--- /dev/null
+++ b/m2_mixer_amd/csrc/heads_dev.h
@@ -0,0 +1,33 @@
+#pragma once
+#include "common.h"
+
+static __device__ __forceinline__ float head_dot4(const f32x4_t x, const f32x4_t y, float a) {
+#pragma unroll
+    for (int e = 0; e < 4; ++e) a = __builtin_fmaf(x[e], y[e], a);
+    return a;
+}
+static __device__ __forceinline__ void head_axpy4(float s, const f32x4_t w, f32x4_t& a) {
+#pragma unroll
+    for (int e = 0; e < 4; ++e) a[e] = __builtin_fmaf(s, w[e], a[e]);
+}
+
+static __device__ __forceinline__ void head_ce_lanes32(float logit, int k, int K, int y, float scale, bool valid, float& dl, float& term,
+                                                       int& am) {
+    const bool live = k < K;
+    const float v = live ? logit : -3.0e38f;
+    float mx = v;
+    am = live ? k : 0x7fffffff;
+#pragma unroll
+    for (int o = 16; o >= 1; o >>= 1) {
+        const float ov = __shfl_xor(mx, o, 64);
+        const int oa = __shfl_xor(am, o, 64);
+        if (ov > mx || (ov == mx && oa < am)) { mx = ov; am = oa; }
+    }
+    const float ex = live ? __expf(v - mx) : 0.f;
+    float se = ex;
+#pragma unroll
+    for (int o = 16; o >= 1; o >>= 1) se += __shfl_xor(se, o, 64);
+    dl = valid ? scale * (ex * (1.0f / se) - (k == y ? 1.f : 0.f)) : 0.f;
+    const float vy = __shfl(v, (int)(threadIdx.x & 32) + y, 64);
+    term = valid ? (__logf(se) + mx) - vy : 0.f;
+}
diff --git a/m2_mixer_amd/csrc/host.h b/m2_mixer_amd/csrc/host.h
--- a/m2_mixer_amd/csrc/host.h
+++ b/m2_mixer_amd/csrc/host.h
@@ -17,7 +17,8 @@
                                  const long* out_ss, int training, unsigned int seed, unsigned int step, const unsigned int* step_dev,
                                  hipStream_t st);
 
-bool m2m_small_part_deferred(SplitReduceTower& x, const m2m_tower* t, int B);
+struct m2m_bwd_heads_reduce { const m2m_head* heads; int nheads, K; float* losses; };
+bool m2m_small_part_deferred(SplitReduceTower& x, const m2m_tower* t, int B, const m2m_bwd_heads_reduce* hr = nullptr);
 int m2m_chain_backward_rows(const m2m_tower* t, int B, const float* d_out, long d_out_ss, const float* d_pooled, float* d_x0,
                             long d_x0_ss, unsigned int seed, unsigned int step, const unsigned int* step_dev, hipStream_t st);
 int m2m_chain_backward_rows_group(const m2m_tower* const* v, int B, const float* const* d_out, const long* d_out_ss,
diff --git a/m2_mixer_amd/csrc/tower_bwd.hip b/m2_mixer_amd/csrc/tower_bwd.hip
--- a/m2_mixer_amd/csrc/tower_bwd.hip
+++ b/m2_mixer_amd/csrc/tower_bwd.hip
@@ -1,16 +1,90 @@
 #include "tile.h"
 #include "token_mfma.h"
 #include "dispatch.h"
+#include "heads_dev.h"
 #include <algorithm>
 
 #define BH_MAXH 3
+#define BH_MAXK 16
 struct BwdHeads {
     m2m_head h[BH_MAXH];
     const int64_t* labels;
+    const float* weights;
     float* logits;
     int32_t* preds;
     int nheads, K, own;
 };
+struct BwdHeadRegs { f32x4_t p, w[BH_MAXK / 2]; float bias, coef; int y; };
+template <int D>
+static __device__ __forceinline__ void bwd_head_load(BwdHeadRegs& r, const BwdHeads& hd, int h, long s, bool valid, int lane) {
+    static_assert(D == 128, "a wave's 32-lane halves hold one 128-float row as float4 chunks");
+    const int k = lane & 31, k0 = (lane >> 5) * (BH_MAXK / 2), K = hd.K;
+    const M2M_AS1 float* pl = reinterpret_cast<const M2M_AS1 float*>(to_gptr(hd.h[h].pooled));
+    const M2M_AS1 float* w = reinterpret_cast<const M2M_AS1 float*>(to_gptr(hd.h[h].w));
+    const M2M_AS1 float* b = reinterpret_cast<const M2M_AS1 float*>(to_gptr(hd.h[h].b));
+    const f32x4_t z = f32x4_t{0.f, 0.f, 0.f, 0.f};
+    r.p = z;
+    if (valid) r.p = *reinterpret_cast<const M2M_AS1 f32x4_t*>(pl + s * D + k * 4);
+#pragma unroll
+    for (int i = 0; i < BH_MAXK / 2; ++i) {
+        r.w[i] = z;
+        if (valid && k0 + i < K) r.w[i] = *reinterpret_cast<const M2M_AS1 f32x4_t*>(w + (k0 + i) * D + k * 4);
+    }
+    r.bias = k < K ? b[k] : 0.f;
+    r.y = valid ? (int)hd.labels[s] : 0;
+    r.coef = hd.weights ? hd.weights[h] : hd.h[h].weight;
+}
+template <int D>
+static __device__ __forceinline__ void bwd_head_pair(const BwdHeadRegs& r, const BwdHeads& hd, int h, int pair, int sl, long s, bool valid,
+                                                     int B, int lane, float* hpool, float* hdl, float* hterm, float* hdp) {
+    constexpr int KH = BH_MAXK / 2;
+    const int K = hd.K, k = lane & 31, half = lane >> 5;
+    float acc[KH];
+#pragma unroll
+    for (int i = 0; i < KH; ++i) acc[i] = 0.f;
+#pragma unroll
+    for (int j = 0; j < D / 16; ++j) {
+#pragma unroll
+        for (int i = 0; i < KH; ++i) {
+            const float below = j == 0 ? 0.f : __shfl(acc[i], lane - 4, 64);
+            if ((k >> 2) == j) acc[i] = head_dot4(r.p, r.w[i], below);
+        }
+    }
+    float mine = 0.f;
+#pragma unroll
+    for (int i = 0; i < KH; ++i) {
+        const float lg = wave_sum_xor(acc[i], 4);
+        const float all = __shfl(lg, (lane & 32) + 28, 64);
+        mine = (lane & (KH - 1)) == i ? all : mine;
+    }
+    const float logit = __shfl(mine, ((k / KH) & 1) * 32 + (k & (KH - 1)), 64) + r.bias;
+    float dl, term;
+    int am;
+    head_ce_lanes32(logit, k, K, r.y, r.coef / (float)B, valid, dl, term, am);
+    if (k >= K) dl = 0.f;
+    if (valid && lane < K) hd.logits[((long)h * B + s) * K + k] = logit;
+    if (valid && lane == 0) hd.preds[(long)h * B + s] = am;
+    if (lane < BH_MAXK) hdl[pair * BH_MAXK + lane] = dl;
+    if (lane == 0) hterm[pair] = term / (float)B;
+    if (lane < 32) *reinterpret_cast<f32x4_t*>(hpool + pair * D + k * 4) = r.p;
+    f32x4_t a = f32x4_t{0.f, 0.f, 0.f, 0.f};
+#pragma unroll
+    for (int pass = 0; pass < 2; ++pass) {
+        if (pass == 1) {
+#pragma unroll
+            for (int e = 0; e < 4; ++e) a[e] = __shfl(a[e], lane & 31, 64);
+        }
+#pragma unroll
+        for (int i = 0; i < KH; ++i) {
+            const float dk = __shfl(dl, pass * KH + i, 64);
+            if (half == pass) head_axpy4(dk, r.w[i], a);
+        }
+    }
+    if (valid && lane >= 32) {
+        if (h == hd.own) *reinterpret_cast<f32x4_t*>(hdp + sl * D + k * 4) = a;
+        else *reinterpret_cast<f32x4_t*>(hd.h[h].d_pooled + s * D + k * 4) = a;
+    }
+}
 
 template <int P, int D, int NMAX, int TG> struct BwdLds {
     static constexpr bool TOK = NMAX > 0;
@@ -101,81 +175,21 @@
     TIMER_LSTART();
     if (PART && threadIdx.x <= (unsigned)tw.nblocks + (HEADS ? BH_MAXH : 0))
         slotp[threadIdx.x] = (unsigned long long)(part + ((long)threadIdx.x * nwg + wg) * SPP_STRIDE);
-    float* hdp = slabs + 3 * 4 * D + BH_MAXH * 32 * (D + 1) + BH_MAXH * 4 * 32;
+    float* hpool = slabs;
+    float* hdl = hpool + BH_MAXH * BM * D;
+    float* hterm = hdl + BH_MAXH * BM * BH_MAXK;
+    float* hdp = hterm + BH_MAXH * BM;
+    static_assert(!HEADS || BH_MAXH * BM * (D + BH_MAXK + 1) + BM * D <= NSL * TILE_F, "the heads' LDS lies inside the slabs");
+    BwdHeadRegs hreg;
+    int hpair = 0;
     if constexpr (HEADS && PART && TOK) {
-        const int nh = hd->nheads, K = hd->K, DL = D + 1;
-        float* hpool = slabs;
-        float* hwt = hpool + 3 * 4 * D;
-        float* hlog = hwt + BH_MAXH * 32 * DL;
-        for (int i = tid; i < nh * SPW * D; i += NTHREADS) {
-            const int h = i / (SPW * D), sl = (i / D) % SPW, d = i % D;
-            hpool[(h * 4 + sl) * D + d] = sl < ns ? hd->h[h].pooled[(long)(s0 + sl) * D + d] : 0.f;
-        }
-        for (int i = tid; i < nh * K * D; i += NTHREADS) {
-            const int h = i / (K * D), k = (i / D) % K, d = i % D;
-            hwt[(h * 32 + k) * DL + d] = hd->h[h].w[k * D + d];
-        }
-        __syncthreads();
-        for (int i = tid >> 3; i < nh * SPW * K; i += NTHREADS / 8) {
-            const int h = i / (SPW * K), sl = (i / K) % SPW, k = i % K, part8 = tid & 7;
-            float a = 0.f;
-            for (int d = part8; d < D; d += 8) a = __builtin_fmaf(hpool[(h * 4 + sl) * D + d], hwt[(h * 32 + k) * DL + d], a);
-            a = wave_sum_xor(a, 8) + hd->h[h].b[k];
-            if (part8 == 0) {
-                hlog[(h * 4 + sl) * 32 + k] = a;
-                if (sl < ns) hd->logits[((long)h * B + s0 + sl) * K + k] = a;
-            }
-        }
-        __syncthreads();
-        float term = 0.f;
-        if (tid < nh * SPW) {
-            const int h = tid / SPW, sl = tid % SPW;
-            float* lg = hlog + (h * 4 + sl) * 32;
-            if (sl < ns) {
-                const int y = (int)hd->labels[s0 + sl];
-                float mx = lg[0];
-                int am = 0;
-                for (int k = 1; k < K; ++k) { const float v = lg[k]; if (v > mx) { mx = v; am = k; } }
-                float se = 0.f;
-                for (int k = 0; k < K; ++k) se += __expf(lg[k] - mx);
-                term = (__logf(se) + mx - lg[y]) / (float)B;
-                const float scale = hd->h[h].weight / (float)B, inv = 1.0f / se;
-                for (int k = 0; k < K; ++k) lg[k] = scale * (__expf(lg[k] - mx) * inv - (k == y ? 1.f : 0.f));
-                hd->preds[(long)h * B + s0 + sl] = am;
-            } else {
-                for (int k = 0; k < K; ++k) lg[k] = 0.f;
-            }
-            hlog[BH_MAXH * 4 * 32 - 16 + tid] = term;
-        }
-        __syncthreads();
-        for (int i = tid; i < nh * ns * D; i += NTHREADS) {
-            const int h = i / (ns * D), sl = (i / D) % ns, d = i % D;
-            float a = 0.f;
-            for (int k = 0; k < K; ++k) a = __builtin_fmaf(hlog[(h * 4 + sl) * 32 + k], hwt[(h * 32 + k) * DL + d], a);
-            if (h == hd->own) hdp[sl * D + d] = a;
-            else hd->h[h].d_pooled[(long)(s0 + sl) * D + d] = a;
-        }
-        for (int i = tid; i < nh * (K * D + K + 2); i += NTHREADS) {
-            const int h = i / (K * D + K + 2), e = i % (K * D + K + 2);
-            float* sl_h = reinterpret_cast<float*>(slotp[tw.nblocks + 1 + h]);
-            float a = 0.f;
-            if (e < K * D) {
-                const int k = e / D, d = e % D;
-                for (int sl = 0; sl < SPW; ++sl) a = __builtin_fmaf(hlog[(h * 4 + sl) * 32 + k], hpool[(h * 4 + sl) * D + d], a);
-            } else if (e < K * D + K) {
-                for (int sl = 0; sl < SPW; ++sl) a += hlog[(h * 4 + sl) * 32 + (e - K * D)];
-            } else {
-                for (int sl = 0; sl < SPW; ++sl) a += hlog[BH_MAXH * 4 * 32 - 16 + h * SPW + sl];
-                if (e == K * D + K + 1) a *= hd->h[h].weight;
-            }
-            sl_h[e] = a;
-        }
-        __syncthreads();
+        hpair = __builtin_amdgcn_readfirstlane(wave);
+        if (hpair < hd->nheads * SPW) bwd_head_load<D>(hreg, *hd, hpair / SPW, s0 + hpair % SPW, hpair % SPW < ns, lane);
     }
     constexpr int MAXB = (int)(sizeof(tw.blk) / sizeof(tw.blk[0]));
     constexpr int XI = (BM * (D / 4) + NTHREADS - 1) / NTHREADS, BPT = 8, TI = TOK ? (32 * TW_LD + NTHREADS - 1) / NTHREADS : 1;
     float4 uv[XI];
-    {
+    if constexpr (!(HEADS && PART && TOK)) {
         const float invN = 1.0f / (float)N;
 #pragma unroll
         for (int k = 0; k < XI; ++k) {
@@ -184,10 +198,7 @@
             if (idx < BM * (D / 4) && r < R) {
                 const long gr = row0 + r, gs = gr / N;
                 if (d_out) uv[k] = *reinterpret_cast<const float4*>(d_out + gs * d_out_ss + (gr % N) * D + c);
-                if constexpr (HEADS && PART && TOK) {
-                    const float4 p = *reinterpret_cast<const float4*>(hdp + (gs - s0) * D + c);
-                    uv[k].x += p.x * invN; uv[k].y += p.y * invN; uv[k].z += p.z * invN; uv[k].w += p.w * invN;
-                } else if (d_pooled) {
+                if (d_pooled) {
                     const float4 p = *reinterpret_cast<const float4*>(d_pooled + gs * D + c);
                     uv[k].x += p.x * invN; uv[k].y += p.y * invN; uv[k].z += p.z * invN; uv[k].w += p.w * invN;
                 }
@@ -249,6 +260,50 @@
                     if (tid + k * NTHREADS < 32 * TW_LD) pb[O_TOKW + tid + k * NTHREADS] = tv[k][b];
             }
         }
+    if constexpr (HEADS && PART && TOK) {
+        const int nh = hd->nheads, K = hd->K;
+        for (; hpair < nh * SPW; ) {
+            const int h = hpair / SPW, sl = hpair % SPW;
+            bwd_head_pair<D>(hreg, *hd, h, hpair, sl, s0 + sl, sl < ns, B, lane, hpool, hdl, hterm, hdp);
+            hpair += NWAVES;
+            if (hpair < nh * SPW) bwd_head_load<D>(hreg, *hd, hpair / SPW, s0 + hpair % SPW, hpair % SPW < ns, lane);
+        }
+        __syncthreads();
+        const int k = tid >> 5, c4 = (tid & 31) * 4;
+        static_assert(NTHREADS / 32 == BH_MAXK, "one thread per (class, float4 chunk)");
+#pragma unroll
+        for (int h = 0; h < BH_MAXH; ++h)
+            if (h < nh) {
+                float* sl_h = reinterpret_cast<float*>(slotp[tw.nblocks + 1 + h]);
+                if (k < K) {
+                    f32x4_t a = f32x4_t{0.f, 0.f, 0.f, 0.f};
+#pragma unroll 2
+                    for (int sl = 0; sl < SPW; ++sl)
+                        head_axpy4(hdl[(h * SPW + sl) * BH_MAXK + k], *reinterpret_cast<const f32x4_t*>(hpool + (h * SPW + sl) * D + c4), a);
+                    *reinterpret_cast<f32x4_t*>(sl_h + k * D + c4) = a;
+                }
+                if (tid < K + 2) {
+                    float a = 0.f;
+                    if (tid < K) {
+                        for (int sl = 0; sl < SPW; ++sl) a += hdl[(h * SPW + sl) * BH_MAXK + tid];
+                    } else {
+                        for (int sl = 0; sl < SPW; ++sl) a += hterm[h * SPW + sl];
+                        if (tid == K + 1) a *= hd->weights ? hd->weights[h] : hd->h[h].weight;
+                    }
+                    sl_h[K * D + tid] = a;
+                }
+            }
+        const float invN = 1.0f / (float)N;
+#pragma unroll
+        for (int q = 0; q < XI; ++q) {
+            const int idx = tid + q * NTHREADS, r = idx / (D / 4), c = (idx % (D / 4)) * 4;
+            uv[q] = make_float4(0.f, 0.f, 0.f, 0.f);
+            if (idx < BM * (D / 4) && r < R) {
+                const float4 p = *reinterpret_cast<const float4*>(hdp + (r / N) * D + c);
+                uv[q] = make_float4(p.x * invN, p.y * invN, p.z * invN, p.w * invN);
+            }
+        }
+    }
     {
 #pragma unroll
         for (int k = 0; k < XI; ++k) {
@@ -999,13 +1054,13 @@
     return !off && t->gpart != nullptr && !m2m_is_wide(t) && t->prec == PREC_BF16 && t->D == 128 && t->nblocks >= 1 &&
            2 * t->T * t->N + t->T + t->N <= SPP_TOK_MAX;
 }
-static void m2m_small_part_reduce_args(SplitReduceTower& x, const m2m_tower* t, int nwg, const BwdHeads* hd = nullptr, float* losses = nullptr) {
+static void m2m_small_part_reduce_args(SplitReduceTower& x, const m2m_tower* t, int nwg, const m2m_bwd_heads_reduce* hr = nullptr) {
     memset(&x, 0, sizeof(x));
     x.part = t->gpart; x.ntiles = nwg; x.nlaunch = t->nblocks + 1; x.D = t->D; x.N = t->N; x.T = t->T;
-    if (hd) {
-        x.head_set0 = t->nblocks + 1; x.nheads = hd->nheads; x.K = hd->K; x.losses = losses;
-        for (int h = 0; h < hd->nheads; ++h) { x.g_hw[h] = hd->h[h].g_w; x.g_hb[h] = hd->h[h].g_b; }
-        x.nlaunch += hd->nheads;
+    if (hr) {
+        x.head_set0 = t->nblocks + 1; x.nheads = hr->nheads; x.K = hr->K; x.losses = hr->losses;
+        for (int h = 0; h < hr->nheads; ++h) { x.g_hw[h] = hr->heads[h].g_w; x.g_hb[h] = hr->heads[h].g_b; }
+        x.nlaunch += hr->nheads;
     }
     if (t->has_final_ln) { x.g_lnf_w = t->g_lnf_w; x.g_lnf_b = t->g_lnf_b; }
     for (int b = 0; b < t->nblocks; ++b) {
@@ -1017,10 +1072,10 @@
         x.g_b2[L] = k.g_ch_b2;
     }
 }
-bool m2m_small_part_deferred(SplitReduceTower& x, const m2m_tower* t, int B) {
+bool m2m_small_part_deferred(SplitReduceTower& x, const m2m_tower* t, int B, const m2m_bwd_heads_reduce* hr) {
     if (!t || m2m_is_wide(t) || t->N < 1 || t->N > 8 || !m2m_small_part(t) || m2m_split_eligible(t, B, 1)) return false;
     const int SPW = BM / t->N;
-    m2m_small_part_reduce_args(x, t, (B + SPW - 1) / SPW);
+    m2m_small_part_reduce_args(x, t, (B + SPW - 1) / SPW, hr);
     return true;
 }
 template <int P, int D, int NMAX, int TG, int DM, bool PART = false, bool HREC = false>
@@ -1116,10 +1171,12 @@
                                                                              seed, step, step_dev);
     });
     if (rc) return rc;
+    if (t->wgrad_flags & M2M_WGRAD_REDUCES_SMALL) return 0;
     SplitReduceArgs r;
     memset(&r, 0, sizeof(r));
     r.ntow = 1;
-    m2m_small_part_reduce_args(r.t[0], t, grid, &hd, losses);
+    const m2m_bwd_heads_reduce hr = {hd.h, hd.nheads, hd.K, losses};
+    m2m_small_part_reduce_args(r.t[0], t, grid, &hr);
     return m2m_split_small_grads(r, st);
 }
 
@@ -1229,17 +1286,18 @@
     return -1;
 }
 
+static bool bwd_heads_eligible(const m2m_tower* t, int B, int nheads, int K) {
+    if (!t || m2m_check_tower(t, B) != 0) return false;
+    if (!m2m_small_part(t) || m2m_split_eligible(t, B, 1)) return false;
+    return nheads >= 1 && nheads <= BH_MAXH && K >= 2 && K * t->D + K + 2 <= SPP_STRIDE && K <= BH_MAXK;
+}
 extern "C" int m2m_tower_backward_heads_ok(const m2m_tower* t, int B, int nheads, int K) {
-    if (!t || m2m_check_tower(t, B) != 0) return 0;
-    static const bool on = m2m_env_int("M2M_FUSED_HEADS", 0) == 1;
-    if (!on || !m2m_small_part(t) || m2m_split_eligible(t, B, 1)) return 0;
-    if (nheads < 1 || nheads > BH_MAXH || K < 2 || K * t->D + K + 2 > SPP_STRIDE || K > 16) return 0;
-    return 1;
-}
-extern "C" int m2m_tower_backward_heads(const m2m_tower* t, int B, const m2m_head* heads, int nheads, int own, const int64_t* labels,
-                                        int K, float* logits, float* losses, int32_t* preds, float* d_x0, int64_t d_x0_ss,
-                                        uint32_t seed, uint32_t step, const uint32_t* step_dev, void* stream) {
-    if (!m2m_tower_backward_heads_ok(t, B, nheads, K)) { m2m_set_error("tower_backward_heads: unsupported tower / heads (see m2m_tower_backward_heads_ok)", __FILE__, __LINE__); return -1; }
+    return m2m_env_int("M2M_FUSED_HEADS", 0) == 1 && bwd_heads_eligible(t, B, nheads, K) ? 1 : 0;
+}
+extern "C" int m2m_tower_backward_heads_w(const m2m_tower* t, int B, const m2m_head* heads, int nheads, int own, const int64_t* labels,
+                                          int K, float* logits, float* losses, int32_t* preds, float* d_x0, int64_t d_x0_ss,
+                                          uint32_t seed, uint32_t step, const uint32_t* step_dev, const float* weights, void* stream) {
+    if (!bwd_heads_eligible(t, B, nheads, K)) { m2m_set_error("tower_backward_heads: unsupported tower / heads (see m2m_tower_backward_heads_ok)", __FILE__, __LINE__); return -1; }
     if (!heads || !labels || !logits || !losses || !preds || !d_x0 || own < 0 || own >= nheads) { m2m_set_error("tower_backward_heads: null argument", __FILE__, __LINE__); return -1; }
     if (int rc = bwd_split_mode_init(reinterpret_cast<hipStream_t>(stream))) return rc;
     BwdHeads hd;
@@ -1251,13 +1309,19 @@
             return -1;
         }
     }
-    hd.labels = labels; hd.logits = logits; hd.preds = preds; hd.nheads = nheads; hd.K = K; hd.own = own;
+    hd.labels = labels; hd.weights = weights; hd.logits = logits; hd.preds = preds; hd.nheads = nheads; hd.K = K; hd.own = own;
     hipStream_t st = reinterpret_cast<hipStream_t>(stream);
     return m2m_fused_class(t->N, t->T, [&](auto NMAX, auto TG) {
         return m2m_dispatch_dm(1, t->p_drop, [&](auto DM) {
             return launch_bwd_heads_dm<PREC_BF16, 128, NMAX(), TG(), DM()>(t, B, hd, losses, d_x0, d_x0_ss, seed, step, step_dev, st);
         });
     });
+}
+
+extern "C" int m2m_tower_backward_heads(const m2m_tower* t, int B, const m2m_head* heads, int nheads, int own, const int64_t* labels,
+                                        int K, float* logits, float* losses, int32_t* preds, float* d_x0, int64_t d_x0_ss,
+                                        uint32_t seed, uint32_t step, const uint32_t* step_dev, void* stream) {
+    return m2m_tower_backward_heads_w(t, B, heads, nheads, own, labels, K, logits, losses, preds, d_x0, d_x0_ss, seed, step, step_dev, nullptr, stream);
 }
 
 extern "C" int m2m_tower_backward(const m2m_tower* t, int B, const float* d_out, int64_t d_out_ss, const float* d_pooled,
diff --git a/m2_mixer_amd/csrc/tower_wgrad.hip b/m2_mixer_amd/csrc/tower_wgrad.hip
--- a/m2_mixer_amd/csrc/tower_wgrad.hip
+++ b/m2_mixer_amd/csrc/tower_wgrad.hip
@@ -466,7 +466,8 @@
 static int launch_wgrad_group(const m2m_tower* const* host, const m2m_tower* const* dev, int n, const m2m_embed* const* embeds,
                               const float* const* inputs, const float* const* d_x0s, const m2m_tower* const* embed_towers,
                               int nembeds, int B, unsigned int seed, unsigned int step, const unsigned int* step_dev, hipStream_t st,
-                              const SplitReduceTower* heads_reduce = nullptr, unsigned int* bump_counter = nullptr) {
+                              const SplitReduceTower* heads_reduce = nullptr, unsigned int* bump_counter = nullptr,
+                              const m2m_bwd_heads_reduce* bwd_heads = nullptr, int bwd_heads_tower = -1) {
     typedef WgradKernelGeom<P, D, RCDM> KG;
     WgradGroupArgs a;
     memset(&a, 0, sizeof(a));
@@ -538,7 +539,7 @@
     for (int i = 0; i < n; ++i) {
         if (!(host[i]->wgrad_flags & M2M_WGRAD_REDUCES_SMALL)) continue;
         SplitReduceTower x;
-        if (!m2m_small_part_deferred(x, host[i], B)) continue;
+        if (!m2m_small_part_deferred(x, host[i], B, i == bwd_heads_tower ? bwd_heads : nullptr)) continue;
         if (ra.ntow < SPR_MAX_TOWERS && KG::THREADS % SPR_COLS == 0) { ra.t[ra.ntow++] = x; continue; }
         SplitReduceArgs one;
         memset(&one, 0, sizeof(one));
@@ -593,10 +594,25 @@
                              const m2m_embed* const* embeds, const float* const* inputs, const float* const* d_x0s,
                              const m2m_tower* const* embed_towers, int nembeds,
                              int B, uint32_t seed, uint32_t step, const uint32_t* step_dev,
-                             const m2m_head* heads, int nheads, int K, void* stream, uint32_t* bump_counter = nullptr) {
+                             const m2m_head* heads, int nheads, int K, void* stream, uint32_t* bump_counter = nullptr,
+                             int bwd_heads_tower = -1, float* losses = nullptr) {
     SplitReduceTower hr;
     const SplitReduceTower* heads_reduce = nullptr;
-    if (heads && nheads > 0) {
+    m2m_bwd_heads_reduce bh = {heads, nheads, K, losses};
+    const bool fused_heads = bwd_heads_tower >= 0;
+    if (fused_heads) {
+        if (!heads || nheads < 1 || nheads > 3 || K < 2 || !losses || !towers || bwd_heads_tower >= ntowers || !towers[bwd_heads_tower]) {
+            m2m_set_error("towers_wgrad_bwd_heads: 1..3 heads, K >= 2, losses and the index of the tower whose backward computed them", __FILE__, __LINE__);
+            return -1;
+        }
+        SplitReduceTower probe;
+        if (!(towers[bwd_heads_tower]->wgrad_flags & M2M_WGRAD_REDUCES_SMALL) || !m2m_small_part_deferred(probe, towers[bwd_heads_tower], B, &bh)) {
+            m2m_set_error("towers_wgrad_bwd_heads: the heads' tower needs M2M_WGRAD_REDUCES_SMALL and the slot form of its backward", __FILE__, __LINE__);
+            return -1;
+        }
+        for (int h = 0; h < nheads; ++h)
+            if (!heads[h].g_w || !heads[h].g_b || heads[h].g_part) { m2m_set_error("towers_wgrad_bwd_heads: every head needs g_w and g_b, and no g_part", __FILE__, __LINE__); return -1; }
+    } else if (heads && nheads > 0) {
         if (nheads > 3 || K < 2 || !towers || ntowers < 1 || !towers[0]) { m2m_set_error("towers_wgrad_heads: 1..3 heads, K >= 2", __FILE__, __LINE__); return -1; }
         const int D = towers[0]->D, tiles = m2m_heads_part_tiles(B);
         if ((long)K * D + K + 2 > SPP_STRIDE) { m2m_set_error("towers_wgrad_heads: K*D + K + 2 exceeds the slot", __FILE__, __LINE__); return -1; }
@@ -646,10 +662,12 @@
     }
     if (m2m_wgrad_recompute(t, B))
         return m2m_dispatch<DM_NONE, DM_HALF>(m2m_drop_mode(1, t->p_drop), -1, [&](auto DM) {
-            return launch_wgrad_group<PREC_BF16, 128, DM()>(towers, dev_towers, ntowers, embeds, inputs, d_x0s, embed_towers, nembeds, B, seed, step, step_dev, st, heads_reduce);
+            return launch_wgrad_group<PREC_BF16, 128, DM()>(towers, dev_towers, ntowers, embeds, inputs, d_x0s, embed_towers, nembeds, B, seed, step, step_dev, st, heads_reduce,
+                                                            nullptr, fused_heads ? &bh : nullptr, bwd_heads_tower);
         });
     const int rc = m2m_dispatch_pd(m2m_wide_dims{}, t->prec, t->D, [&](auto P, auto D) {
-        return launch_wgrad_group<P(), D(), -1>(towers, dev_towers, ntowers, embeds, inputs, d_x0s, embed_towers, nembeds, B, seed, step, step_dev, st, heads_reduce, bump_counter);
+        return launch_wgrad_group<P(), D(), -1>(towers, dev_towers, ntowers, embeds, inputs, d_x0s, embed_towers, nembeds, B, seed, step, step_dev, st, heads_reduce, bump_counter,
+                                                fused_heads ? &bh : nullptr, bwd_heads_tower);
     });
     if (rc != M2M_NO_BUILD) return rc;
     m2m_set_error("towers_wgrad: unsupported (prec, D)", __FILE__, __LINE__);
@@ -676,6 +694,17 @@
                                      int B, uint32_t seed, uint32_t step, const uint32_t* step_dev,
                                      const m2m_head* heads, int nheads, int K, uint32_t* bump_counter, void* stream) {
     return towers_wgrad_impl(towers, dev_towers, ntowers, embeds, inputs, d_x0s, embed_towers, nembeds, B, seed, step, step_dev, heads, nheads, K, stream, bump_counter);
+}
+
+extern "C" int m2m_towers_wgrad_bwd_heads(const m2m_tower* const* towers, const m2m_tower* const* dev_towers, int ntowers,
+                                          const m2m_embed* const* embeds, const float* const* inputs, const float* const* d_x0s,
+                                          const m2m_tower* const* embed_towers, int nembeds,
+                                          int B, uint32_t seed, uint32_t step, const uint32_t* step_dev,
+                                          const m2m_head* heads, int nheads, int K, int heads_tower, float* losses,
+                                          uint32_t* bump_counter, void* stream) {
+    if (heads_tower < 0) { m2m_set_error("towers_wgrad_bwd_heads: heads_tower < 0", __FILE__, __LINE__); return -1; }
+    return towers_wgrad_impl(towers, dev_towers, ntowers, embeds, inputs, d_x0s, embed_towers, nembeds, B, seed, step, step_dev, heads, nheads, K, stream, bump_counter,
+                             heads_tower, losses);
 }
 
 extern "C" int m2m_embeds_wgrad_form(const m2m_embed* const* embeds, const m2m_tower* const* embed_towers, int nembeds, int B) {
diff --git a/m2_mixer_amd/engine.py b/m2_mixer_amd/engine.py
--- a/m2_mixer_amd/engine.py
+++ b/m2_mixer_amd/engine.py
@@ -266,12 +266,11 @@
         self.segments = bounds
         if share is not None:
             self.adam_state, self.drop_step = share.adam_state, share.drop_step
-            self.loss_weights, self._loss_weight_group = share.loss_weights, share._loss_weight_group
+            self.loss_weights = share.loss_weights
         else:
             self.adam_state = torch.tensor([0.0, lr, 0.0, 0.0], device=dev)
             self.drop_step = torch.zeros(1, dtype=torch.int32, device=dev)
             self.loss_weights = torch.tensor(self._head_weight_list(), dtype=torch.float32, device=dev)
-            self._loss_weight_group = {"fused_heads": False}
         self.seed = (share.seed if share is not None else seed) & 0xFFFFFFFF
         self.scores: Optional[ScoreTable] = None
         if share is not None:
@@ -304,8 +303,6 @@
         self.s_emb = torch.cuda.Stream(device=dev)
         self.concurrent = config.switch_on("M2M_CONCURRENT")
         self._build()
-        if self._fused_heads:
-            self._loss_weight_group["fused_heads"] = True
         self.pack()
 
     def _make_tower(self, prefix: str, c: dict, N: int, site: int) -> TowerRuntime:
@@ -442,9 +439,6 @@
     def set_loss_weights(self, *weights: float):
         if len(weights) != len(self.HEAD_NAMES):
             raise ValueError(f"set_loss_weights: {len(self.HEAD_NAMES)} coefficients ({', '.join(self.HEAD_NAMES)})")
-        if self._loss_weight_group["fused_heads"]:
-            raise RuntimeError("set_loss_weights: the fused heads + fusion backward launch (M2M_FUSED_HEADS=1) takes the loss "
-                               "weights by value; a changing loss weight needs that switch off")
         vals = [float(w) for w in weights]
         self.loss_weights.copy_(torch.tensor(vals, dtype=torch.float32))
         self.head_weights = dict(zip(self.HEAD_NAMES, vals))
@@ -771,7 +765,7 @@
         self._setup_wgrad([[self.t_fus], [self.t_a, self.t_b]] if self._early_fus_wgrad else [[self.t_fus, self.t_a, self.t_b]])
         self._fused_heads = self._heads_are_ce() and self.t_fus.backward_heads_ok(B, 3, self.K)
         self._heads_pool = (self.t_a.wide and self.t_b.wide and self.t_fus.wide and config.switch_on("M2M_HEADS_POOL"))
-        self.t_fus.set_wgrad_reduces_small(not self._fused_heads and config.switch_on("M2M_DEFER_SMALL"))
+        self.t_fus.set_wgrad_reduces_small(config.switch_on("M2M_DEFER_SMALL"))
         self._head_part, self._wgrad_heads = None, None
         if (self._heads_write_slots() and not self._fused_heads and config.switch_on("M2M_HEAD_SLOTS")
                 and self.K * D + self.K + 2 <= L.SPLIT_GPART):
@@ -940,7 +934,7 @@
         so = 1 if self._pending_bump else 0
         if self._fused_heads:
             self.t_fus.backward_heads(B, self._heads, 2, self._labels, self.K, (self.logits, self.losses, self.preds),
-                                      self.d_fused, fs, self.seed, so, sd)
+                                      self.d_fused, fs, self.seed, so, sd, weights=self.loss_weights)
         else:
             self.t_fus.backward(B, None, 0, self.dpool_fus, self.d_fused, fs, self.seed, so, sd)
         if self.concat:
@@ -967,10 +961,12 @@
             self.t_b.backward(B, d_b_part, sb_, self.dpool_b, self.dx0_b, self.Nb * D, self.seed, so, sd)
             main.wait_stream(s_a)
         bump = self.drop_step if self._pending_bump else None
+        hk = dict(heads=self._wgrad_heads, K=self.K)
+        if self._fused_heads and self.t_fus.desc.wgrad_flags & L.WGRAD_REDUCES_SMALL:
+            hk = dict(heads=self._heads, K=self.K, bwd_heads=(0, self.losses))
         if can_group_embeds(self.e_a, self.e_b) and self.e_a.prec == self.t_a.prec and self.e_a.D == self.t_a.D:
             towers_wgrad(wg_towers, B, [self.e_a, self.e_b], [xa, xb], [self.dx0_a, self.dx0_b],
-                         seed=self.seed, step=so, step_dev=sd, embed_towers=self._embed_towers, heads=self._wgrad_heads, K=self.K,
-                         bump=bump)
+                         seed=self.seed, step=so, step_dev=sd, embed_towers=self._embed_towers, bump=bump, **hk)
         else:
             if bump is not None:
                 raise RuntimeError("the embedding fold needs the merged weight-gradient launch (it advances the dropout counter)")
@@ -978,7 +974,7 @@
             with torch.cuda.stream(s_e):
                 self.e_b.wgrad(xb, self.dx0_b, B)
                 self.e_a.wgrad(xa, self.dx0_a, B)
-            towers_wgrad(wg_towers, B, seed=self.seed, step=so, step_dev=sd, heads=self._wgrad_heads, K=self.K)
+            towers_wgrad(wg_towers, B, seed=self.seed, step=so, step_dev=sd, **hk)
             main.wait_stream(s_e)
         self._pending_bump = False
         if self._early_fus_wgrad:
diff --git a/m2_mixer_amd/runtime.py b/m2_mixer_amd/runtime.py
--- a/m2_mixer_amd/runtime.py
+++ b/m2_mixer_amd/runtime.py
@@ -1,7 +1,7 @@
 from __future__ import annotations
 
 import ctypes as C
-from typing import Dict, List, Optional, Sequence
+from typing import Dict, List, Optional, Sequence, Tuple
 
 import torch
 
@@ -347,12 +347,15 @@
         return bool(L.lib().m2m_tower_backward_heads_ok(C.byref(self.desc), B, nheads, K))
 
     def backward_heads(self, B: int, heads: Sequence[dict], own: int, labels: torch.Tensor, K: int, out, d_x0: torch.Tensor,
-                       d_x0_ss: int, seed: int, step: int, step_dev: Optional[torch.Tensor] = None):
+                       d_x0_ss: int, seed: int, step: int, step_dev: Optional[torch.Tensor] = None,
+                       weights: Optional[torch.Tensor] = None):
+        _check_weights(weights, len(heads))
         arr = _head_array(heads)
         logits, losses, preds = out
-        L.check(L.lib().m2m_tower_backward_heads(C.byref(self.desc), B, arr, len(heads), own, labels.data_ptr(), K, logits.data_ptr(),
-                                                 losses.data_ptr(), preds.data_ptr(), d_x0.data_ptr(), d_x0_ss,
-                                                 *_drop_tail(seed, step, step_dev)), "tower_backward_heads")
+        tail = _drop_tail(seed, step, step_dev)
+        L.check(L.lib().m2m_tower_backward_heads_w(C.byref(self.desc), B, arr, len(heads), own, labels.data_ptr(), K, logits.data_ptr(),
+                                                   losses.data_ptr(), preds.data_ptr(), d_x0.data_ptr(), d_x0_ss,
+                                                   *tail[:3], L.ptr(weights), tail[3]), "tower_backward_heads")
 
     def wgrad(self, B: int, seed: int, step: int, step_dev: Optional[torch.Tensor] = None):
         L.check(L.lib().m2m_tower_wgrad(C.byref(self.desc), B, *_drop_tail(seed, step, step_dev)), "tower_wgrad")
@@ -421,11 +424,16 @@
 def towers_wgrad(towers: Sequence[TowerRuntime], B: int, embeds: Sequence["EmbedRuntime"] = (),
                  inputs: Sequence[torch.Tensor] = (), d_x0s: Sequence[torch.Tensor] = (), seed: int = 0, step: int = 0,
                  step_dev: Optional[torch.Tensor] = None, embed_towers: Sequence[TowerRuntime] = (),
-                 heads: Optional[Sequence[dict]] = None, K: int = 0, bump: Optional[torch.Tensor] = None):
+                 heads: Optional[Sequence[dict]] = None, K: int = 0, bump: Optional[torch.Tensor] = None,
+                 bwd_heads: Optional[Tuple[int, torch.Tensor]] = None):
     n, ne = len(towers), len(embeds)
     et = _tower_ptrs(embed_towers) if len(embed_towers) == ne and ne else None
     args = (_tower_ptrs(towers), _device_descs(towers), n, _embed_ptrs(embeds), _data_ptrs(inputs), _data_ptrs(d_x0s), et, ne, B,
             *_drop_tail(seed, step, step_dev)[:3])
+    if bwd_heads is not None:
+        L.check(L.lib().m2m_towers_wgrad_bwd_heads(*args, _head_array(heads), len(heads), K, int(bwd_heads[0]), bwd_heads[1].data_ptr(),
+                                                   L.ptr(bump), L.stream_ptr()), "towers_wgrad_bwd_heads")
+        return
     if bump is not None:
         L.check(L.lib().m2m_towers_wgrad_tail(*args, _head_array(heads) if heads else None, len(heads) if heads else 0, K,
                                               bump.data_ptr(), L.stream_ptr()), "towers_wgrad_tail")
```
